# JonasGeiping/fullbatchtraining

Measured on AMD Instinct MI355X. Metric: full-batch GD images/sec (ResNet-18 CIFAR-10 shaped, all chunks accumulated per step), higher is better.
Workload: dtype bf16

## Files before the change

fullbatchtraining_amd/csrc/bn.hip:

```cpp
#include "common.h"
#include "profile.h"

__device__ __forceinline__ bool partial_sum2(const float* __restrict__ part, int n_mblocks, int blocks_per_group, int C, int g,
                                             int& c, double& s, double& q) {
    __shared__ double red[2][64][16];
    const int segs = (int)blockDim.x >> 4;
    const int cl = threadIdx.x & 15, seg = threadIdx.x >> 4;
    c = blockIdx.x * 16 + cl;
    double a = 0.0, b = 0.0;
    if (c < C) {
        const float* ps = part + ((long long)g * blocks_per_group) * C + c;
        const float* pq = part + ((long long)n_mblocks + (long long)g * blocks_per_group) * C + c;
        for (int k = seg; k < blocks_per_group; k += segs) { a += (double)ps[(long long)k * C]; b += (double)pq[(long long)k * C]; }
    }
    red[0][seg][cl] = a; red[1][seg][cl] = b;
    __syncthreads();
    if (seg != 0 || c >= C) return false;
    s = 0.0; q = 0.0;
    for (int k = 0; k < segs; ++k) { s += red[0][k][cl]; q += red[1][k][cl]; }
    return true;
}
static inline int bn_finalize_threads(int blocks_per_group) { return blocks_per_group >= 256 ? 1024 : 256; }

__global__ void bn_fwd_finalize_kernel(const float* __restrict__ part, int n_mblocks, int blocks_per_group, int C, double inv_count,
// ... 238 lines not shown
    float m = rm[c], v = rv[c];
    const float ub = unbias[c], keep = 1.f - momentum;
    for (int g = 0; g < n_groups; ++g)
        for (int p = 0; p < n_passes; ++p) {
            const long long o = p * pass_stride + (long long)g * ch_total + c;
            m = keep * m + momentum * mean_tab[o];
            v = keep * v + momentum * (var_tab[o] * ub);
        }
    rm[c] = m; rv[c] = v;
}

extern "C" int fb_bn_running_update(float* running_mean, float* running_var, const float* mean_tab, const float* var_tab, int32_t n_passes,
                                    int64_t pass_stride, const float* unbias, int32_t n_groups, int32_t ch_total, float momentum,
                                    void* stream) {
    if (!running_mean || !running_var || !mean_tab || !var_tab || !unbias) FB_FAIL(FB_ERR_ARG, "fb_bn_running_update: null pointer");
    hipLaunchKernelGGL(bn_running_update_kernel, dim3((ch_total + 255) / 256), dim3(256), 0, (hipStream_t)stream, running_mean,
                       running_var, mean_tab, var_tab, n_passes, (long long)pass_stride, unbias, n_groups, ch_total, momentum);
    FB_CHECK_LAUNCH("fb_bn_running_update");
    return FB_OK;
}

static inline int bn_reduce_pixels(long long n_pixels, long long ppg) {
    int pb = 128;
    while (pb < 1024 && ppg % (2 * pb) == 0 && n_pixels / (2 * pb) >= 2048) pb *= 2;
    return pb;
}
extern "C" int32_t fb_bn_bwd_reduce_rows(int64_t n_pixels, int64_t pixels_per_group) {
    if (n_pixels <= 0 || pixels_per_group <= 0) return 0;
    const int pb = bn_reduce_pixels(n_pixels, pixels_per_group);
    return (int32_t)((n_pixels + pb - 1) / pb);
}

struct BnReduceB { const uint4* x; const float* invstd; float* partial; int ch_off; };
template <typename T, bool DUAL = false>
__global__ __launch_bounds__(256) void bn_bwd_reduce_kernel(const uint4* __restrict__ dout, const uint4* __restrict__ y,
                                                            const unsigned char* __restrict__ mask,
                                                            const uint4* __restrict__ x, const float* __restrict__ mean_tab,
                                                            const float* __restrict__ invstd, int ch_total, int ch_off,
                                                            float* __restrict__ partial, long long n_pixels, int C, long long ppg,
                                                            int n_mblocks, int PB, const BnReduceB B) {
    constexpr int V = ET<T>::VEC;
    extern __shared__ float sm[];
    const int cvec = C / V;
    const long long p0 = (long long)blockIdx.x * PB;
    const long long g = p0 / ppg;
    const long long p1 = p0 + PB < n_pixels ? p0 + PB : n_pixels;
    auto mask_at = [&](long long i) -> unsigned {
        if (mask) return mask[i];
        if (!y) return 0xffu;
        float yv[V];
        ET<T>::unpack(y[i], yv);
        unsigned mk = 0;
#pragma unroll
        for (int k = 0; k < V; ++k) mk |= (yv[k] > 0.f ? 1u : 0u) << k;
        return mk;
    };
    int rows;
    if (256 % cvec == 0) {
        rows = 256 / cvec;
        const int cv = threadIdx.x % cvec, row = threadIdx.x / cvec, c0 = cv * V;
        float mu[V], is[V], s1[V], s2[V];
        float muB[DUAL ? V : 1], isB[DUAL ? V : 1], s2B[DUAL ? V : 1];
#pragma unroll
        for (int k = 0; k < V; ++k) { mu[k] = mean_tab[g * ch_total + ch_off + c0 + k]; is[k] = invstd[g * C + c0 + k]; s1[k] = 0.f; s2[k] = 0.f; }
        if constexpr (DUAL) {
#pragma unroll
            for (int k = 0; k < V; ++k) { muB[k] = mean_tab[g * ch_total + B.ch_off + c0 + k]; isB[k] = B.invstd[g * C + c0 + k]; s2B[k] = 0.f; }
        }
        auto one = [&](const uint4& dr, const uint4& xr, const uint4& xbr, unsigned mk) {
            float d[V], xv[V];
            ET<T>::unpack(dr, d); ET<T>::unpack(xr, xv);
#pragma unroll
            for (int k = 0; k < V; ++k) {
                const float dy = ((mk >> k) & 1u) ? d[k] : 0.f;
                s1[k] += dy; s2[k] += dy * ((xv[k] - mu[k]) * is[k]);
            }
            if constexpr (DUAL) {
                float xb[V];
                ET<T>::unpack(xbr, xb);
#pragma unroll
                for (int k = 0; k < V; ++k) {
                    const float dy = ((mk >> k) & 1u) ? d[k] : 0.f;
                    s2B[k] += dy * ((xb[k] - muB[k]) * isB[k]);
                }
            }
        };
        const long long hi = p1 * cvec;
        long long i = p0 * cvec + threadIdx.x;
        for (; i + (BN_SPAN_U - 1) * 256 < hi; i += BN_SPAN_U * 256) {
            uint4 dr[BN_SPAN_U], xr[BN_SPAN_U], xbr[BN_SPAN_U];
            unsigned mk[BN_SPAN_U];
#pragma unroll
            for (int u = 0; u < BN_SPAN_U; ++u) {
                dr[u] = ld_reduce(dout + i + u * 256); xr[u] = ld_reduce(x + i + u * 256); mk[u] = mask_at(i + u * 256);
                if constexpr (DUAL) xbr[u] = ld_reduce(B.x + i + u * 256); else xbr[u] = xr[u];
            }
#pragma unroll
            for (int u = 0; u < BN_SPAN_U; ++u) one(dr[u], xr[u], xbr[u], mk[u]);
        }
        for (; i < hi; i += 256) { if constexpr (DUAL) one(dout[i], x[i], B.x[i], mask_at(i)); else one(dout[i], x[i], x[i], mask_at(i)); }
#pragma unroll
        for (int k = 0; k < V; ++k) { sm[(row * C + c0 + k) * 2] = s1[k]; sm[(row * C + c0 + k) * 2 + 1] = s2[k]; }
        if constexpr (DUAL) {
#pragma unroll
            for (int k = 0; k < V; ++k) sm[2 * rows * C + row * C + c0 + k] = s2B[k];
        }
    } else {
        rows = 256 / cvec > 0 ? 256 / cvec : 1;
        const int lanes = cvec < 256 ? cvec : 256;
        for (int cv = threadIdx.x % lanes; cv < cvec; cv += lanes) {
            const int row = threadIdx.x / lanes;
            const int c0 = cv * V;
            float mu[V], is[V], s1[V], s2[V];
#pragma unroll
            for (int k = 0; k < V; ++k) { mu[k] = mean_tab[g * ch_total + ch_off + c0 + k]; is[k] = invstd[g * C + c0 + k]; s1[k] = 0.f; s2[k] = 0.f; }
            if (row < rows) {
                for (long long pidx = p0 + row; pidx < p1; pidx += rows) {
                    const long long i = pidx * cvec + cv;
                    float d[V], xv[V];
                    ET<T>::unpack(dout[i], d); ET<T>::unpack(x[i], xv);
                    const unsigned mk = mask_at(i);
#pragma unroll
                    for (int k = 0; k < V; ++k) {
                        const float dy = ((mk >> k) & 1u) ? d[k] : 0.f;
                        s1[k] += dy; s2[k] += dy * ((xv[k] - mu[k]) * is[k]);
                    }
                }
#pragma unroll
                for (int k = 0; k < V; ++k) { sm[(row * C + c0 + k) * 2] = s1[k]; sm[(row * C + c0 + k) * 2 + 1] = s2[k]; }
            }
        }
    }
    __syncthreads();
    for (int c = threadIdx.x; c < C; c += 256) {
        float a = 0.f, b = 0.f;
        for (int r = 0; r < rows; ++r) { a += sm[(r * C + c) * 2]; b += sm[(r * C + c) * 2 + 1]; }
        partial[(long long)blockIdx.x * C + c] = a;
        partial[((long long)n_mblocks + blockIdx.x) * C + c] = b;
        if constexpr (DUAL) {
            float bb = 0.f;
            for (int r = 0; r < rows; ++r) bb += sm[2 * rows * C + r * C + c];
            B.partial[(long long)blockIdx.x * C + c] = a;
            B.partial[((long long)n_mblocks + blockIdx.x) * C + c] = bb;
        }
    }
}

extern "C" int fb_bn_bwd_reduce(const void* dout, const void* y, const void* mask, const void* x, const float* mean_tab, const float* invstd,
                                int32_t ch_total, int32_t ch_off, float* partial, int64_t n_pixels, int32_t C,
                                int64_t pixels_per_group, int32_t dtype, void* stream) {
    if (!dout || !x || !mean_tab || !invstd || !partial) FB_FAIL(FB_ERR_ARG, "fb_bn_bwd_reduce: null pointer");
    if (pixels_per_group % 128 != 0) FB_FAIL(FB_ERR_SHAPE, "fb_bn_bwd_reduce: pixels_per_group=%lld must be a multiple of 128", (long long)pixels_per_group);
    const int V = dtype == FB_F32 ? 4 : 8;
    if (C % V != 0) FB_FAIL(FB_ERR_SHAPE, "fb_bn_bwd_reduce: C=%d", C);
    const int cvec = C / V, rows = 256 / cvec > 0 ? 256 / cvec : 1;
    const int PB = bn_reduce_pixels(n_pixels, pixels_per_group);
    const int n_mblocks = fb_bn_bwd_reduce_rows(n_pixels, pixels_per_group);
    const size_t smem = (size_t)rows * C * 2 * sizeof(float);
    if (smem > 64 * 1024) FB_FAIL(FB_ERR_UNSUPPORTED, "fb_bn_bwd_reduce: C=%d too large", C);
    const int32_t info[FB_PROF_INFO] = {(int32_t)(n_pixels / 128), C, (int32_t)(pixels_per_group / 128), dtype, 0, (mask || y) ? 1 : 0, 0, 0, 0, 0, 0};
    const int prof = fb_prof_begin(FB_PROF_BN_BWD_REDUCE, (hipStream_t)stream, info);
    if (dtype == FB_F32)
        hipLaunchKernelGGL((bn_bwd_reduce_kernel<float>), dim3(n_mblocks), dim3(256), smem, (hipStream_t)stream, (const uint4*)dout, (const uint4*)y,
                           (const unsigned char*)mask, (const uint4*)x, mean_tab, invstd, ch_total, ch_off, partial, (long long)n_pixels, C, (long long)pixels_per_group, n_mblocks, PB, BnReduceB{});
    else
        hipLaunchKernelGGL((bn_bwd_reduce_kernel<bf16_tag>), dim3(n_mblocks), dim3(256), smem, (hipStream_t)stream, (const uint4*)dout, (const uint4*)y,
                           (const unsigned char*)mask, (const uint4*)x, mean_tab, invstd, ch_total, ch_off, partial, (long long)n_pixels, C, (long long)pixels_per_group, n_mblocks, PB, BnReduceB{});
    fb_prof_end(prof, (hipStream_t)stream);
    FB_CHECK_LAUNCH("fb_bn_bwd_reduce");
    return FB_OK;
}

extern "C" int fb_bn_bwd_reduce2(const void* dout, const void* mask, const void* x_a, const float* invstd_a, int32_t ch_off_a, float* partial_a,
                                 const void* x_b, const float* invstd_b, int32_t ch_off_b, float* partial_b, const float* mean_tab, int32_t ch_total,
                                 int64_t n_pixels, int32_t C, int64_t pixels_per_group, int32_t dtype, void* stream) {
    if (!dout || !x_a || !x_b || !mean_tab || !invstd_a || !invstd_b || !partial_a || !partial_b) FB_FAIL(FB_ERR_ARG, "fb_bn_bwd_reduce2: null pointer");
    if (pixels_per_group % 128 != 0) FB_FAIL(FB_ERR_SHAPE, "fb_bn_bwd_reduce2: pixels_per_group=%lld must be a multiple of 128", (long long)pixels_per_group);
    const int V = dtype == FB_F32 ? 4 : 8;
    if (C % V != 0 || 256 % (C / V) != 0) FB_FAIL(FB_ERR_UNSUPPORTED, "fb_bn_bwd_reduce2: C=%d (the channel vectors of a pixel must divide 256)", C);
    const int cvec = C / V, rows = 256 / cvec;
    const int PB = bn_reduce_pixels(n_pixels, pixels_per_group);
    const int n_mblocks = fb_bn_bwd_reduce_rows(n_pixels, pixels_per_group);
    const size_t smem = (size_t)rows * C * 3 * sizeof(float);
    const int32_t info[FB_PROF_INFO] = {(int32_t)(n_pixels / 128), C, (int32_t)(pixels_per_group / 128), dtype, 1 , mask ? 1 : 0, 0, 0, 0, 0, 0};
    const int prof = fb_prof_begin(FB_PROF_BN_BWD_REDUCE, (hipStream_t)stream, info);
    const BnReduceB B{(const uint4*)x_b, invstd_b, partial_b, ch_off_b};
    if (dtype == FB_F32)
        hipLaunchKernelGGL((bn_bwd_reduce_kernel<float, true>), dim3(n_mblocks), dim3(256), smem, (hipStream_t)stream, (const uint4*)dout, (const uint4*)nullptr,
                           (const unsigned char*)mask, (const uint4*)x_a, mean_tab, invstd_a, ch_total, ch_off_a, partial_a, (long long)n_pixels, C, (long long)pixels_per_group, n_mblocks, PB, B);
    else
        hipLaunchKernelGGL((bn_bwd_reduce_kernel<bf16_tag, true>), dim3(n_mblocks), dim3(256), smem, (hipStream_t)stream, (const uint4*)dout, (const uint4*)nullptr,
                           (const unsigned char*)mask, (const uint4*)x_a, mean_tab, invstd_a, ch_total, ch_off_a, partial_a, (long long)n_pixels, C, (long long)pixels_per_group, n_mblocks, PB, B);
    fb_prof_end(prof, (hipStream_t)stream);
    FB_CHECK_LAUNCH("fb_bn_bwd_reduce2");
    return FB_OK;
}

__global__ void bn_bwd_finalize_kernel(const float* __restrict__ part, int n_mblocks, int blocks_per_group, int C, double inv_count,
                                       const float* __restrict__ scale, const float* __restrict__ mean_tab, const float* __restrict__ invstd,
                                       int ch_total, int ch_off, float* __restrict__ dgamma, float* __restrict__ dbeta, long long gstride,
                                       float* __restrict__ coef, int raw_x) {
    const int g = blockIdx.y;
    int c; double s1, s2;
    if (!partial_sum2(part, n_mblocks, blocks_per_group, C, g, c, s1, s2)) return;
    if (raw_x)
        s2 = (double)invstd[(long long)g * C + c] * (s2 - (double)mean_tab[(long long)g * ch_total + ch_off + c] * s1);
    dbeta[(long long)g * gstride + c] = (float)s1;
    dgamma[(long long)g * gstride + c] = (float)s2;
    const double sc = scale[(long long)g * C + c], is = invstd[(long long)g * C + c], mu = mean_tab[(long long)g * ch_total + ch_off + c];
    const double cx = -sc * is * s2 * inv_count;
    float* o = coef + ((long long)g * C + c) * 3;
    o[0] = (float)sc; o[1] = (float)cx; o[2] = (float)(-sc * s1 * inv_count - cx * mu);
}

extern "C" int fb_bn_bwd_finalize(const float* partial, int32_t n_mblocks, int32_t n_groups, int32_t C, double count, const float* scale,
                                  const float* mean_tab, const float* invstd, int32_t ch_total, int32_t ch_off, float* dgamma,
                                  float* dbeta, int64_t grad_group_stride, float* coef, int32_t raw_x, void* stream) {
    if (!partial || !scale || !mean_tab || !invstd || !dgamma || !dbeta || !coef) FB_FAIL(FB_ERR_ARG, "fb_bn_bwd_finalize: null pointer");
    if (n_mblocks % n_groups != 0) FB_FAIL(FB_ERR_SHAPE, "fb_bn_bwd_finalize: blocks/groups");
    dim3 grid((C + 15) / 16, n_groups);
    hipLaunchKernelGGL(bn_bwd_finalize_kernel, grid, dim3(bn_finalize_threads(n_mblocks / n_groups)), 0, (hipStream_t)stream, partial, n_mblocks, n_mblocks / n_groups, C, 1.0 / count,
                       scale, mean_tab, invstd, ch_total, ch_off, dgamma, dbeta, (long long)grad_group_stride, coef, (int)raw_x);
    FB_CHECK_LAUNCH("fb_bn_bwd_finalize");
    return FB_OK;
}

template <typename T>
__global__ void bn_bwd_apply_kernel(const uint4* __restrict__ dout, const uint4* __restrict__ y, const unsigned char* __restrict__ mask,
                                    const uint4* __restrict__ x,
                                    const float* __restrict__ coef, uint4* __restrict__ dx, uint4* __restrict__ dy_out, long long n_vec,
                                    int cvec, long long vec_per_group, int C) {
    constexpr int V = ET<T>::VEC;
    for (long long i = (long long)blockIdx.x * blockDim.x + threadIdx.x; i < n_vec; i += (long long)gridDim.x * blockDim.x) {
        const int c0 = (int)(i % cvec) * V;
        const long long g = i / vec_per_group;
        float d[V], xv[V], yv[V], o[V], dyv[V];
        ET<T>::unpack(dout[i], d); ET<T>::unpack(x[i], xv);
        unsigned mk = 0xffu;
        if (mask) mk = mask[i];
        else if (y) {
            ET<T>::unpack(y[i], yv);
            mk = 0;
#pragma unroll
            for (int k = 0; k < V; ++k) mk |= (yv[k] > 0.f ? 1u : 0u) << k;
        }
        const float* cf = coef + (g * C + c0) * 3;
#pragma unroll
        for (int k = 0; k < V; ++k) {
            const float dy = ((mk >> k) & 1u) ? d[k] : 0.f;
            dyv[k] = dy;
            o[k] = fb_bn_dx(cf[3 * k], cf[3 * k + 1], cf[3 * k + 2], dy, xv[k]);
        }
        dx[i] = ET<T>::pack(o);
        if (dy_out) dy_out[i] = ET<T>::pack(dyv);
    }
}

struct BnApplyB { const uint4* x; const float* coef; uint4* dx; };
template <typename T, bool DUAL = false>
__global__ __launch_bounds__(256) void bn_bwd_apply_span_kernel(const uint4* __restrict__ dout, const uint4* __restrict__ y,
                                                                const unsigned char* __restrict__ mask, const uint4* __restrict__ x,
                                                                const float* __restrict__ coef, uint4* __restrict__ dx, uint4* __restrict__ dy_out,
                                                                long long n_vec, int cvec, long long vec_per_group, int C, int span, float* __restrict__ amax,
                                                                BnApplyB B) {
    constexpr int V = ET<T>::VEC;
    float am = 0.f;
    const long long g = blockIdx.y, base = g * vec_per_group;
    const long long lim = n_vec - base < vec_per_group ? n_vec - base : vec_per_group;
    const long long lo = (long long)blockIdx.x * span;
    const long long hi = lo + span < lim ? lo + span : lim;
    const int c0 = (int)(threadIdx.x % cvec) * V;
    float cf[3 * V];
    load_coef<3 * V>(coef + (g * C + c0) * 3, cf);
    float cfB[DUAL ? 3 * V : 1];
    if constexpr (DUAL) { load_coef<3 * V>(B.coef + (g * C + c0) * 3, cfB); B.x += base; B.dx += base; }
    dout += base; x += base; dx += base;
    if (mask) mask += base;
    if (y) y += base;
    if (dy_out) dy_out += base;
    auto one = [&](const uint4& dr, const uint4& xr, const uint4& xbr, unsigned mk, long long i) {
        float d[V], xv[V], o[V], dyv[V];
        ET<T>::unpack(dr, d); ET<T>::unpack(xr, xv);
#pragma unroll
        for (int k = 0; k < V; ++k) {
            const float dy = ((mk >> k) & 1u) ? d[k] : 0.f;
            dyv[k] = dy;
            o[k] = fb_bn_dx(cf[3 * k], cf[3 * k + 1], cf[3 * k + 2], dy, xv[k]);
        }
        if (amax) {
#pragma unroll
            for (int k = 0; k < V; ++k) am = fmaxf(am, fabsf(o[k]));
        }
        st_stream(dx + i, ET<T>::pack(o));
        if (dy_out) st_stream(dy_out + i, ET<T>::pack(dyv));
        if constexpr (DUAL) {
            float xb[V], ob[V];
            ET<T>::unpack(xbr, xb);
#pragma unroll
            for (int k = 0; k < V; ++k) ob[k] = fb_bn_dx(cfB[3 * k], cfB[3 * k + 1], cfB[3 * k + 2], dyv[k], xb[k]);
            st_stream(B.dx + i, ET<T>::pack(ob));
        }
    };
    auto mask_at = [&](long long i) -> unsigned {
        if (mask) return mask[i];
        if (!y) return 0xffu;
        float yv[V];
        ET<T>::unpack(y[i], yv);
        unsigned mk = 0;
#pragma unroll
        for (int k = 0; k < V; ++k) mk |= (yv[k] > 0.f ? 1u : 0u) << k;
        return mk;
    };
    long long i = lo + threadIdx.x;
    for (; i + (BN_SPAN_U - 1) * 256 < hi; i += BN_SPAN_U * 256) {
        uint4 dr[BN_SPAN_U], xr[BN_SPAN_U], xbr[BN_SPAN_U];
        unsigned mk[BN_SPAN_U];
#pragma unroll
        for (int u = 0; u < BN_SPAN_U; ++u) {
            dr[u] = ld_stream(dout + i + u * 256); xr[u] = ld_stream(x + i + u * 256); mk[u] = mask_at(i + u * 256);
            if constexpr (DUAL) xbr[u] = ld_stream(B.x + i + u * 256); else xbr[u] = xr[u];
        }
#pragma unroll
        for (int u = 0; u < BN_SPAN_U; ++u) one(dr[u], xr[u], xbr[u], mk[u], i + u * 256);
    }
    for (; i < hi; i += 256) { if constexpr (DUAL) one(dout[i], x[i], B.x[i], mask_at(i), i); else one(dout[i], x[i], x[i], mask_at(i), i); }
    if (amax) amax_commit(amax, am);
}

extern "C" int fb_bn_bwd_apply(const void* dout, const void* y, const void* mask, const void* x, const float* coef, void* dx, void* dy_out,
                               int64_t n_pixels, int32_t C, int64_t pixels_per_group, int32_t dtype, float* amax_out, float* amax_ws, void* stream) {
    if (!dout || !x || !coef || !dx) FB_FAIL(FB_ERR_ARG, "fb_bn_bwd_apply: null pointer");
    if (amax_out && (dtype != FB_F32 || !amax_ws)) FB_FAIL(FB_ERR_ARG, "fb_bn_bwd_apply: amax_out is for fp32 tensors and needs amax_ws (fb_ws_bn_amax_floats)");
    const int64_t n_groups = (n_pixels + pixels_per_group - 1) / pixels_per_group;
    const int V = dtype == FB_F32 ? 4 : 8;
    const int cvec = C / V;
    const long long n_vec = n_pixels * cvec, vpg = pixels_per_group * cvec;
    const int32_t info[FB_PROF_INFO] = {(int32_t)(n_pixels / 128), C, (int32_t)(pixels_per_group / 128), dtype, 0, (mask || y) ? 1 : 0, dy_out ? 1 : 0, 0, 0, 0, 0};
    if (256 % cvec == 0 && vpg > 0) {
        const int prof = fb_prof_begin(FB_PROF_BN_BWD_APPLY, (hipStream_t)stream, info);
        const int span = bn_span(n_vec);
        const dim3 grid((unsigned)((vpg + span - 1) / span), (unsigned)((n_vec + vpg - 1) / vpg));
        if (dtype == FB_F32)
            hipLaunchKernelGGL((bn_bwd_apply_span_kernel<float>), grid, dim3(256), 0, (hipStream_t)stream, (const uint4*)dout, (const uint4*)y,
                               (const unsigned char*)mask, (const uint4*)x, coef, (uint4*)dx, (uint4*)dy_out, n_vec, cvec, vpg, C, span, amax_out ? amax_ws : nullptr, BnApplyB{});
        else
            hipLaunchKernelGGL((bn_bwd_apply_span_kernel<bf16_tag>), grid, dim3(256), 0, (hipStream_t)stream, (const uint4*)dout, (const uint4*)y,
                               (const unsigned char*)mask, (const uint4*)x, coef, (uint4*)dx, (uint4*)dy_out, n_vec, cvec, vpg, C, span, nullptr, BnApplyB{});
        fb_prof_end(prof, (hipStream_t)stream);
        if (amax_out) hipLaunchKernelGGL(amax_finish_kernel, dim3(grid.y), dim3(256), 0, (hipStream_t)stream, amax_ws, (int)grid.x, amax_out);
        FB_CHECK_LAUNCH("fb_bn_bwd_apply");
        return FB_OK;
    }
    const int blocks = (int)((n_vec + 255) / 256 < 8192 ? (n_vec + 255) / 256 : 8192);
    if (dtype == FB_F32)
        hipLaunchKernelGGL((bn_bwd_apply_kernel<float>), dim3(blocks), dim3(256), 0, (hipStream_t)stream, (const uint4*)dout, (const uint4*)y,
                           (const unsigned char*)mask, (const uint4*)x, coef, (uint4*)dx, (uint4*)dy_out, n_vec, cvec, vpg, C);
    else
        hipLaunchKernelGGL((bn_bwd_apply_kernel<bf16_tag>), dim3(blocks), dim3(256), 0, (hipStream_t)stream, (const uint4*)dout, (const uint4*)y,
                           (const unsigned char*)mask, (const uint4*)x, coef, (uint4*)dx, (uint4*)dy_out, n_vec, cvec, vpg, C);
    FB_CHECK_LAUNCH("fb_bn_bwd_apply");
    if (amax_out) return fb_absmax((const float*)dx, pixels_per_group * C, (int32_t)n_groups, pixels_per_group * C, 1, amax_out, stream);
    return FB_OK;
}


extern "C" int fb_bn_bwd_apply2(const void* dout, const void* mask, const void* x_a, const float* coef_a, void* dx_a, const void* x_b, const float* coef_b,
                                void* dx_b, int64_t n_pixels, int32_t C, int64_t pixels_per_group, int32_t dtype, void* stream) {
    if (!dout || !x_a || !coef_a || !dx_a || !x_b || !coef_b || !dx_b) FB_FAIL(FB_ERR_ARG, "fb_bn_bwd_apply2: null pointer");
    const int V = dtype == FB_F32 ? 4 : 8;
    if (C % V != 0 || 256 % (C / V) != 0 || pixels_per_group <= 0) FB_FAIL(FB_ERR_UNSUPPORTED, "fb_bn_bwd_apply2: C=%d (the channel vectors of a pixel must divide 256)", C);
    const int cvec = C / V;
    const long long n_vec = n_pixels * cvec, vpg = pixels_per_group * cvec;
    const int32_t info[FB_PROF_INFO] = {(int32_t)(n_pixels / 128), C, (int32_t)(pixels_per_group / 128), dtype, 1 , mask ? 1 : 0, 0, 0, 0, 0, 0};
    const int prof = fb_prof_begin(FB_PROF_BN_BWD_APPLY, (hipStream_t)stream, info);
    const int span = bn_span(n_vec);
    const dim3 grid((unsigned)((vpg + span - 1) / span), (unsigned)((n_vec + vpg - 1) / vpg));
    const BnApplyB B{(const uint4*)x_b, coef_b, (uint4*)dx_b};
    if (dtype == FB_F32)
        hipLaunchKernelGGL((bn_bwd_apply_span_kernel<float, true>), grid, dim3(256), 0, (hipStream_t)stream, (const uint4*)dout, (const uint4*)nullptr,
                           (const unsigned char*)mask, (const uint4*)x_a, coef_a, (uint4*)dx_a, (uint4*)nullptr, n_vec, cvec, vpg, C, span, (float*)nullptr, B);
    else
        hipLaunchKernelGGL((bn_bwd_apply_span_kernel<bf16_tag, true>), grid, dim3(256), 0, (hipStream_t)stream, (const uint4*)dout, (const uint4*)nullptr,
                           (const unsigned char*)mask, (const uint4*)x_a, coef_a, (uint4*)dx_a, (uint4*)nullptr, n_vec, cvec, vpg, C, span, (float*)nullptr, B);
    fb_prof_end(prof, (hipStream_t)stream);
    FB_CHECK_LAUNCH("fb_bn_bwd_apply2");
    return FB_OK;
}
```

fullbatchtraining_amd/csrc/cmdlist.cpp:

```cpp
#include <stdlib.h>

#include <memory>
#include <utility>
#include <vector>

#include "common.h"

namespace {

template <typename T> inline T word_as(uint64_t w) {
    T v;
    memcpy(&v, &w, sizeof(T));
    return v;
}

using Thunk = int (*)(const uint64_t*, void*);

template <typename F, F f> struct Bind;
template <typename... A, int (*f)(A...)> struct Bind<int (*)(A...), f> {
    static constexpr int N = sizeof...(A);
    template <size_t I, typename T> static T arg(const uint64_t* w, void* st) {
        if constexpr (I == N - 1) return (T)st;
        else return word_as<T>(w[I]);
    }
    template <size_t... I> static int run(const uint64_t* w, void* st, std::index_sequence<I...>) { return f(arg<I, A>(w, st)...); }
    static int call(const uint64_t* w, void* st) { return run(w, st, std::index_sequence_for<A...>{}); }
};

struct Entry { const char* name; Thunk fn; int nargs; };
#define FB_ENTRY(name) {#name, &Bind<decltype(&name), &name>::call, Bind<decltype(&name), &name>::N}
const Entry kEntries[] = {
    FB_ENTRY(fb_conv2d), FB_ENTRY(fb_conv2d_wgrad), FB_ENTRY(fb_absmax), FB_ENTRY(fb_wgrad_reduce), FB_ENTRY(fb_weight_prep),
    FB_ENTRY(fb_bn_fwd_finalize), FB_ENTRY(fb_bn_apply), FB_ENTRY(fb_bn_running_update), FB_ENTRY(fb_bn_bwd_reduce),
    FB_ENTRY(fb_bn_bwd_finalize), FB_ENTRY(fb_bn_bwd_apply), FB_ENTRY(fb_avgpool2_fwd), FB_ENTRY(fb_maxpool3s2_fwd),
    FB_ENTRY(fb_maxpool3s2_bwd), FB_ENTRY(fb_head_pool), FB_ENTRY(fb_head_loss), FB_ENTRY(fb_head_bwd), FB_ENTRY(fb_mt_sqnorm),
    FB_ENTRY(fb_mt_accumulate), FB_ENTRY(fb_mt_fd_perturb), FB_ENTRY(fb_mt_fd_combine_accumulate), FB_ENTRY(fb_mt_fd_combine),
    FB_ENTRY(fb_mt_chunk_clip), FB_ENTRY(fb_bn_eval_coeffs), FB_ENTRY(fb_mt_norms2), FB_ENTRY(fb_mt_clip_sgd), FB_ENTRY(fb_mt_scale), FB_ENTRY(fb_bn_bwd_fused), FB_ENTRY(fb_bn_bwd_reduce2), FB_ENTRY(fb_bn_bwd_apply2),
    FB_ENTRY(fb_conv2d_wgrad_chain), FB_ENTRY(fb_mt_accumulate_sum), FB_ENTRY(fb_mt_accumulate_skip),
    FB_ENTRY(fb_maxpool3s2_fwd_idx), FB_ENTRY(fb_maxpool3s2_bwd_idx),
};
constexpr int kNumEntries = sizeof(kEntries) / sizeof(kEntries[0]);

enum { CMD_CALL = 0, CMD_EVENT_RECORD = 1, CMD_EVENT_WAIT = 2 };
struct Cmd { int32_t kind, fn, stream, ev; uint32_t off, n; };
struct CmdList {
    std::vector<Cmd> cmds;
    std::vector<uint64_t> words;
    std::vector<std::unique_ptr<uint64_t[]>> blobs;
};

std::vector<hipEvent_t> g_events;

}

extern "C" int32_t fb_cmd_fn_id(const char* name) {
    for (int i = 0; i < kNumEntries; ++i)
        if (strcmp(kEntries[i].name, name) == 0) return i;
    return -1;
}
extern "C" int32_t fb_cmd_fn_nargs(int32_t fn) { return fn >= 0 && fn < kNumEntries ? kEntries[fn].nargs : -1; }

extern "C" int32_t fb_event_new(void) {
    hipEvent_t e;
    if (hipEventCreateWithFlags(&e, hipEventDisableTiming) != hipSuccess) {
        snprintf(fb_err_buf, sizeof(fb_err_buf), "fb_event_new: hipEventCreateWithFlags failed");
        return -1;
    }
    g_events.push_back(e);
    return (int32_t)g_events.size() - 1;
}
extern "C" int32_t fb_event_count(void) { return (int32_t)g_events.size(); }
extern "C" int fb_event_record(int32_t ev, void* stream) {
// ... 62 lines not shown
```

fullbatchtraining_amd/csrc/common.h:

```cpp
#pragma once
#include <hip/hip_runtime.h>
#include <stdint.h>
#include <stdio.h>
#include <string.h>

#include "../../include/fb_engine.h"

typedef __attribute__((ext_vector_type(8))) __bf16 bf16x8_t;
typedef __attribute__((ext_vector_type(4))) short s16x4_t;
typedef __attribute__((ext_vector_type(4))) float f32x4_t;

extern thread_local char fb_err_buf[512];
#define FB_FAIL(code, ...)                                   \
    do {                                                     \
        snprintf(fb_err_buf, sizeof(fb_err_buf), __VA_ARGS__); \
        return (code);                                       \
    } while (0)
#define FB_CHECK_LAUNCH(name)                                                                   \
    do {                                                                                        \
        hipError_t e_ = hipGetLastError();                                                      \
        if (e_ != hipSuccess) FB_FAIL(FB_ERR_LAUNCH, "%s: launch failed: %s", name, hipGetErrorString(e_)); \
    } while (0)

static inline int64_t ceil_div64(int64_t a, int64_t b) { return (a + b - 1) / b; }
// ... 234 lines not shown
    c = __builtin_amdgcn_mfma_f32_16x16x32_f16(ah, bh, c, 0, 0, 0);
    return c;
}
__device__ __forceinline__ f32x4_t mma_planes3h(const uint4 (&a)[2], const uint4 (&b)[2], f32x4_t c, float inv) {
    const f16x8_t ah = __builtin_bit_cast(f16x8_t, a[0]), al = __builtin_bit_cast(f16x8_t, a[1]);
    const f16x8_t bh = __builtin_bit_cast(f16x8_t, b[0]), bl = __builtin_bit_cast(f16x8_t, b[1]);
    f32x4_t t = {0.f, 0.f, 0.f, 0.f};
    t = __builtin_amdgcn_mfma_f32_16x16x32_f16(al, bh, t, 0, 0, 0);
    t = __builtin_amdgcn_mfma_f32_16x16x32_f16(ah, bl, t, 0, 0, 0);
    t = __builtin_amdgcn_mfma_f32_16x16x32_f16(ah, bh, t, 0, 0, 0);
    return fma4(t, inv, c);
}
bool fb_f32_split_enabled();
bool fb_experimental();
const char* fb_getenv_experimental(const char* name);
int fb_persistent_cus();

typedef __attribute__((ext_vector_type(4))) unsigned fb_store_u32x4;
#ifndef FB_STORE_GUARD_NOPS
#define FB_STORE_GUARD_NOPS 3
#endif
__device__ __forceinline__ void store_b128_guard(fb_store_u32x4 data) {
#if FB_STORE_GUARD_NOPS >= 0
#ifdef FB_STORE_GUARD_NOMEM
    asm volatile("s_nop %1" ::"v"(data), "n"(FB_STORE_GUARD_NOPS));
#else
    asm volatile("s_nop %1" ::"v"(data), "n"(FB_STORE_GUARD_NOPS) : "memory");
#endif
#endif
}

__device__ __forceinline__ float fb_bn_dx(float c_dy, float c_x, float c_0, float dy, float x) { return fmaf(c_dy, dy, fmaf(c_x, x, c_0)); }

__device__ __forceinline__ float row16_sum(float v) {
    v += __builtin_bit_cast(float, __builtin_amdgcn_update_dpp(0, __builtin_bit_cast(int, v), 0x128, 0xf, 0xf, false));
    v += __builtin_bit_cast(float, __builtin_amdgcn_update_dpp(0, __builtin_bit_cast(int, v), 0x124, 0xf, 0xf, false));
    v += __builtin_bit_cast(float, __builtin_amdgcn_update_dpp(0, __builtin_bit_cast(int, v), 0x122, 0xf, 0xf, false));
    v += __builtin_bit_cast(float, __builtin_amdgcn_update_dpp(0, __builtin_bit_cast(int, v), 0x121, 0xf, 0xf, false));
    return v;
}

template <int NV> __device__ __forceinline__ void block_reduce_sum(float (&v)[NV], float* smem) {
    const int lane = threadIdx.x & 63, wave = threadIdx.x >> 6, nw = (blockDim.x + 63) >> 6;
#pragma unroll
    for (int i = 0; i < NV; ++i) {
#pragma unroll
        for (int off = 32; off > 0; off >>= 1) v[i] += __shfl_xor(v[i], off);
    }
    if (lane == 0)
        for (int i = 0; i < NV; ++i) smem[i * nw + wave] = v[i];
    __syncthreads();
    if (threadIdx.x == 0)
        for (int i = 0; i < NV; ++i) {
            float s = 0.f;
            for (int w = 0; w < nw; ++w) s += smem[i * nw + w];
            v[i] = s;
        }
    __syncthreads();
}
```

fullbatchtraining_amd/csrc/conv3x3_halo5.hip:

```cpp
#include "common.h"

#include <type_traits>

struct Halo5Params {
    const char* src; const char* wgt; char* dst; const char* addend; float* stat;
    const unsigned char* addend_mask;
    const char* bst_x; const unsigned char* bst_mask;
    int n_img, mode, addend_mode, n_mblocks, n_tiles;
#ifdef FB_H5_TRACE
    long long* trace;
#endif
};
#ifdef FB_H5_TRACE
#define H5_STAMP(k) do { if (tid == 0) p.trace[(long long)L * 8 + (k)] = wall_clock64(); } while (0)
#else
#define H5_STAMP(k) do { } while (0)
#endif

namespace {
template <int N> __device__ __forceinline__ void h5_wait_vmcnt() { asm volatile("s_waitcnt vmcnt(%0)" ::"n"(N) : "memory"); }
template <int N> __device__ __forceinline__ void h5_wait_lgkmcnt() {
    asm volatile("s_waitcnt lgkmcnt(%0)" ::"n"(N) : "memory");
    __builtin_amdgcn_sched_barrier(0);
}
typedef __attribute__((ext_vector_type(4))) unsigned h5_u32x4;
typedef __attribute__((ext_vector_type(2))) unsigned h5_u32x2;
template <int OFF> __device__ __forceinline__ uint4 h5_read16(unsigned byte_addr) {
    h5_u32x4 v;
    asm volatile("ds_read_b128 %0, %1 offset:%2" : "=v"(v) : "v"(byte_addr), "n"(OFF));
    return make_uint4(v[0], v[1], v[2], v[3]);
}
template <int I, int N, typename F> __device__ __forceinline__ void h5_static_for(F&& f) {
    if constexpr (I < N) { f(std::integral_constant<int, I>{}); h5_static_for<I + 1, N>(f); }
}
__device__ __forceinline__ int h5_xcd_remap(int b, int n) {
    const int q = n >> 3, r = n & 7, xcd = b & 7, slot = b >> 3;
    return (xcd < r ? xcd * (q + 1) : r * (q + 1) + (xcd - r) * q) + slot;
}
constexpr unsigned H5_OOB = 0x80000000u;
constexpr int H5_W = 32, H5_TH = 8, H5_PITCH = 34, H5_ROWS = (H5_TH + 2) * H5_PITCH;
constexpr int H5_NGRP = (H5_ROWS + 7) / 8;
constexpr int H5_HALO_BYTES = H5_NGRP * 1024, H5_WT_BYTES = 64 * 128, H5_WGT_BYTES = 9 * H5_WT_BYTES;
constexpr int H5_KH = (H5_NGRP + 3) / 4;
#ifndef FB_H5_ADD_DEPTH
#define FB_H5_ADD_DEPTH 3
#endif
constexpr int H5_AD = FB_H5_ADD_DEPTH, H5_ADN = H5_AD + 1;
}

template <int MODE, int ADD, int BST = 0>
__global__ __launch_bounds__(256) void conv3x3s1_c64_halo5_kernel(const Halo5Params p) {
#if defined(__HIP_DEVICE_COMPILE__)
    constexpr int W = H5_W, PITCH = H5_PITCH;
    __shared__ __attribute__((aligned(16))) char lds[H5_WGT_BYTES + 2 * H5_HALO_BYTES + 1024];

    const int tid = threadIdx.x, lane = tid & 63;
    const int wave = __builtin_amdgcn_readfirstlane(tid >> 6);
    const int ph = wave & 1, ch = wave >> 1;
    const int NB = gridDim.x;
    const int lrow8 = lane >> 3, t = lane & 15, g = lane >> 4;
    const unsigned lds0 = (unsigned)(size_t)(__attribute__((address_space(3))) char*)lds;

    {
        const __amdgpu_buffer_rsrc_t rW = __builtin_amdgcn_make_buffer_rsrc((void*)p.wgt, 0, 64 * 9 * 128, 0x00020000);
#pragma unroll
        for (int u = 0; u < 9; ++u) {
            const int tap = MODE == 0 ? u : 8 - u;
#pragma unroll
            for (int k = 0; k < 2; ++k) {
                const int piece = wave + 4 * k;
                const unsigned voff = (unsigned)((piece * 8 + lrow8) * 9 * 128 + (((lane & 7) ^ lrow8) * 16));
                __builtin_amdgcn_raw_ptr_buffer_load_lds(rW, (__attribute__((address_space(3))) void*)(lds + u * H5_WT_BYTES + piece * 1024), 16, voff,
                                                         tap * 128, 0, 0);
            }
        }
    }
    unsigned voffH[H5_KH];
    unsigned topbits = 0, botbits = 0;
#pragma unroll
    for (int k = 0; k < H5_KH; ++k) {
        const int row = (wave + 4 * k) * 8 + lrow8;
        const int hy = row / PITCH, hx = row - hy * PITCH;
        const bool ok = row < H5_ROWS && hx >= 1 && hx <= W;
        voffH[k] = ok ? (unsigned)((hy * W + hx) * 128 + (((lane & 7) ^ (hx & 7)) * 16)) : H5_OOB;
        topbits |= (hy == 0 ? 1u : 0u) << k;
        botbits |= (hy == H5_TH + 1 ? 1u : 0u) << k;
    }
    unsigned wa[2], wb[2];
#pragma unroll
    for (int h = 0; h < 2; ++h) {
        wa[h] = lds0 + (ch * 32 + t) * 128 + (((g + 4 * h) ^ (t & 7)) * 16);
        wb[h] = wa[h] + 4 * H5_WT_BYTES;
    }
    unsigned pa[2][3][2];
#pragma unroll
    for (int bf = 0; bf < 2; ++bf)
#pragma unroll
        for (int b = 0; b < 3; ++b)
#pragma unroll
            for (int h = 0; h < 2; ++h)
                pa[bf][b][h] = lds0 + H5_WGT_BYTES + bf * H5_HALO_BYTES + (ph * 4 * PITCH + t + b) * 128 + (((g + 4 * h) ^ ((t + b) & 7)) * 16);
    const int voffD = ((ph * 128 + t) * 64 + ch * 32 + g * 4) * 2;
    const int voffS = ((ph * 128 + t) * 64 + ch * 32 + (g & 1) * 16 + (g >> 1) * 8) * 2;

    auto halo_piece = [&](auto kc, int buf, int L, bool live) {
        constexpr int K = decltype(kc)::value;
        const int grp = wave + 4 * K;
        const int n0 = L >> 2, y0 = (L & 3) * H5_TH;
        const long long origin = ((long long)(n0 * W + y0 - 1) * W - 1) * 128;
        const __amdgpu_buffer_rsrc_t rA = __builtin_amdgcn_make_buffer_rsrc((void*)(p.src + origin), 0, ((H5_TH + 2) * W + 2) * 128, 0x00020000);
        const unsigned dead = (y0 == 0 ? topbits : 0u) | (y0 + H5_TH == W ? botbits : 0u);
        const unsigned v = (((dead >> K) & 1u) || !live) ? H5_OOB : voffH[K];
        const int dst = grp < H5_NGRP ? H5_WGT_BYTES + buf * H5_HALO_BYTES + grp * 1024 : H5_WGT_BYTES + 2 * H5_HALO_BYTES;
        __builtin_amdgcn_raw_ptr_buffer_load_lds(rA, (__attribute__((address_space(3))) void*)(lds + dst), 16, v, 0, 0, 0);
    };

    float ssum[2][4], ssq[2][4];
    h5_u32x2 ad[H5_ADN][2];
    unsigned adm[H5_ADN];
    h5_u32x2 bx[H5_ADN][2];
    unsigned bxm[H5_ADN];
    auto ad_issue = [&](auto jc, const int Lp) {
        constexpr int J = decltype(jc)::value;
        if constexpr (BST != 0 && J < 8) {
            const __amdgpu_buffer_rsrc_t rsrcX = __builtin_amdgcn_make_buffer_rsrc((void*)(p.bst_x + (long long)Lp * 256 * 128), 0, 256 * 128, 0x00020000);
#pragma unroll
            for (int i = 0; i < 2; ++i) bx[J % H5_ADN][i] = __builtin_amdgcn_raw_buffer_load_b64(rsrcX, voffD + i * 32, J * 2048, 0);
            const __amdgpu_buffer_rsrc_t rsrcN = __builtin_amdgcn_make_buffer_rsrc((void*)(p.bst_mask + (long long)Lp * 256 * 8), 0, 256 * 8, 0x00020000);
            bxm[J % H5_ADN] = __builtin_amdgcn_raw_buffer_load_b32(rsrcN, ((ph * 128 + t) * 8 + ch * 4), J * 128, 0);
        }
        if constexpr (ADD != 0 && J < 8) {
            const __amdgpu_buffer_rsrc_t rsrcE = __builtin_amdgcn_make_buffer_rsrc((void*)(p.addend + (long long)Lp * 256 * 128), 0, 256 * 128, 0x00020000);
#pragma unroll
            for (int i = 0; i < 2; ++i) ad[J % H5_ADN][i] = __builtin_amdgcn_raw_buffer_load_b64(rsrcE, voffD + i * 32, J * 2048, 0);
            if constexpr (ADD == 2) {
                const __amdgpu_buffer_rsrc_t rsrcM = __builtin_amdgcn_make_buffer_rsrc((void*)(p.addend_mask + (long long)Lp * 256 * 8), 0, 256 * 8, 0x00020000);
                adm[J % H5_ADN] = __builtin_amdgcn_raw_buffer_load_b32(rsrcM, ((ph * 128 + t) * 8 + ch * 4), J * 128, 0);
            }
        }
    };
    auto epi_prefetch = [&](const int Lp) { h5_static_for<0, H5_AD>([&](auto jc) { ad_issue(jc, Lp); }); };
    auto epi_slice = [&](auto sc, f32x4_t (&accp)[2][8], const int Lp) {
        constexpr int S = decltype(sc)::value;
        if constexpr (S < 16) {
            if constexpr (S == 0) {
#pragma unroll
                for (int i = 0; i < 2; ++i)
// ... 35 lines not shown
                        for (int r = 0; r < 4; ++r) { ssum[i][r] += v[r]; ssq[i][r] += v[r] * v[r]; }
                    }
                }
                const h5_u32x2 lo = __builtin_amdgcn_permlane16_swap(pk[0][0], pk[1][0], false, false);
                const h5_u32x2 hi = __builtin_amdgcn_permlane16_swap(pk[0][1], pk[1][1], false, false);
                const h5_u32x4 outv = {lo[0], hi[0], lo[1], hi[1]};
                __builtin_amdgcn_raw_buffer_store_b128(outv, rsrcD, voffS, J * 2048, 0);
                store_b128_guard(outv);
                ad_issue(std::integral_constant<int, J + H5_AD>{}, Lp);
            }
        } else if constexpr (S == 16) {
            if constexpr (MODE == 0 || BST != 0) {
#pragma unroll
                for (int i = 0; i < 2; ++i)
#pragma unroll
                    for (int r = 0; r < 4; ++r) { ssum[i][r] = row16_sum(ssum[i][r]); ssq[i][r] = row16_sum(ssq[i][r]); }
            }
        } else {
            if ((MODE == 0 || BST != 0) && t == 0) {
                const long long blk = 2LL * Lp + ph;
#pragma unroll
                for (int i = 0; i < 2; ++i) {
                    const int co = ch * 32 + i * 16 + g * 4;
                    *(float4*)(p.stat + blk * 64 + co) = make_float4(ssum[i][0], ssum[i][1], ssum[i][2], ssum[i][3]);
                    *(float4*)(p.stat + ((long long)p.n_mblocks + blk) * 64 + co) = make_float4(ssq[i][0], ssq[i][1], ssq[i][2], ssq[i][3]);
                }
            }
        }
    };

    int L = h5_xcd_remap(blockIdx.x, NB);
    if (L >= p.n_tiles) return;
    h5_static_for<0, H5_KH>([&](auto kc) { halo_piece(kc, 0, L, true); });

    f32x4_t accA[2][8], accB[2][8];

    auto tile = [&](auto bufc, auto prevc, const int L, const bool has_next) {
        constexpr int BUF = decltype(bufc)::value;
        constexpr bool PREV = decltype(prevc)::value;
        f32x4_t (&acc)[2][8] = BUF ? accB : accA;
        f32x4_t (&accp)[2][8] = BUF ? accA : accB;
        H5_STAMP(0);
        h5_wait_vmcnt<0>();
        __builtin_amdgcn_s_barrier();
        H5_STAMP(1);
#pragma unroll
        for (int i = 0; i < 2; ++i)
#pragma unroll
            for (int j = 0; j < 8; ++j) acc[i][j] = (f32x4_t){0.f, 0.f, 0.f, 0.f};

        uint4 wf[2][2], pf[2][8];
        auto issue_reads = [&](auto sc) {
            constexpr int S = decltype(sc)::value, U = S >> 1, H = S & 1, A = U / 3, B = U % 3, SET = S & 1;
            h5_static_for<0, 2>([&](auto ic) {
                constexpr int I = decltype(ic)::value;
                if constexpr (U < 4) wf[SET][I] = h5_read16<U * H5_WT_BYTES + I * 2048>(wa[H]);
                else wf[SET][I] = h5_read16<(U - 4) * H5_WT_BYTES + I * 2048>(wb[H]);
            });
            h5_static_for<0, 8>([&](auto jc) {
                constexpr int J = decltype(jc)::value;
                pf[SET][J] = h5_read16<((A + (J >> 1)) * PITCH + (J & 1) * 16) * 128>(pa[BUF][B][H]);
            });
        };
        issue_reads(std::integral_constant<int, 0>{});
        if constexpr (PREV) epi_prefetch(L - NB);
        h5_static_for<0, 18>([&](auto sc) {
            constexpr int S = decltype(sc)::value, SET = S & 1;
            if constexpr (S + 1 < 18) {
                issue_reads(std::integral_constant<int, S + 1>{});
                h5_wait_lgkmcnt<10>();
            } else {
                h5_wait_lgkmcnt<0>();
            }
#pragma unroll
            for (int i = 0; i < 2; ++i)
#pragma unroll
                for (int j = 0; j < 8; ++j) acc[i][j] = mma_chunk<bf16_tag>(wf[SET][i], pf[SET][j], acc[i][j]);
            if constexpr (PREV) epi_slice(sc, accp, L - NB);
            if constexpr (PREV) {
#pragma unroll
                for (int k = 0; k < 16; ++k) {
                    __builtin_amdgcn_sched_group_barrier(0x008, 1, 0);
                    __builtin_amdgcn_sched_group_barrier(0x002, 2, 0);
                }
            }
            if constexpr (S < H5_KH) halo_piece(std::integral_constant<int, S>{}, BUF ^ 1, has_next ? L + NB : L, has_next);
        });
        H5_STAMP(3);
    };

    bool has_next = L + NB < p.n_tiles;
    tile(std::integral_constant<int, 0>{}, std::false_type{}, L, has_next);
    int parity = 0;
    while (has_next) {
        L += NB;
        has_next = L + NB < p.n_tiles;
        tile(std::integral_constant<int, 1>{}, std::true_type{}, L, has_next);
        parity = 1;
        if (!has_next) break;
        L += NB;
        has_next = L + NB < p.n_tiles;
        tile(std::integral_constant<int, 0>{}, std::true_type{}, L, has_next);
        parity = 0;
    }
    epi_prefetch(L);
    if (parity == 0) h5_static_for<0, 18>([&](auto sc) { epi_slice(sc, accA, L); });
    else h5_static_for<0, 18>([&](auto sc) { epi_slice(sc, accB, L); });
    h5_wait_vmcnt<0>();
    H5_STAMP(4); H5_STAMP(5);
#endif
}

int fb_conv3x3_halo5_takes(const fb_conv_args* a) {
    static const bool disabled = getenv("FB_DISABLE_HALO5") != nullptr;
    if (disabled || a->dtype != FB_BF16) return 0;
    if (a->R != 3 || a->S != 3 || a->stride != 1 || a->pad != 1) return 0;
    if (a->Hs != 32 || a->Ws != 32 || a->Hd != 32 || a->Wd != 32 || a->Cs != 64 || a->Cd != 64) return 0;
    if (a->imgs_per_wset > 0 && a->imgs_per_wset < a->n_img) return 0;
    if (a->addend && a->addend_mode != 1) return 0;
    if (a->addend_mask && (!a->addend || a->mode != 1)) return 0;
    if (a->mode == 0 && !a->stat_partial) return 0;
    if (a->bst_x && (a->mode != 1 || !a->bst_mask || !a->stat_partial)) return 0;
    return 1;
}

int fb_try_conv3x3_halo5(const fb_conv_args* a, hipStream_t st) {
    if (!fb_conv3x3_halo5_takes(a)) return 0;
    const int n_cu = fb_persistent_cus();
    Halo5Params p;
    p.src = (const char*)a->src; p.wgt = (const char*)a->wgt; p.dst = (char*)a->dst; p.addend = (const char*)a->addend;
    p.stat = (a->mode == 0 || a->bst_x) ? a->stat_partial : nullptr;
    p.addend_mask = (const unsigned char*)a->addend_mask;
    p.bst_x = (const char*)a->bst_x; p.bst_mask = (const unsigned char*)a->bst_mask;
    p.n_img = a->n_img; p.mode = a->mode; p.addend_mode = a->addend ? 1 : 0;
    p.n_tiles = a->n_img * 4;
    p.n_mblocks = p.n_tiles * 2;
#ifdef FB_H5_TRACE
    extern long long* g_h5_trace;
    p.trace = g_h5_trace;
#endif
    const dim3 grid(p.n_tiles < n_cu ? p.n_tiles : n_cu);
    if (a->mode == 0) {
        hipLaunchKernelGGL((conv3x3s1_c64_halo5_kernel<0, 0>), grid, dim3(256), 0, st, p);
    } else if (a->bst_x) {
        if (a->addend && a->addend_mask) hipLaunchKernelGGL((conv3x3s1_c64_halo5_kernel<1, 2, 1>), grid, dim3(256), 0, st, p);
        else if (a->addend) hipLaunchKernelGGL((conv3x3s1_c64_halo5_kernel<1, 1, 1>), grid, dim3(256), 0, st, p);
        else hipLaunchKernelGGL((conv3x3s1_c64_halo5_kernel<1, 0, 1>), grid, dim3(256), 0, st, p);
    } else if (a->addend && a->addend_mask) {
        hipLaunchKernelGGL((conv3x3s1_c64_halo5_kernel<1, 2>), grid, dim3(256), 0, st, p);
    } else if (a->addend) {
        hipLaunchKernelGGL((conv3x3s1_c64_halo5_kernel<1, 1>), grid, dim3(256), 0, st, p);
    } else {
        hipLaunchKernelGGL((conv3x3s1_c64_halo5_kernel<1, 0>), grid, dim3(256), 0, st, p);
    }
    return 1;
}
```

fullbatchtraining_amd/csrc/conv_igemm.hip:

```cpp
#include "common.h"
#include "profile.h"

#include "conv_params.h"

template <typename T, int BN_CO>
__global__ __launch_bounds__(256) void conv_igemm_kernel(const ConvParams p) {
    constexpr int EB = ET<T>::EB;
    constexpr int BKE = 128 / EB;
    constexpr int WROWS = BN_CO / 32;
    constexpr int FI = BN_CO / 32;
    constexpr int FJ = 4;
    constexpr int TILE_CHUNKS = (128 + BN_CO) * 8;
    __shared__ uint4 lds[2 * TILE_CHUNKS];

    const int tid = threadIdx.x, lane = tid & 63, wave = tid >> 6;
    const int wave_co = wave >> 1, wave_px = wave & 1;
    const int mblk = blockIdx.x, co_blk = blockIdx.y, cls = blockIdx.z;
    const int cpy = (p.os == 2) ? (cls >> 1) : 0, cpx = (p.os == 2) ? (cls & 1) : 0;
    const int chunk = tid & 7, lrow = tid >> 3;

    int a_img[4], a_y[4], a_x[4];
    const int qHW = p.qH * p.qW;
#pragma unroll
    for (int i = 0; i < 4; ++i) {
// ... 125 lines not shown
#pragma unroll
                for (int r = 0; r < 4; ++r) { ssum[i][r] += v[r]; ssq[i][r] += v[r] * v[r]; }
            }
        }
    }
    if (p.stat != nullptr) {
        float* red = (float*)lds;
        __syncthreads();
#pragma unroll
        for (int i = 0; i < FI; ++i)
#pragma unroll
            for (int r = 0; r < 4; ++r) {
                float a = ssum[i][r], b = ssq[i][r];
                a = row16_sum(a); b = row16_sum(b);
                if ((lane & 15) == 0) {
                    const int col = wave_co * (BN_CO / 2) + i * 16 + (lane >> 4) * 4 + r;
                    red[(wave_px * BN_CO + col) * 2] = a; red[(wave_px * BN_CO + col) * 2 + 1] = b;
                }
            }
        __syncthreads();
        if (tid < BN_CO) {
            const float a = red[tid * 2] + red[(BN_CO + tid) * 2];
            const float b = red[tid * 2 + 1] + red[(BN_CO + tid) * 2 + 1];
            const long long blk = (long long)cls * gridDim.x + mblk;
            p.stat[blk * p.Cd + co_blk * BN_CO + tid] = a;
            p.stat[((long long)p.n_mblocks + blk) * p.Cd + co_blk * BN_CO + tid] = b;
        }
    }
}

int fb_try_conv3x3_halo4(const fb_conv_args* a, hipStream_t st);
int fb_try_conv3x3_halo5(const fb_conv_args* a, hipStream_t st);
int fb_conv3x3_halo5_takes(const fb_conv_args* a);
int fb_try_conv3x3s2_dgrad_quad(const fb_conv_args* a, hipStream_t st);
int fb_try_conv1x1_k32(const fb_conv_args* a, hipStream_t st);
int fb_try_conv1x1_stream(const fb_conv_args* a, hipStream_t st);
int fb_try_conv1x1_gemm(const fb_conv_args* a, hipStream_t st);
int fb_try_conv1x1_pipe(const fb_conv_args* a, hipStream_t st);

int fb_conv1x1_pipe_takes(const fb_conv_args* a);
int fb_conv3x3_halo4_takes(const fb_conv_args* a);
int fb_conv1x1_gemm_takes(const fb_conv_args* a);
static int igemm_masked_addend_ok(const fb_conv_args* a) {
    if (getenv("FB_IGEMM_NO_MASK") != nullptr || a->mode != 1 || a->stride != 1 || a->bst_x) return 0;
    if (a->Cs % 32 != 0 || a->Cd % 64 != 0) return 0;
    static const bool v1 = getenv("FB_IGEMM_V1") != nullptr;
    if (v1) return 0;
    ConvParams p{};
    p.n_img = a->n_img; p.Hs = a->Hs; p.Ws = a->Ws; p.Cs = a->Cs; p.Hd = a->Hd; p.Wd = a->Wd; p.Cd = a->Cd; p.R = a->R; p.S = a->S;
    p.qH = a->Hd; p.qW = a->Wd;
    return fb_igemm_glds_fits(p, a->dtype);
}
extern "C" int32_t fb_conv_masked_addend_supported(const fb_conv_args* a) {
    if (!a || !a->addend || !a->addend_mask || a->addend_mode != 1) return 0;
    return fb_conv3x3_halo5_takes(a) || fb_conv1x1_pipe_takes(a) || fb_conv3x3_halo4_takes(a) || fb_conv1x1_gemm_takes(a) || igemm_masked_addend_ok(a);
}

extern "C" int32_t fb_conv_bwd_stat_supported(const fb_conv_args* a) {
    static const bool disabled = getenv("FB_DISABLE_FUSED_BWD_STAT") != nullptr;
    if (disabled || !a || !a->bst_x || !a->bst_mask || !a->stat_partial || a->mode != 1 || a->dtype != FB_BF16) return 0;
    if ((long long)a->n_img * a->Hd * a->Wd % 128 != 0) return 0;
    static const char* widths = getenv("FB_FUSED_BWD_STAT_W");
    if (widths) {
        char tag[8];
        snprintf(tag, sizeof(tag), "%d,", a->Wd);
        char list[64];
        snprintf(list, sizeof(list), "%s,", widths);
        if (!strstr(list, tag) || (a->Wd < 10 && list != strstr(list, tag) && *(strstr(list, tag) - 1) != ',')) return 0;
    }
    return fb_conv3x3_halo5_takes(a) || fb_conv3x3_halo4_takes(a);
}

template <typename T> static int launch_conv(const ConvParams& p, int classes, hipStream_t st) {
    const int mblocks = (p.M + 127) / 128;
    if (p.Cd % 128 == 0 && (long long)mblocks * (p.Cd / 128) * classes >= 512) {
        dim3 grid(mblocks, p.Cd / 128, classes);
        hipLaunchKernelGGL((conv_igemm_kernel<T, 128>), grid, dim3(256), 0, st, p);
    } else {
        dim3 grid(mblocks, p.Cd / 64, classes);
        hipLaunchKernelGGL((conv_igemm_kernel<T, 64>), grid, dim3(256), 0, st, p);
    }
    return 0;
}

extern "C" int fb_conv2d(const fb_conv_args* a, void* stream) {
    if (!a || !a->src || !a->wgt || !a->dst) FB_FAIL(FB_ERR_ARG, "fb_conv2d: null pointer");
    const int EB = a->dtype == FB_F32 ? 4 : 2;
    if (a->Cs % 32 != 0) FB_FAIL(FB_ERR_SHAPE, "fb_conv2d: Cs=%d must be a multiple of 32", a->Cs);
    if (a->Cd % 64 != 0) FB_FAIL(FB_ERR_SHAPE, "fb_conv2d: Cd=%d must be a multiple of 64", a->Cd);
    if (a->mode != 0 && a->mode != 1) FB_FAIL(FB_ERR_ARG, "fb_conv2d: mode %d", a->mode);
    if (a->addend_mask && !fb_conv_masked_addend_supported(a))
        FB_FAIL(FB_ERR_UNSUPPORTED, "fb_conv2d: addend_mask is not implemented for this shape (ask fb_conv_masked_addend_supported)");
    if (a->bst_x && !fb_conv_bwd_stat_supported(a))
        FB_FAIL(FB_ERR_UNSUPPORTED, "fb_conv2d: the fused BatchNorm-backward reduction is not implemented for this shape (ask fb_conv_bwd_stat_supported)");
    if (a->stride != 1 && a->stride != 2) FB_FAIL(FB_ERR_UNSUPPORTED, "fb_conv2d: stride %d", a->stride);
    ConvParams p;
    p.src = (const char*)a->src; p.wgt = (const char*)a->wgt; p.dst = (char*)a->dst; p.addend = (const char*)a->addend;
    p.stat = a->stat_partial;
    p.n_img = a->n_img; p.Hs = a->Hs; p.Ws = a->Ws; p.Cs = a->Cs; p.Hd = a->Hd; p.Wd = a->Wd; p.Cd = a->Cd;
    p.R = a->R; p.S = a->S; p.stride = a->stride; p.pad = a->pad; p.mode = a->mode;
    p.imgs_per_wset = a->imgs_per_wset > 0 ? a->imgs_per_wset : a->n_img;
    p.wset_stride_bytes = a->wset_stride * EB;
    p.addend_mode = a->addend ? a->addend_mode : 0;
    p.addend_mask = a->addend ? (const unsigned char*)a->addend_mask : nullptr;
    p.amax_src = a->dtype == FB_F32 ? a->amax_src : nullptr; p.amax_wgt = a->dtype == FB_F32 ? a->amax_wgt : nullptr;
    if ((p.amax_src == nullptr) != (p.amax_wgt == nullptr)) FB_FAIL(FB_ERR_ARG, "fb_conv2d: amax_src and amax_wgt go together");
    p.amax_imgs = a->amax_imgs > 0 ? a->amax_imgs : a->n_img;
    int classes = 1;
    if (a->mode == 0) {
        if (a->Hd != (a->Hs + 2 * a->pad - a->R) / a->stride + 1 || a->Wd != (a->Ws + 2 * a->pad - a->S) / a->stride + 1)
            FB_FAIL(FB_ERR_SHAPE, "fb_conv2d: fwd output %dx%d inconsistent with input %dx%d", a->Hd, a->Wd, a->Hs, a->Ws);
        p.qH = a->Hd; p.qW = a->Wd; p.os = 1; p.ss = a->stride;
    } else {
        if (a->Hs != (a->Hd + 2 * a->pad - a->R) / a->stride + 1 || a->Ws != (a->Wd + 2 * a->pad - a->S) / a->stride + 1)
            FB_FAIL(FB_ERR_SHAPE, "fb_conv2d: dgrad shapes inconsistent");
        if (a->stat_partial && !a->bst_x) FB_FAIL(FB_ERR_ARG, "fb_conv2d: statistics in mode 1 need bst_x / bst_mask");
        if (a->stride == 1) { p.qH = a->Hd; p.qW = a->Wd; p.os = 1; }
        else {
            if ((a->Hd & 1) || (a->Wd & 1)) FB_FAIL(FB_ERR_SHAPE, "fb_conv2d: stride-2 dgrad needs even input dims");
            p.qH = a->Hd / 2; p.qW = a->Wd / 2; p.os = 2; classes = 4;
        }
        p.ss = 1;
    }
    p.M = a->n_img * p.qH * p.qW;
    p.n_mblocks = ((p.M + 127) / 128) * classes;
    hipStream_t st = (hipStream_t)stream;
    const int32_t info[FB_PROF_INFO] = {a->n_img, a->Hs, a->Ws, a->Cs, a->Hd, a->Wd, a->Cd, a->R, a->stride,
                                        (a->addend ? a->addend_mode : 0) | (a->addend_mask ? 4 : 0) | (a->bst_x ? 8 : 0) | (a->dtype << 4), 0};
// ... 27 lines not shown
```

fullbatchtraining_amd/csrc/conv_wgrad.hip:

```cpp
#include "common.h"
#include "profile.h"

struct WgradParams {
    const char* x; const char* dy; float* out;
    int n_img, Hs, Ws, Cs, Hd, Wd, Cd;
    int R, S, stride, pad;
    int imgs_per_group, split_k, px_per_group, px_per_split;
    long long group_stride;
    const float* amax_x; const float* amax_dy;
    const char* bn_x; const unsigned char* bn_mask; const float* bn_coef;
};

template <typename T> struct WG;
template <> struct WG<bf16_tag> { static constexpr int PAD = 16; };
template <> struct WG<float> { static constexpr int PAD = 64; };
template <> struct WG<f32s_tag> : WG<float> {};
template <> struct WG<f32h_tag> : WG<float> {};

template <typename T> __device__ __forceinline__ void load_frag_t(const char* tile, int row_bytes, int pb, int c0, int lane, uint4 (&out)[2]);
template <> __device__ __forceinline__ void load_frag_t<bf16_tag>(const char* tile, int row_bytes, int pb, int c0, int lane, uint4 (&out)[2]) {
    const int t = lane & 15, g = lane >> 4;
    const char* a0 = tile + (pb + g * 8 + (t >> 2)) * row_bytes + (c0 + (t & 3) * 4) * 2;
    const s16x4_t lo = __builtin_amdgcn_ds_read_tr16_b64_v4i16((s16x4_t __attribute__((address_space(3)))*)(a0));
    const s16x4_t hi = __builtin_amdgcn_ds_read_tr16_b64_v4i16((s16x4_t __attribute__((address_space(3)))*)(a0 + 4 * row_bytes));
// ... 192 lines not shown
    if constexpr (WK > 1) {
        float* red = (float*)lds;
        __syncthreads();
#pragma unroll
        for (int i = 0; i < 4; ++i)
#pragma unroll
            for (int j = 0; j < NJ; ++j)
#pragma unroll
                for (int q = 0; q < 4; ++q) red[(wk * 64 + i * 16 + (lane >> 4) * 4 + q) * TN + wn * 16 * NJ + j * 16 + (lane & 15)] = acc[i][j][q];
        __syncthreads();
        for (int e = tid; e < 64 * TN; e += 256) {
            float v = 0.f;
#pragma unroll
            for (int w = 0; w < WK; ++w) v += red[w * 64 * TN + e];
            const int co = tile_m * TM + e / TN, ci = tile_n * TN + e % TN;
            out[((long long)co * taps + tap) * p.Cs + ci] = v;
        }
    } else {
#pragma unroll
        for (int i = 0; i < 4; ++i)
#pragma unroll
            for (int j = 0; j < NJ; ++j)
#pragma unroll
                for (int q = 0; q < 4; ++q) {
                    const int co = tile_m * TM + wm * 64 + i * 16 + (lane >> 4) * 4 + q;
                    const int ci = tile_n * TN + wn * 16 * NJ + j * 16 + (lane & 15);
                    out[((long long)co * taps + tap) * p.Cs + ci] = acc[i][j][q];
                }
    }
}

int fb_try_wgrad3x3(const fb_wgrad_args* a, hipStream_t st);
int fb_try_wgrad3x3_v2(const fb_wgrad_args* a, hipStream_t st);
int fb_try_wgrad1x1(const fb_wgrad_args* a, hipStream_t st);

extern "C" int32_t fb_wgrad_bn_fused_supported(const fb_wgrad_args* a) {
    static const bool disabled = getenv("FB_DISABLE_WGRAD_BNF") != nullptr;
    return !disabled && a && !a->amax_x && !a->amax_dy && a->R == 1 && a->S == 1 && a->stride == 1 && a->pad == 0 && a->Cs % 32 == 0 && a->Cs % 64 != 0
           && a->Cd % 64 == 0 && a->Hs == a->Hd && a->Ws == a->Wd;
}

extern "C" int fb_conv2d_wgrad(const fb_wgrad_args* a, void* stream) {
    if (!a || !a->x || !a->dy || !a->dw_partial) FB_FAIL(FB_ERR_ARG, "fb_conv2d_wgrad: null pointer");
    if (a->bn_x && (!a->bn_coef || !fb_wgrad_bn_fused_supported(a))) FB_FAIL(FB_ERR_UNSUPPORTED, "fb_conv2d_wgrad: bn_x (BatchNorm apply in the loader) is for 1x1 layers with Cs < 64 (no fp16x2 planes) and needs bn_coef");
    if (a->Cs % 32 != 0 || a->Cd % 64 != 0) FB_FAIL(FB_ERR_SHAPE, "fb_conv2d_wgrad: Cs=%d must be a multiple of 32, Cd=%d of 64", a->Cs, a->Cd);
    if (a->n_img % a->imgs_per_group != 0) FB_FAIL(FB_ERR_SHAPE, "fb_conv2d_wgrad: n_img %% imgs_per_group != 0");
    if (a->split_k < 1) FB_FAIL(FB_ERR_ARG, "fb_conv2d_wgrad: split_k < 1");
    WgradParams p;
    p.x = (const char*)a->x; p.dy = (const char*)a->dy; p.out = a->dw_partial;
    p.n_img = a->n_img; p.Hs = a->Hs; p.Ws = a->Ws; p.Cs = a->Cs; p.Hd = a->Hd; p.Wd = a->Wd; p.Cd = a->Cd;
    p.R = a->R; p.S = a->S; p.stride = a->stride; p.pad = a->pad;
    p.imgs_per_group = a->imgs_per_group; p.split_k = a->split_k;
    p.group_stride = a->group_stride ? a->group_stride : (long long)a->split_k * a->Cd * a->R * a->S * a->Cs;
    p.px_per_group = a->imgs_per_group * a->Hd * a->Wd;
    p.amax_x = a->dtype == FB_F32 ? a->amax_x : nullptr; p.amax_dy = a->dtype == FB_F32 ? a->amax_dy : nullptr;
    p.bn_x = (const char*)a->bn_x; p.bn_mask = (const unsigned char*)a->bn_mask; p.bn_coef = a->bn_coef;
    if ((p.amax_x == nullptr) != (p.amax_dy == nullptr)) FB_FAIL(FB_ERR_ARG, "fb_conv2d_wgrad: amax_x and amax_dy go together");
    const bool hsplit = p.amax_x != nullptr;
    const int n_groups = a->n_img / a->imgs_per_group;
    hipStream_t st = (hipStream_t)stream;
    const bool big = (a->Cs % 128 == 0) && (a->Cd % 128 == 0) && (a->Cs >= 256 || a->Cd >= 256 || a->R == 3);
    const int kstep = big ? (a->dtype == FB_F32 ? 32 : 64) : 128;
    p.px_per_split = (int)(ceil_div64(ceil_div64(p.px_per_group, a->split_k), kstep) * kstep);
    const int taps = a->R * a->S;
    const bool split = fb_f32_split_enabled();
    const int32_t info[FB_PROF_INFO] = {a->n_img, a->Hs, a->Ws, a->Cs, a->Hd, a->Wd, a->Cd, a->R, a->stride, a->split_k | (a->dtype << 16), FB_K_WGRAD_GENERIC};
    const int prof = fb_prof_begin(FB_PROF_WGRAD, st, info);
    static const bool wide160 = getenv("FB_DISABLE_WGRAD_WIDE160") == nullptr;
    if (wide160 && a->dtype == FB_BF16 && a->R == 1 && a->S == 1 && a->Cs % 160 == 0 && a->Cs % 64 != 0 && a->Cd % 64 == 0) {
        dim3 grid((a->Cd / 64) * (a->Cs / 160), taps, n_groups * a->split_k);
        if (a->bn_x) hipLaunchKernelGGL((conv_wgrad_kernel<bf16_tag, 1, 2, 2, 2, 5, true>), grid, dim3(256), 0, st, p);
        else hipLaunchKernelGGL((conv_wgrad_kernel<bf16_tag, 1, 2, 2, 2, 5, false>), grid, dim3(256), 0, st, p);
    } else if (a->bn_x) {
        dim3 grid((a->Cd / 64) * (a->Cs / 32), taps, n_groups * a->split_k);
        if (a->dtype == FB_F32 && split) hipLaunchKernelGGL((conv_wgrad_kernel<f32s_tag, 1, 1, 4, 1, 2, true>), grid, dim3(256), 0, st, p);
        else if (a->dtype == FB_F32) hipLaunchKernelGGL((conv_wgrad_kernel<float, 1, 1, 4, 1, 2, true>), grid, dim3(256), 0, st, p);
        else hipLaunchKernelGGL((conv_wgrad_kernel<bf16_tag, 1, 1, 4, 1, 2, true>), grid, dim3(256), 0, st, p);
    } else if (fb_try_wgrad3x3_v2(a, st)) { fb_prof_kernel(prof, FB_K_WGRAD3X3_V2);
// ... 160 lines not shown
```

fullbatchtraining_amd/csrc/conv_wgrad3x3_v2.hip:

```cpp
#include "common.h"

#include <type_traits>

struct Wgrad3V2Params {
    const char* x; const char* dy; float* out;
    int n_img, H, Cs, Cd;
    int imgs_per_group, imgs_per_block, split_k;
    long long group_stride;
    int n_chains; float* sq_part;
};

namespace {
typedef __attribute__((ext_vector_type(2))) unsigned w3_u32x2;
template <int OFF> __device__ __forceinline__ w3_u32x2 w3_read_tr(unsigned byte_addr) {
    w3_u32x2 v;
    asm volatile("ds_read_b64_tr_b16 %0, %1 offset:%2" : "=v"(v) : "v"(byte_addr), "n"(OFF));
    return v;
}
template <int N> __device__ __forceinline__ void w3_wait_lgkmcnt() {
    asm volatile("s_waitcnt lgkmcnt(%0)" ::"n"(N) : "memory");
    __builtin_amdgcn_sched_barrier(0);
}
template <int N> __device__ __forceinline__ void w3_wait_vmcnt() { asm volatile("s_waitcnt vmcnt(%0)" ::"n"(N) : "memory"); }
template <int I, int N, typename F> __device__ __forceinline__ void w3_static_for(F&& f) {
    if constexpr (I < N) { f(std::integral_constant<int, I>{}); w3_static_for<I + 1, N>(f); }
}
__device__ __forceinline__ uint4 w3_join(w3_u32x2 lo, w3_u32x2 hi) { return make_uint4(lo[0], lo[1], hi[0], hi[1]); }
__device__ __forceinline__ int w3_f(int row) { return ((row >> 1) & 1) | (((row >> 3) & 1) << 1); }
constexpr unsigned W3_OOB = 0x80000000u;

template <int W> struct W3GeoGen {
    static constexpr bool PER_BLOCK = true;
    static constexpr int RS = W == 56 ? 1 : (W == 28 ? 4 : 7);
    static constexpr int VALID = RS * W;
    static constexpr int KPX = (VALID + 31) / 32 * 32;
    static constexpr int PITCH = W == 56 ? 64 : (W == 28 ? 32 : 16);
    static constexpr int IMGS = 1;
    static constexpr int IMG_ROWS = (RS + 2) * PITCH;
    static constexpr int HROWS = IMG_ROWS;
    static constexpr bool WHOLE = false;
    __device__ static __forceinline__ int pix_row(int p, int s) { return p < VALID ? (p / W) * PITCH + (p % W) + s : 0; }
    static constexpr int blk_rows(int, int R) { return R * PITCH; }
// ... 27 lines not shown
    static constexpr int KPX = 32;
    static constexpr int PITCH = W == 16 ? 40 : (W == 8 ? 24 : 16);
    static constexpr int RS = W == 16 ? 2 : 4;
    static constexpr int IMGS = W == 4 ? 2 : 1;
    static constexpr int IMG_ROWS = (2 * RS + 1) * PITCH;
    static constexpr int HROWS = IMGS * IMG_ROWS;
    static constexpr int HI_DELTA = W == 4 ? 2 * PITCH : 8;
    static constexpr bool WHOLE = W == 4;
    __device__ static __forceinline__ int lane_row(int pl, int s) {
        if constexpr (W == 4) return (pl / 16) * IMG_ROWS + 2 * ((pl % 16) / 4) * PITCH + 2 * (pl % 4) + s;
        else return 2 * (pl / W) * PITCH + 2 * (pl % W) + s;
    }
    static constexpr int blk_rows(int, int R) { return R * PITCH; }
    __device__ static __forceinline__ int fB(int row) { return (row >> 1) & 3; }
};
struct W3GeoCP4 {
    static constexpr bool PER_BLOCK = false;
    static constexpr int VALID = 64, KPX = 64, PITCH = 4, RS = 4, IMGS = 4;
    static constexpr int IMG_ROWS = 17;
    static constexpr int BLK_ROWS = 48;
    static constexpr int HROWS = 88;
    static constexpr int HI_DELTA = 4;
    static constexpr bool WHOLE = true;
    __device__ static __forceinline__ int tap_row(int pl, int u) {
        const int img = pl / 16, y = (pl % 16) / 4 + u / 3 - 1, x = pl % 4 + u % 3 - 1;
        return img * IMG_ROWS + ((y >= 0 && y < 4 && x >= 0 && x < 4) ? y * 4 + x : 16);
    }
    __device__ static __forceinline__ int lane_row(int, int) { return 0; }
    static constexpr int blk_rows(int BLK, int) { return BLK * BLK_ROWS; }
    __device__ static __forceinline__ int fB(int row) { return w3_f(row); }
};
}

template <int W, int SD, bool CP = false, bool CHAIN = false>
__global__ __launch_bounds__(CHAIN ? 512 : 256) void conv_wgrad3x3_v2_kernel(const Wgrad3V2Params p) {
#if defined(__HIP_DEVICE_COMPILE__)
    static_assert(!CP || (W == 4 && SD == 1), "compact layout: 4x4 maps, stride 1");
    static_assert(!CHAIN || CP, "chunk chains: compact 4x4 layout");
    constexpr int NWV = CHAIN ? 8 : 4, FIW = CHAIN ? 2 : 4;
    using G = typename std::conditional<CP, W3GeoCP4, W3Geo<W, SD>>::type;
    constexpr int WI = SD * W;
    const int Hi = SD * p.H;
    constexpr int KPX = G::KPX, PITCH = G::PITCH, HROWS = G::HROWS;
    constexpr int A_BYTES = KPX * 128, B_BYTES = HROWS * 128, STAGE = A_BYTES + B_BYTES;
    constexpr int NGA = KPX / 8, NGB = HROWS / 8;
    constexpr int KA = (NGA + NWV - 1) / NWV, KB = (NGB + NWV - 1) / NWV;
    __shared__ __attribute__((aligned(16))) char lds[2 * STAGE];

    const int tid = threadIdx.x, lane = tid & 63;
    const int wave = __builtin_amdgcn_readfirstlane(tid >> 6);
    const int cib = CHAIN ? (wave & 3) : wave, coh = CHAIN ? (wave >> 2) : 0;
    const int tiles_n = p.Cs / 64, tiles = tiles_n * (p.Cd / 64);
    const int n_items = gridDim.x;
    int item;
    {
        const int b = blockIdx.x, q = n_items >> 3, r = n_items & 7, xcd = b & 7, slot = b >> 3;
        item = (xcd < r ? xcd * (q + 1) : r * (q + 1) + (xcd - r) * q) + slot;
    }
    const int tile = item % tiles, gs = item / tiles;
    const int tile_m = __builtin_amdgcn_readfirstlane(tile / tiles_n), tile_n = __builtin_amdgcn_readfirstlane(tile % tiles_n);
    const int group = __builtin_amdgcn_readfirstlane(CHAIN ? gs : gs / p.split_k), split = __builtin_amdgcn_readfirstlane(CHAIN ? 0 : gs % p.split_k);
    const int n_chunks = p.n_img / p.imgs_per_group;
    const int my_chunks = CHAIN ? (n_chunks - group + p.n_chains - 1) / p.n_chains : 0;
    const int spc = p.imgs_per_group / G::IMGS;
    const int img0 = CHAIN ? 0 : group * p.imgs_per_group + split * p.imgs_per_block;
    const int img_end = CHAIN ? p.n_img : min(img0 + p.imgs_per_block, (group + 1) * p.imgs_per_group);
    const int steps_per_img = G::WHOLE ? 1 : p.H / G::RS;
    const int n_steps = CHAIN ? my_chunks * spc : (G::WHOLE ? (img_end - img0) / G::IMGS : (img_end - img0) * steps_per_img);
    const int rowA_b = p.Cd * 2, rowB_b = p.Cs * 2;
// ... 30 lines not shown
            voffB[k] = (xok && sy >= 0 && sy < WI) ? base + (unsigned)(sy * WI * rowB_b) : W3_OOB;
        } else {
            hyB[k] = xok ? hy - 1 : -(1 << 20);
            voffB[k] = base;
        }
    }
    auto issue = [&](int stage, int step) {
        char* base = lds + stage * STAGE;
        int img, y0;
        if constexpr (CHAIN) { img = (group + (step / spc) * p.n_chains) * p.imgs_per_group + (step % spc) * G::IMGS; y0 = 0; }
        else if constexpr (G::WHOLE) { img = step * G::IMGS; y0 = 0; }
        else { img = step / steps_per_img; y0 = (step % steps_per_img) * G::RS; }
        const int soffA = (img * p.H + y0) * W * rowA_b;
#pragma unroll
        for (int k = 0; k < KA; ++k)
            if (wave + NWV * k < NGA)
                __builtin_amdgcn_raw_ptr_buffer_load_lds(rsrcA, (__attribute__((address_space(3))) void*)(base + (wave + NWV * k) * 1024), 16,
                                                         voffA[k], soffA, 0, 0);
        const int soffB = img * Hi * WI * rowB_b;
#pragma unroll
        for (int k = 0; k < KB; ++k) {
            if (wave + NWV * k < NGB) {
                unsigned v = voffB[k];
                if constexpr (!G::WHOLE) {
                    const int sy = SD * y0 + hyB[k];
                    v = (unsigned)sy < (unsigned)Hi ? voffB[k] + (unsigned)(sy * WI * rowB_b) : W3_OOB;
                }
                __builtin_amdgcn_raw_ptr_buffer_load_lds(rsrcB, (__attribute__((address_space(3))) void*)(base + A_BYTES + (wave + NWV * k) * 1024),
                                                         16, v, soffB, 0, 0);
            }
        }
    };

    const unsigned lds0 = (unsigned)(size_t)(__attribute__((address_space(3))) char*)lds;
    const int t = lane & 15, g = lane >> 4;
    const int pl = g * 8 + (t >> 2);
    unsigned la[FIW];
#pragma unroll
    for (int i = 0; i < FIW; ++i) la[i] = lds0 + pl * 128 + (((i + coh * FIW) ^ w3_f(pl)) * 32) + (t & 3) * 8;
    constexpr int NBLK = G::PER_BLOCK ? KPX / 32 : 1, NS = CP ? 9 : 3;
    unsigned lb[NBLK][NS], lbh[NBLK][NS];
#pragma unroll
    for (int blk = 0; blk < NBLK; ++blk)
#pragma unroll
        for (int s = 0; s < NS; ++s) {
            int row, rowh;
            if constexpr (CP) { row = W3GeoCP4::tap_row(pl, s); rowh = W3GeoCP4::tap_row(pl + 4, s); }
            else if constexpr (G::PER_BLOCK) { row = G::pix_row(blk * 32 + pl, s); rowh = G::pix_row(blk * 32 + pl + 4, s); }
            else { row = G::lane_row(pl, s); rowh = row + G::HI_DELTA; }
            lb[blk][s] = lds0 + A_BYTES + row * 128 + ((cib ^ G::fB(row)) * 32) + (t & 3) * 8;
            lbh[blk][s] = lds0 + A_BYTES + rowh * 128 + ((cib ^ G::fB(rowh)) * 32) + (t & 3) * 8;
        }

    f32x4_t acc[9][FIW], tot[CHAIN ? 9 : 1][CHAIN ? FIW : 1];
#pragma unroll
    for (int u = 0; u < 9; ++u)
#pragma unroll
        for (int i = 0; i < FIW; ++i) {
            acc[u][i] = (f32x4_t){0.f, 0.f, 0.f, 0.f};
            if constexpr (CHAIN) tot[u][i] = (f32x4_t){0.f, 0.f, 0.f, 0.f};
        }

    if (n_steps > 0) {
        issue(0, 0);
        w3_wait_vmcnt<0>();
        __builtin_amdgcn_s_barrier();
    }
    for (int step = 0; step < n_steps; ++step) {
        const int cur = step & 1;
        if (step + 1 < n_steps) issue(cur ^ 1, step + 1);
        const unsigned so = cur * STAGE;
        unsigned a0[FIW];
#pragma unroll
        for (int i = 0; i < FIW; ++i) a0[i] = la[i] + so;
        w3_static_for<0, KPX / 32>([&](auto blkc) {
            constexpr int BLK = decltype(blkc)::value;
            constexpr int PB = BLK * 32;
            constexpr int BI = G::PER_BLOCK ? BLK : 0;
            unsigned b0[NS], b1[NS];
#pragma unroll
            for (int s = 0; s < NS; ++s) { b0[s] = lb[BI][s] + so; b1[s] = lbh[BI][s] + so; }
            uint4 af[FIW];
            w3_static_for<0, FIW>([&](auto ic) {
                constexpr int I = decltype(ic)::value;
                af[I] = w3_join(w3_read_tr<PB * 128>(a0[I]), w3_read_tr<PB * 128 + 512>(a0[I]));
            });
            uint4 bf[9];
            w3_static_for<0, 3>([&](auto bc) {
                constexpr int B0 = decltype(bc)::value * 3;
                w3_static_for<B0, B0 + 3>([&](auto uc) {
                    constexpr int U = decltype(uc)::value, R = U / 3, S = U % 3;
                    constexpr int OFF = G::blk_rows(BLK, R) * 128, BS = CP ? U : S;
                    bf[U] = w3_join(w3_read_tr<OFF>(b0[BS]), w3_read_tr<OFF>(b1[BS]));
                });
                w3_wait_lgkmcnt<0>();
#pragma unroll
                for (int u = B0; u < B0 + 3; ++u)
#pragma unroll
                    for (int i = 0; i < FIW; ++i) acc[u][i] = mma_chunk<bf16_tag>(af[i], bf[u], acc[u][i]);
            });
        });
        if constexpr (CHAIN) {
            if (step % spc == spc - 1) {
                float sq = 0.f;
#pragma unroll
                for (int u = 0; u < 9; ++u)
#pragma unroll
                    for (int i = 0; i < FIW; ++i)
#pragma unroll
                        for (int q = 0; q < 4; ++q) {
                            sq = fmaf(acc[u][i][q], acc[u][i][q], sq);
                            tot[u][i][q] += acc[u][i][q];
                            acc[u][i][q] = 0.f;
                        }
#pragma unroll
                for (int off = 32; off > 0; off >>= 1) sq += __shfl_xor(sq, off);
                if (lane == 0) p.sq_part[((long long)(group + (step / spc) * p.n_chains) * tiles + tile) * 8 + wave] = sq;
            }
        }
        w3_wait_vmcnt<0>();
        __builtin_amdgcn_s_barrier();
    }

    float* out = CHAIN ? p.out + ((long long)group * p.Cd) * 9 * p.Cs : p.out + group * p.group_stride + ((long long)split * p.Cd) * 9 * p.Cs;
    const __amdgpu_buffer_rsrc_t rsrcO = __builtin_amdgcn_make_buffer_rsrc((void*)out, 0, p.Cd * 9 * p.Cs * 4, 0x00020000);
    const int voffO = (((tile_m * 64 + coh * 32 + (lane >> 4) * 4) * 9) * p.Cs + tile_n * 64 + cib * 16 + (lane & 15)) * 4;
    const int row4 = p.Cs * 4;
#pragma unroll
    for (int u = 0; u < 9; ++u)
#pragma unroll
        for (int i = 0; i < FIW; ++i)
#pragma unroll
            for (int q = 0; q < 4; ++q)
                __builtin_amdgcn_raw_buffer_store_b32(__float_as_uint(CHAIN ? tot[u][i][q] : acc[u][i][q]), rsrcO, voffO, ((i * 16 + q) * 9 + u) * row4, 0);
#endif
}

int fb_try_wgrad3x3_v2(const fb_wgrad_args* a, hipStream_t st) {
    static const bool disabled = getenv("FB_DISABLE_WGRAD3_V2") != nullptr;
    if (disabled || a->dtype != FB_BF16) return 0;
    if (a->R != 3 || a->S != 3 || a->pad != 1 || (a->stride != 1 && a->stride != 2)) return 0;
    const int SD = a->stride;
    if (a->Hs != SD * a->Hd || a->Ws != SD * a->Wd || a->Hd != a->Wd) return 0;
    const int W = a->Wd;
    const bool general = SD == 1 && (W == 56 || W == 28 || W == 14);
    if (W != 32 && W != 16 && W != 8 && W != 4 && !general) return 0;
    if (SD == 2 && W == 32) return 0;
    if (a->Cs % 64 != 0 || a->Cd % 64 != 0) return 0;
    int imgs_per_block = (a->imgs_per_group + a->split_k - 1) / a->split_k;
    const char* cp_env = getenv("FB_WGRAD3_COMPACT");
    const bool compact = W == 4 && SD == 1 && a->imgs_per_group % 4 == 0 && !(cp_env && atoi(cp_env) == 0);
    if (compact) imgs_per_block = (imgs_per_block + 3) / 4 * 4;
    else if (W == 4) { if (a->imgs_per_group & 1) return 0; imgs_per_block += imgs_per_block & 1; }
    const long long bytes_x = (long long)(imgs_per_block + 2) * a->Hs * a->Ws * a->Cs * 2, bytes_dy = (long long)(imgs_per_block + 2) * a->Hd * a->Wd * a->Cd * 2;
    if (bytes_x >= (1LL << 31) || bytes_dy >= (1LL << 31)) return 0;
    Wgrad3V2Params p;
    p.x = (const char*)a->x; p.dy = (const char*)a->dy; p.out = a->dw_partial;
    p.n_img = a->n_img; p.H = a->Hd; p.Cs = a->Cs; p.Cd = a->Cd;
    p.imgs_per_group = a->imgs_per_group; p.split_k = a->split_k; p.imgs_per_block = imgs_per_block;
    p.group_stride = a->group_stride ? a->group_stride : (long long)a->split_k * a->Cd * 9 * a->Cs;
    p.n_chains = 0; p.sq_part = nullptr;
    const int n_groups = a->n_img / a->imgs_per_group;
    dim3 grid((a->Cd / 64) * (a->Cs / 64) * n_groups * a->split_k);
    if (SD == 1) {
        if (W == 56) hipLaunchKernelGGL((conv_wgrad3x3_v2_kernel<56, 1>), grid, dim3(256), 0, st, p);
        else if (W == 28) hipLaunchKernelGGL((conv_wgrad3x3_v2_kernel<28, 1>), grid, dim3(256), 0, st, p);
        else if (W == 14) hipLaunchKernelGGL((conv_wgrad3x3_v2_kernel<14, 1>), grid, dim3(256), 0, st, p);
        else if (W == 32) hipLaunchKernelGGL((conv_wgrad3x3_v2_kernel<32, 1>), grid, dim3(256), 0, st, p);
        else if (W == 16) hipLaunchKernelGGL((conv_wgrad3x3_v2_kernel<16, 1>), grid, dim3(256), 0, st, p);
        else if (W == 8) hipLaunchKernelGGL((conv_wgrad3x3_v2_kernel<8, 1>), grid, dim3(256), 0, st, p);
        else if (compact) hipLaunchKernelGGL((conv_wgrad3x3_v2_kernel<4, 1, true>), grid, dim3(256), 0, st, p);
        else hipLaunchKernelGGL((conv_wgrad3x3_v2_kernel<4, 1>), grid, dim3(256), 0, st, p);
    } else {
        if (W == 16) hipLaunchKernelGGL((conv_wgrad3x3_v2_kernel<16, 2>), grid, dim3(256), 0, st, p);
        else if (W == 8) hipLaunchKernelGGL((conv_wgrad3x3_v2_kernel<8, 2>), grid, dim3(256), 0, st, p);
        else hipLaunchKernelGGL((conv_wgrad3x3_v2_kernel<4, 2>), grid, dim3(256), 0, st, p);
    }
    return 1;
}

static bool w3_chain_ok(const fb_wgrad_args* a) {
    static const bool disabled = getenv("FB_DISABLE_WGRAD3_CHAIN") != nullptr;
    if (disabled || !a || a->dtype != FB_BF16) return false;
    if (a->R != 3 || a->S != 3 || a->pad != 1 || a->stride != 1) return false;
    if (a->Hd != 4 || a->Wd != 4 || a->Hs != 4 || a->Ws != 4) return false;
    if (a->Cs % 64 != 0 || a->Cd % 64 != 0 || a->imgs_per_group < 4 || a->imgs_per_group % 4 != 0 || a->n_img % a->imgs_per_group != 0) return false;
    if (a->bn_x || a->amax_x || a->amax_dy) return false;
    if ((long long)a->n_img * 16 * a->Cs * 2 >= (1LL << 31) || (long long)a->n_img * 16 * a->Cd * 2 >= (1LL << 31)) return false;
    return true;
}

extern "C" int32_t fb_wgrad_chain_supported(const fb_wgrad_args* a) { return w3_chain_ok(a) ? 1 : 0; }

extern "C" int fb_conv2d_wgrad_chain(const fb_wgrad_args* a, int32_t n_chains, float* slabs, float* sq_part, void* stream) {
    if (!a || !a->x || !a->dy || !slabs || !sq_part) FB_FAIL(FB_ERR_ARG, "fb_conv2d_wgrad_chain: null pointer");
    if (!w3_chain_ok(a)) FB_FAIL(FB_ERR_UNSUPPORTED, "fb_conv2d_wgrad_chain: bf16 3x3 / stride 1 / pad 1 weight gradients on 4x4 maps, channels in multiples of 64, chunks of 4k images");
    const int n_chunks = a->n_img / a->imgs_per_group;
    if (n_chains < 1 || n_chains > n_chunks) FB_FAIL(FB_ERR_ARG, "fb_conv2d_wgrad_chain: n_chains=%d for %d chunks", n_chains, n_chunks);
    Wgrad3V2Params p;
    p.x = (const char*)a->x; p.dy = (const char*)a->dy; p.out = slabs;
    p.n_img = a->n_img; p.H = a->Hd; p.Cs = a->Cs; p.Cd = a->Cd;
    p.imgs_per_group = a->imgs_per_group; p.split_k = 1; p.imgs_per_block = a->imgs_per_group;
    p.group_stride = 0; p.n_chains = n_chains; p.sq_part = sq_part;
    dim3 grid((a->Cd / 64) * (a->Cs / 64) * n_chains);
    hipLaunchKernelGGL((conv_wgrad3x3_v2_kernel<4, 1, true, true>), grid, dim3(512), 0, (hipStream_t)stream, p);
    FB_CHECK_LAUNCH("fb_conv2d_wgrad_chain");
    return FB_OK;
}
```

fullbatchtraining_amd/csrc/runtime.cpp:

```cpp
#include <stdlib.h>
#include <vector>

#include "common.h"
#include "profile.h"
#include "conv_params.h"

thread_local char fb_err_buf[512] = "";
extern "C" const char* fb_last_error_string(void) { return fb_err_buf; }
extern "C" int fb_abi_version(void) { return 13; }

extern "C" int64_t fb_ws_conv_stat_floats(const fb_conv_args* a) {
    return a ? 2 * (((int64_t)a->n_img * a->Hd * a->Wd + 127) / 128) * a->Cd : 0;
}
extern "C" int64_t fb_ws_wgrad_slab_floats(const fb_wgrad_args* a) {
    if (!a || a->imgs_per_group <= 0) return 0;
    return (int64_t)(a->n_img / a->imgs_per_group) * a->split_k * a->Cd * a->R * a->S * a->Cs;
}
extern "C" int64_t fb_ws_bn_partial_floats(int64_t n_pixels, int32_t C) { return 2 * ((n_pixels + 127) / 128) * C; }
extern "C" int64_t fb_ws_mt_floats(int32_t n_groups) { return (int64_t)(n_groups > 2 ? n_groups : 2) * FB_MT_BLOCKS; }

bool fb_experimental() {
    static const bool on = getenv("FB_EXPERIMENTAL") != nullptr && atoi(getenv("FB_EXPERIMENTAL")) != 0;
    return on;
}
static const char* fb_exp_getenv(const char* name) { return fb_experimental() ? getenv(name) : nullptr; }
const char* fb_getenv_experimental(const char* name) { return fb_exp_getenv(name); }
int fb_persistent_cus() {
    static int per_dev[64] = {0};
    int dev = 0;
    if (hipGetDevice(&dev) != hipSuccess || dev < 0 || dev >= 64) dev = 0;
    int n = per_dev[dev];
    if (n == 0) {
        int cus = 0;
        if (hipDeviceGetAttribute(&cus, hipDeviceAttributeMultiprocessorCount, dev) != hipSuccess || cus <= 0) cus = 256;
        const char* r = getenv("FB_CU_RESERVE");
        const int reserve = r ? atoi(r) : 0;
        n = cus - (reserve > 0 ? reserve : 0);
        if (n < 8) n = 8;
        per_dev[dev] = n;
    }
    return n;
}
// ... 80 lines not shown
```

fullbatchtraining_amd/engine.py:

```python
import math
import os
import time
import warnings

import torch

from . import lib
from .lib import call, _ptr

BN_EPS = 1e-5
BN_MOMENTUM = 0.1


def _round_up(x, m):
    return (x + m - 1) // m * m


class ConvBN:

    def __init__(self, conv_name, bn_name, cin_real, cout, k, stride, pad, hin, win, patches=False):
        self.conv_name, self.bn_name = conv_name, bn_name
        self.k_orig, self.stride_orig, self.pad_orig = k, stride, pad
        self.hout = (hin + 2 * pad - k) // stride + 1
        self.wout = (win + 2 * pad - k) // stride + 1
# ... 96 lines not shown
        self.feat, self.h_final = cin, h
        self.late_block = sum(len(stage) for stage in list(model.layers)[:-1])
        self.late_offset = self.offsets[f"layers.{len(model.layers) - 1}.0.conv1.weight"]
        self.layers = [self.stem] + [c for b in self.blocks for c in b.convs + ([b.shortcut] if b.shortcut else [])]
        order = {name: i for i, name in enumerate(self.param_names)}
        self.layers_by_param = sorted(self.layers, key=lambda L: order[f"{L.conv_name}.weight"])
        ch, wc = 0, 0
        for L in self.layers_by_param:
            L.w_off = self.offsets[f"{L.conv_name}.weight"]
            L.g_off = self.offsets[f"{L.bn_name}.weight"]
            L.b_off = self.offsets[f"{L.bn_name}.bias"]
            L.ch_off, L.wc_off = ch, wc
            ch += L.cout
            wc += L.wc_numel
        self.ch_total, self.wc_total = ch, _round_up(wc, 64)
        self.fcw_off, self.fcb_off = self.offsets["fc.weight"], self.offsets["fc.bias"]


def stem_patches(x_nchw, layer, dtype, aug=None, out=None):
    if x_nchw.device.type != "cuda":
        raise lib.EngineError("stem_patches: the patch gather runs on the GPU (no CPU path)")
    x = x_nchw.float().contiguous()
    n, c, h, w = x.shape
    if out is None:
        out = torch.empty(n, layer.hout, layer.wout, layer.cin_pad, device=x.device, dtype=dtype)
    oy = ox = fl = pv = None
    crop_pad = 0
    if aug is not None:
        oy, ox, fl, crop_pad, pad_value = aug
        pv = (lib.c_float * c)(*[float(v) for v in pad_value]) if pad_value is not None else None
    call("fb_stem_patches", x.data_ptr(), out.data_ptr(), n, c, h, w, layer.k_orig, layer.stride_orig, layer.pad_orig, layer.cin_pad,
         _ptr(oy), _ptr(ox), _ptr(fl), crop_pad, pv, lib.dtype_code(dtype))
    return out


class _Events:
    RING = 1024

    def __init__(self):
        self.ring, self.pos, self.free = [], 0, []

    def release(self, ids):
        self.free.extend(ids)

    def record(self, stream=None):
        if lib.recording():
            ev = self.free.pop() if self.free else lib.event_new()
            lib.current_recorder().events.append(ev)
        elif len(self.ring) < self.RING:
            ev = lib.event_new()
            self.ring.append(ev)
        else:
            ev = self.ring[self.pos]
            self.pos = (self.pos + 1) % self.RING
        lib.event_record(ev, stream)
        return ev

    def wait(self, ev, stream=None):
        lib.event_wait(ev, stream)


class _Pool:

    def __init__(self, device, dtype, on_reuse=None, events=None):
        self.device, self.dtype, self.free, self.on_reuse, self.events = device, dtype, {}, on_reuse, events

# ... 54 lines not shown
        self.w_dgrad = [torch.zeros(1, self.plan.wc_total, device=self.device, dtype=self.dt), None]
        if fd_sets:
            self.w_fwd[1] = torch.zeros(self.G, self.plan.wc_total, device=self.device, dtype=self.dt)
            self.w_dgrad[1] = torch.zeros(self.G, self.plan.wc_total, device=self.device, dtype=self.dt)
        self.n_passes = 1 + fd_sets
        self.mean_tab = torch.zeros(self.n_passes, self.G, self.plan.ch_total, **f32)
        self.var_tab = torch.zeros(self.n_passes, self.G, self.plan.ch_total, **f32)
        self._unbias_tabs = {}
        self.unbias = self._unbias_for(self.valid)
        self.f32_split = os.environ.get("FB_F32_SPLIT", f32_split or "bf16x6") if compute_dtype == torch.float32 else None
        if self.f32_split not in (None, "bf16x6", "f16x2"):
            raise lib.EngineError(f"fp32 arithmetic {self.f32_split!r}: bf16x6 or f16x2")
        self._alloc_activations()
        self.mt_ws = torch.zeros(lib.load().fb_ws_mt_floats(self.G), **f32)
        self.sq = torch.zeros(self.G, **f32)
        self.vnorm2 = torch.zeros(self.G, **f32)
        self.eps_n = torch.zeros(self.G, **f32)
        self.norms2 = torch.zeros(2, **f32)
        self.amax_blocks, self.amax_slots, self.amax_map, self.amax_handouts = [], {}, {}, 0
        for li, L in enumerate(self.plan.layers):
            L.li = li
        self.w_amax = [torch.zeros(len(self.plan.layers), self.G if k else 1, device=self.device, dtype=torch.float32) for k in range(2)]
        self.amax_ws = None
        if self.f32_split == "f16x2":
            n_max = self.G * chunk
            need = max(lib.load().fb_ws_bn_amax_floats(n_max * L.hout * L.wout, L.cout, chunk * L.hout * L.wout) for L in self.plan.layers)
            self.amax_ws = torch.zeros(int(need), device=self.device, dtype=torch.float32)
        self.events = _Events()
        self.pool = _Pool(self.device, self.dt, on_reuse=lambda t: self.amax_map.pop(t.data_ptr(), None), events=self.events)
        self.use_replay = os.environ.get("FB_REPLAY", "1") != "0"
        self.cmdlists, self.replays, self.MAX_CMDLISTS = {}, 0, int(os.environ.get("FB_MAX_CMDLISTS", "256"))
        self.cmd_evictions, self.record_new, self.unrecorded_runs, self._warned_record_off, self._off_misses = 0, True, 0, False, 0
        self.masks = {}
        exp = os.environ.get("FB_EXPERIMENTAL", "0") not in ("", "0")
        self.fuse_bwd_stat = exp and os.environ.get("FB_FUSED_BWD_STAT", "0") != "0"
        self.bst_done = False
        self.bn_fused = exp and os.environ.get("FB_BN_BWD_FUSED", "0") == "1"
        es = torch.empty((), dtype=self.dt).element_size()
        self.bnf_ws = torch.empty(max((self.G * chunk * L.hout * L.wout * L.cout * es // 16 // 4096 * 2 + 4 * self.G) * L.cout for L in self.plan.layers) + 64,
                                  device=self.device, dtype=torch.float32)
        self.bnf_sync = torch.zeros(int(lib.load().fb_ws_bn_bwd_fused_ints(self.G)), device=self.device, dtype=torch.int32)
        sw = os.environ.get("FB_WGRAD_STREAM")
        self.wstream = torch.cuda.Stream(device=self.device) if sw != "0" else None
        self.stream_autotune = sw not in ("0", "1") and any(L.R == 1 and L.cin_pad >= 512 for L in self.plan.layers)
        self.stream_times = None
        self._wgrad_event = None
        self.label_smoothing, self.only_incorrect = 0.0, False
        self.load_from_model(model)

    def _unbias_for(self, batch):
        tab = self._unbias_tabs.get(batch)
        if tab is None:
            unbias = torch.ones(self.plan.ch_total)
            for L in self.plan.layers:
                m = batch * L.hout * L.wout
                unbias[L.ch_off:L.ch_off + L.cout] = m / (m - 1)
            tab = self._unbias_tabs[batch] = unbias.to(self.device)
        return tab

    def _alloc_activations(self):
        n, dev, dt = self.G * self.chunk, self.device, self.dt
        f32 = dict(device=dev, dtype=torch.float32)
        max_part, max_slab = 0, 0
        for L in self.plan.layers:
            L.x = torch.empty(n, L.hout, L.wout, L.cout, device=dev, dtype=dt)
            L.scale = torch.empty(self.G, L.cout, **f32)
# ... 8 lines not shown
            max_slab = max(max_slab, handle.fb_ws_wgrad_slab_floats(lib.C.byref(lib.WgradArgs(
                n_img=n, imgs_per_group=self.chunk, split_k=L.split_k, Cd=L.cout, R=L.R, S=L.S, Cs=L.cin_pad))))
        self.stat_ws = torch.empty(max_part, **f32)
        self.slab_ws = torch.empty(max_slab, **f32)
        self.chain_layers, self.chain_on = [], False
        if dt == torch.bfloat16 and os.environ.get("FB_WGRAD_CHAIN", "0") == "1" and os.environ.get("FB_EXPERIMENTAL", "0") not in ("", "0"):
            for L in self.plan.layers:
                a = lib.WgradArgs(None, None, None, n, L.hin, L.win, L.cin_pad, L.hout, L.wout, L.cout, L.R, L.S, L.stride, L.pad, self.chunk, 1, self.dtc, 0)
                if (len(self.chain_layers) < 4 and L.split_k == 1 and L.cin_pad == L.cin_real and L.w_off % 4 == 0
                        and bool(lib.load().fb_wgrad_chain_supported(lib.C.byref(a)))):
                    L.chain_tiles = (L.cout // 64) * (L.cin_pad // 64)
                    L.n_chains = int(os.environ.get("FB_WGRAD_CHAINS", "0")) or max(1, 512 // L.chain_tiles)
                    L.chain_sq = torch.zeros(self.G, L.chain_tiles * 8, **f32)
                    self.chain_layers.append(L)
        if self.chain_layers:
            self.chain_ws = torch.empty(max(min(L.n_chains, self.G) * L.cout * L.taps * L.cin_pad for L in self.chain_layers), **f32)
            self.gsum = torch.zeros(self.plan.P, **f32)
            cuts, lo = [], 0
            for L in sorted(self.chain_layers, key=lambda l: l.w_off):
                if L.w_off > lo:
                    cuts.append((lo, L.w_off))
                lo = L.w_off + L.cout * L.taps * L.cin_real
            if lo < self.plan.P:
                cuts.append((lo, self.plan.P))
            assert all(a % 4 == 0 for a, _ in cuts), cuts
            self.plain_segments = cuts
            self.sq_seg = torch.zeros(2, self.G, **f32)
        self.stem_out = torch.empty(n, self.plan.stem.hout, self.plan.stem.wout, 64, device=dev, dtype=dt)
        if self.plan.stem_pool:
            hp = (self.plan.stem.hout + 1) // 2
            self.stem_pooled = torch.empty(n, hp, hp, 64, device=dev, dtype=dt)
            self.stem_pool_idx = torch.empty(n, hp, hp, 64, device=dev, dtype=torch.uint8) if os.environ.get("FB_MAXPOOL_IDX", "1") != "0" else None
        for b in self.plan.blocks:
            b.mids = [torch.empty_like(c.x) for c in b.convs[:-1]]
            b.out = torch.empty_like(b.convs[-1].x)
            b.pooled = None
            if b.shortcut is not None and b.stride == 2:
                b.pooled = torch.empty(n, b.hin // 2, b.win // 2, b.cin, device=dev, dtype=dt)
        self.feat = torch.empty(n, self.plan.feat, **f32)
        self.logits = torch.empty(n, self.plan.classes, **f32)
        self.dlogits = torch.empty(n, self.plan.classes, **f32)
        self.loss = torch.zeros(self.G, **f32)
        self.correct = torch.zeros(self.G, **f32)

    def _choose_split(self, L):
        bf16 = self.dt == torch.bfloat16
        G = self.nominal_group
        widths = ((4, 8, 16, 32) + ((14, 28, 56) if bf16 else ())) if L.stride == 1 else ((4, 8, 16) if (bf16 or self.f32_split == "f16x2") else ())
        if (L.R == 3 and L.stride in (1, 2) and L.pad == 1 and L.hout == L.wout and L.hin == L.stride * L.hout and L.wout in widths
                and L.cin_pad % 64 == 0 and L.cout % 64 == 0 and not (L.wout == 4 and self.chunk % 2)):
            tiles = (L.cout // 64) * (L.cin_pad // 64)
            slots = 256 if (L.stride == 2 and L.wout == 4) else 512
            unit = 2 if L.wout == 4 else 1
            return max(1, min(slots // (tiles * G), self.chunk // (2 * unit)))
        big = L.cin_pad % 128 == 0 and L.cout % 128 == 0 and (L.cin_pad >= 256 or L.cout >= 256 or L.R == 3)
        tile = 128 if big else 64
        tiles = (L.cout // tile) * max(L.cin_pad // tile, 1) * L.taps
        px = self.chunk * L.hout * L.wout
        kstep = (32 if self.dt == torch.float32 else 64) if big else 128
        want = max(1, 1024 // max(tiles * G, 1))
        if L is self.plan.stem and L.cin_pad % 64 != 0 and len(self._stem_ranges(G)) > 1:
            per_range = self._stem_ranges(G)[0][1]
            tiles = (L.cout // 64) * (1 if (bf16 and L.cin_pad % 160 == 0) else L.cin_pad // 32)
            want = max(1, 512 // max(tiles * per_range, 1))
        split = max(1, min(want, px // (kstep * 4)))
        while split > 1 and (split - 1) * (_round_up(-(-px // split), kstep)) >= px:
            split -= 1
# ... 116 lines not shown
        if hit is not None and hit[1] == numel:
            return hit[0]
        slot = self._amax_slot(t, numel)
        call("fb_absmax", t.data_ptr(), numel // G, G, numel // G, 1, slot)
        return slot

    def _amax_slot(self, t, numel):
        key = t.data_ptr()
        self.amax_handouts += 1
        slot = self.amax_slots.get(key)
        if slot is None:
            idx = len(self.amax_slots)
            if idx >= self.AMAX_SLOT_LIMIT:
                raise lib.EngineError(f"fp16x2 scale slots: more than {self.AMAX_SLOT_LIMIT} distinct operand buffers -- buffers are expected to be "
                                      "persistent (activations, pool, dataset slices); something allocates a new tensor per launch")
            blk, row = divmod(idx, self.AMAX_BLOCK)
            if blk == len(self.amax_blocks):
                self.amax_blocks.append(torch.zeros(self.AMAX_BLOCK, self.G, device=self.device, dtype=torch.float32))
            slot = self.amax_slots[key] = self.amax_blocks[blk][row].data_ptr()
        self.amax_map[key] = (slot, numel)
        return slot

    def _amax_pair(self, L, src, numel, wsets, G):
        if self.f32_split != "f16x2":
            return None, None
        return self._amax(src, numel, G), self.w_amax[1 if wsets > 1 else 0][L.li].data_ptr()

    def _stem_ranges(self, G):
        S = self.plan.stem
        per_chunk = self.chunk * S.hin * S.win * S.cin_pad * torch.empty((), dtype=self.dt).element_size()
        step = max(1, int(os.environ.get("FB_STEM_RANGE_BYTES", (1 << 31) - 1)) // per_chunk)
        return [(g0, min(step, G - g0)) for g0 in range(0, G, step)]

    def _conv_bn_fwd(self, L, src, G, wsets, theta, pidx):
        if L is self.plan.stem and len(self._stem_ranges(G)) > 1 and not getattr(self, "_in_stem_range", False):
            self._in_stem_range = True
            try:
                amax = self._amax_pair(L, src, G * self.chunk * L.hin * L.win * L.cin_pad, wsets, G)
                for g0, g_n in self._stem_ranges(G):
                    self._conv_bn_fwd_range(L, src, g0, g_n, wsets, theta, pidx, amax)
            finally:
                self._in_stem_range = False
            return
        self._conv_bn_fwd_range(L, src, 0, G, wsets, theta, pidx)

    def _conv_bn_fwd_range(self, L, src, g0, G, wsets, theta, pidx, amax=None):
        es = src.element_size()
        i0 = g0 * self.chunk
        src_ptr = src.data_ptr() + i0 * L.hin * L.win * L.cin_pad * es
        x_ptr = L.x.data_ptr() + i0 * L.hout * L.wout * L.cout * es
        n = G * self.chunk
        wf = self.w_fwd[1 if wsets > 1 else 0]
        wptr = wf.data_ptr() + wf.element_size() * L.wc_off
        evalm = getattr(self, "_eval", False)
        if amax is None:
            am_s, am_w = self._amax_pair(L, src, n * L.hin * L.win * L.cin_pad, wsets, G)
        else:
            am_s = amax[0] + 4 * g0 if amax[0] is not None else None
            am_w = (amax[1] + (4 * g0 if wsets > 1 else 0)) if amax[1] is not None else None
        if wsets > 1:
            wptr += g0 * self.plan.wc_total * wf.element_size()
        a = lib.ConvArgs(src_ptr, wptr, x_ptr, None, None if evalm else self.stat_ws.data_ptr(), n, L.hin, L.win, L.cin_pad, L.hout, L.wout,
                         L.cout, L.R, L.S, L.stride, L.pad, 0, self.chunk if wsets > 1 else n, self.plan.wc_total if wsets > 1 else 0,
                         0, self.dtc, None, None, None, am_s, am_w, self.chunk)
        call("fb_conv2d", lib.C.byref(a))
        if evalm:
            return
        px = n * L.hout * L.wout
        n_mblocks = (px + 127) // 128
        pstride = self.plan.P if wsets > 1 else 0
        tab_off = 4 * g0 * self.plan.ch_total
        th_off = 4 * g0 * pstride
        call("fb_bn_fwd_finalize", self.stat_ws.data_ptr(), n_mblocks, G, L.cout, float(self.valid * L.hout * L.wout),
             theta.data_ptr() + 4 * L.g_off + th_off, theta.data_ptr() + 4 * L.b_off + th_off, pstride, BN_EPS,
             self.mean_tab[pidx].data_ptr() + tab_off, self.var_tab[pidx].data_ptr() + tab_off, self.plan.ch_total, L.ch_off,
             L.scale.data_ptr() + 4 * g0 * L.cout, L.shift.data_ptr() + 4 * g0 * L.cout, L.invstd.data_ptr() + 4 * g0 * L.cout)

    def _bn_apply(self, L, out, G, relu=True, res=None, resL=None, pool=None):
        px = G * self.chunk * L.hout * L.wout
        ppg = self.chunk * L.hout * L.wout
        fused = pool is not None and bool(lib.load().fb_bn_apply_can_pool(L.cout, L.wout, ppg, self.dtc)) and os.environ.get("FB_FUSED_POOL", "1") != "0"
        call("fb_bn_apply", L.x.data_ptr(), out.data_ptr(), L.scale.data_ptr(), L.shift.data_ptr(), _ptr(res),
             resL.scale.data_ptr() if resL is not None else None, resL.shift.data_ptr() if resL is not None else None,
             px, L.cout, ppg, self.valid * L.hout * L.wout if self.valid < self.chunk else 0, 1 if relu else 0,
             _ptr(self._mask_of(out)) if relu else None, _ptr(pool) if fused else None, L.wout, self.dtc,
             *((self._amax_slot(out, px * L.cout), self.amax_ws.data_ptr()) if self.f32_split == "f16x2" else (None, None)))
        return fused

    def _mask_of(self, act):
        key = act.data_ptr()
        m = self.masks.get(key)
        if m is None:
            m = torch.empty(act.numel() * act.element_size() // 16, device=self.device, dtype=torch.uint8)
            self.masks[key] = m
        return m

    def _sl(self, t, G):
        return t[: G * self.chunk]

    def forward(self, patches, labels, G, wsets, theta, pidx):
        plan = self.plan
        self.amax_map.clear()
        self._conv_bn_fwd(plan.stem, patches, G, wsets, theta, pidx)
        self._bn_apply(plan.stem, self.stem_out, G)
        a = self.stem_out
        if plan.stem_pool:
            s = plan.stem
            if self.stem_pool_idx is not None and not getattr(self, "_eval", False):
                call("fb_maxpool3s2_fwd_idx", a.data_ptr(), self.stem_pooled.data_ptr(), self.stem_pool_idx.data_ptr(), G * self.chunk, s.hout, s.wout, 64, self.dtc)
            else:
                call("fb_maxpool3s2_fwd", a.data_ptr(), self.stem_pooled.data_ptr(), G * self.chunk, s.hout, s.wout, 64, self.dtc)
            a = self.stem_pooled
        pooled_ready = False
        for bi, b in enumerate(plan.blocks):
            nxt = plan.blocks[bi + 1] if bi + 1 < len(plan.blocks) else None
            next_pool = nxt.pooled if nxt is not None else None
            a0 = a
            cur = a0
            for i, L in enumerate(b.convs):
                self._conv_bn_fwd(L, cur, G, wsets, theta, pidx)
                if i < len(b.convs) - 1:
                    self._bn_apply(L, b.mids[i], G)
                    cur = b.mids[i]
            last = b.convs[-1]
            if b.shortcut is not None:
                src = a0
                if b.pooled is not None:
                    if not pooled_ready:
                        call("fb_avgpool2_fwd", a0.data_ptr(), b.pooled.data_ptr(), G * self.chunk, b.hin, b.win, b.cin, self.dtc)
                    src = b.pooled
                self._conv_bn_fwd(b.shortcut, src, G, wsets, theta, pidx)
                pooled_ready = self._bn_apply(last, b.out, G, res=b.shortcut.x, resL=b.shortcut, pool=next_pool)
            else:
                pooled_ready = self._bn_apply(last, b.out, G, res=a0, pool=next_pool)
            a = b.out
        n = G * self.chunk
        hw = plan.h_final * plan.h_final
        call("fb_head_pool", a.data_ptr(), self.feat.data_ptr(), n, hw, plan.feat, self.dtc)
        pstride = plan.P if wsets > 1 else 0
        call("fb_head_loss", self.feat.data_ptr(), theta.data_ptr() + 4 * plan.fcw_off, theta.data_ptr() + 4 * plan.fcb_off, pstride,
             labels.data_ptr(), self.logits.data_ptr(), self.dlogits.data_ptr(), self.loss.data_ptr(), self.correct.data_ptr(), G,
             self.chunk, plan.feat, plan.classes,
             0.0 if getattr(self, "_eval", False) else float(self.label_smoothing), 0 if getattr(self, "_eval", False) else int(self.only_incorrect))
        return a

    def _bn_bwd(self, L, dout, mask, G, gout, pidx, want_dy, reduced=False, apply=True):
        n = G * self.chunk
        px = n * L.hout * L.wout
        ppg = self.chunk * L.hout * L.wout
        bits = self.masks.get(mask.data_ptr()) if mask is not None else None
        y = None if bits is not None else mask
        dx = self.pool.get((n, L.hout, L.wout, L.cout)) if apply else None
        dy = self.pool.get((n, L.hout, L.wout, L.cout)) if want_dy else None
        if (apply and not reduced and y is None and self.bn_fused and self.f32_split != "f16x2"
                and lib.load().fb_bn_bwd_fused_supported(px, L.cout, ppg, self.dtc)):
            if int(lib.load().fb_ws_bn_bwd_fused_floats(px, L.cout, ppg, self.dtc)) > self.bnf_ws.numel():
                raise lib.EngineError("fb_bn_bwd_fused: partial-row scratch too small for this launch")
            call("fb_bn_bwd_fused", dout.data_ptr(), _ptr(bits), L.x.data_ptr(), self.mean_tab[pidx].data_ptr(), L.invstd.data_ptr(), L.scale.data_ptr(),
                 self.plan.ch_total, L.ch_off, gout.data_ptr() + 4 * L.g_off, gout.data_ptr() + 4 * L.b_off, self.plan.P, L.coef.data_ptr(),
                 dx.data_ptr(), _ptr(dy), px, L.cout, ppg, float(self.valid * L.hout * L.wout), self.dtc, self.bnf_ws.data_ptr(), self.bnf_sync.data_ptr())
            return dx, dy
        if reduced:
            n_mblocks = px // 128
        else:
            n_mblocks = lib.load().fb_bn_bwd_reduce_rows(px, ppg)
            call("fb_bn_bwd_reduce", dout.data_ptr(), _ptr(y), _ptr(bits), L.x.data_ptr(), self.mean_tab[pidx].data_ptr(), L.invstd.data_ptr(),
                 self.plan.ch_total, L.ch_off, self.stat_ws.data_ptr(), px, L.cout, ppg, self.dtc)
        call("fb_bn_bwd_finalize", self.stat_ws.data_ptr(), n_mblocks, G, L.cout, float(self.valid * L.hout * L.wout), L.scale.data_ptr(),
             self.mean_tab[pidx].data_ptr(), L.invstd.data_ptr(), self.plan.ch_total, L.ch_off,
             gout.data_ptr() + 4 * L.g_off, gout.data_ptr() + 4 * L.b_off, self.plan.P, L.coef.data_ptr(), 1 if reduced else 0)
        if not apply:
            return None, None
        call("fb_bn_bwd_apply", dout.data_ptr(), _ptr(y), _ptr(bits), L.x.data_ptr(), L.coef.data_ptr(), dx.data_ptr(), _ptr(dy), px, L.cout, ppg,
             self.dtc, *((self._amax_slot(dx, px * L.cout), self.amax_ws.data_ptr()) if self.f32_split == "f16x2" else (None, None)))
        return dx, dy

    def _bn_bwd2(self, La, Lb, dout, mask, G, gout, pidx):
        n = G * self.chunk
        px, ppg = n * La.hout * La.wout, self.chunk * La.hout * La.wout
        bits = self.masks[mask.data_ptr()]
        rows = lib.load().fb_bn_bwd_reduce_rows(px, ppg)
        half = 2 * rows * La.cout
        pa, pb = self.stat_ws.data_ptr(), self.stat_ws.data_ptr() + 4 * half
        call("fb_bn_bwd_reduce2", dout.data_ptr(), bits.data_ptr(), La.x.data_ptr(), La.invstd.data_ptr(), La.ch_off, pa, Lb.x.data_ptr(), Lb.invstd.data_ptr(),
             Lb.ch_off, pb, self.mean_tab[pidx].data_ptr(), self.plan.ch_total, px, La.cout, ppg, self.dtc)
        for L, part in ((La, pa), (Lb, pb)):
            call("fb_bn_bwd_finalize", part, rows, G, L.cout, float(self.valid * L.hout * L.wout), L.scale.data_ptr(), self.mean_tab[pidx].data_ptr(),
                 L.invstd.data_ptr(), self.plan.ch_total, L.ch_off, gout.data_ptr() + 4 * L.g_off, gout.data_ptr() + 4 * L.b_off, self.plan.P, L.coef.data_ptr(), 0)
        dxa, dxb = self.pool.get((n, La.hout, La.wout, La.cout)), self.pool.get((n, La.hout, La.wout, La.cout))
        call("fb_bn_bwd_apply2", dout.data_ptr(), bits.data_ptr(), La.x.data_ptr(), La.coef.data_ptr(), dxa.data_ptr(), Lb.x.data_ptr(), Lb.coef.data_ptr(),
             dxb.data_ptr(), px, La.cout, ppg, self.dtc)
        return dxa, dxb

    def _bn_bwd2_ok(self, La, Lb, G):
        if os.environ.get("FB_BN_BWD_DUAL", "1") == "0" or self.f32_split == "f16x2" or La.cout != Lb.cout or (La.hout, La.wout) != (Lb.hout, Lb.wout):
            return False
        vec = 16 // torch.empty((), dtype=self.dt).element_size()
        n = G * self.chunk
        rows = lib.load().fb_bn_bwd_reduce_rows(n * La.hout * La.wout, self.chunk * La.hout * La.wout)
        return La.cout % vec == 0 and 256 % (La.cout // vec) == 0 and 4 * rows * La.cout <= self.stat_ws.numel()

    def _wgrad_bn_ok(self, L, mask):
        if os.environ.get("FB_WGRAD_BNF", "1") == "0" or self.f32_split == "f16x2" or self.masks.get(mask.data_ptr()) is None:
            return False
        a = lib.WgradArgs(None, None, None, self.chunk, L.hin, L.win, L.cin_pad, L.hout, L.wout, L.cout, L.R, L.S, L.stride, L.pad, self.chunk, 1, self.dtc, 0)
        return bool(lib.load().fb_wgrad_bn_fused_supported(lib.C.byref(a)))

    def _wgrad(self, L, src, dx, G, gout, bn=None):
        n = G * self.chunk
        if bn is not None:
            dx = bn[0]
        if self.chain_on and bn is None and any(L is c for c in self.chain_layers):
            S = min(L.n_chains, G)
            a = lib.WgradArgs(src.data_ptr(), dx.data_ptr(), None, n, L.hin, L.win, L.cin_pad, L.hout, L.wout, L.cout, L.R, L.S, L.stride, L.pad,
                              self.chunk, 1, self.dtc, 0)

            def launch_chain():
                call("fb_conv2d_wgrad_chain", lib.C.byref(a), S, self.chain_ws.data_ptr(), L.chain_sq.data_ptr())
                call("fb_wgrad_reduce", self.chain_ws.data_ptr(), self.gsum.data_ptr() + 4 * L.w_off, 0, 1, S, L.cout, L.taps, L.cin_pad, L.cin_real)

            if self.wstream is None:
                launch_chain()
                return
            ready = self.events.record()
            with torch.cuda.stream(self.wstream):
                self.events.wait(ready)
                launch_chain()
                self._wgrad_event = self.events.record()
            return
        direct = L.split_k == 1 and L.cin_pad == L.cin_real
        am_x = am_dy = None
        if self.f32_split == "f16x2":
            am_x, am_dy = self._amax(src, n * L.hin * L.win * L.cin_pad, G), self._amax(dx, n * L.hout * L.wout * L.cout, G)
        ranges = self._stem_ranges(G) if L is self.plan.stem else [(0, G)]
        es = src.element_size()
        args = []
        for g0, g_n in ranges:
            i0 = g0 * self.chunk
            args.append((g0, g_n, lib.WgradArgs(src.data_ptr() + i0 * L.hin * L.win * L.cin_pad * es, dx.data_ptr() + i0 * L.hout * L.wout * L.cout * es,
                                                gout.data_ptr() + 4 * (L.w_off + g0 * self.plan.P) if direct else self.slab_ws.data_ptr(), g_n * self.chunk,
                                                L.hin, L.win, L.cin_pad, L.hout, L.wout, L.cout, L.R, L.S, L.stride, L.pad, self.chunk, L.split_k, self.dtc,
                                                self.plan.P if direct else 0, am_x + 4 * g0 if am_x is not None else None,
                                                am_dy + 4 * g0 if am_dy is not None else None,
                                                *((L.x.data_ptr() + i0 * L.hout * L.wout * L.cout * es, self.masks[bn[1].data_ptr()].data_ptr() + i0 * L.hout * L.wout * L.cout * es // 16,
                                                   L.coef.data_ptr() + 4 * g0 * L.cout * 3) if bn is not None else (None, None, None)))))

        def launch():
            for g0, g_n, a in args:
                call("fb_conv2d_wgrad", lib.C.byref(a))
                if not direct:
                    call("fb_wgrad_reduce", self.slab_ws.data_ptr(), gout.data_ptr() + 4 * (L.w_off + g0 * self.plan.P), self.plan.P, g_n, L.split_k, L.cout,
                         L.taps, L.cin_pad, L.cin_real)

        if self.wstream is None:
            launch()
            return
        ready = self.events.record()
        with torch.cuda.stream(self.wstream):
            self.events.wait(ready)
            launch()
            self._wgrad_event = self.events.record()

    def _dgrad_args(self, L, src, wptr, dst, addend, G, wsets, addend_mode, addend_mask=None, stat=None, bst_x=None, bst_mask=None, amax=(None, None)):
        n = G * self.chunk
        return lib.ConvArgs(src, wptr, dst, addend, stat, n, L.hout, L.wout, L.cout, L.hin, L.win, L.cin_pad,
                            L.R, L.S, L.stride, L.pad, 1, self.chunk if wsets > 1 else n, self.plan.wc_total if wsets > 1 else 0,
                            addend_mode, self.dtc, addend_mask, bst_x, bst_mask, amax[0], amax[1], self.chunk)

    def _dgrad(self, L, dx, G, wsets, addend=None, addend_mode=0, addend_mask=None, bst=None):
        n = G * self.chunk
        out = self.pool.get((n, L.hin, L.win, L.cin_pad))
        wd = self.w_dgrad[1 if wsets > 1 else 0]
        wptr = wd.data_ptr() + wd.element_size() * L.wc_off
        self.bst_done = False
        a = None
        if bst is not None and self.fuse_bwd_stat:
            bits = self.masks.get(bst[1].data_ptr())
            if bits is not None and bst[0].cout == L.cin_pad:
# ... 12 lines not shown
        one = self.theta.data_ptr()
        a = self._dgrad_args(L, one, one, one, one, G, wsets, 1, one)
        return bool(lib.load().fb_conv_masked_addend_supported(lib.C.byref(a)))

    def backward(self, patches, G, wsets, theta, gout, pidx, on_block_done=None):
        plan, pool = self.plan, self.pool
        n = G * self.chunk
        hw = plan.h_final * plan.h_final
        pstride = plan.P if wsets > 1 else 0
        d = pool.get((n, plan.h_final, plan.h_final, plan.feat))
        call("fb_head_bwd", self.feat.data_ptr(), self.dlogits.data_ptr(), theta.data_ptr() + 4 * plan.fcw_off, pstride,
             gout.data_ptr() + 4 * plan.fcw_off, gout.data_ptr() + 4 * plan.fcb_off, plan.P, d.data_ptr(), G, self.chunk, hw, plan.feat,
             plan.classes, self.dtc)
        d_reduced = False
        for bi in range(len(plan.blocks) - 1, -1, -1):
            b = plan.blocks[bi]
            a0 = plan.blocks[bi - 1].out if bi > 0 else (self.stem_pooled if plan.stem_pool else self.stem_out)
            last = b.convs[-1]
            first = b.convs[0]
            out_bits = self.masks.get(b.out.data_ptr())
            lazy = out_bits is not None and (b.shortcut is not None or self._masked_addend_ok(first, G, wsets))
            dxs_early = None
            if lazy and b.shortcut is not None and not d_reduced and self._bn_bwd2_ok(last, b.shortcut, G):
                dx, dxs_early = self._bn_bwd2(last, b.shortcut, d, b.out, G, gout, pidx)
                dy = None
            else:
                dx, dy = self._bn_bwd(last, d, b.out, G, gout, pidx, want_dy=not lazy, reduced=d_reduced)
            if bi > 0:
                consumer = (plan.blocks[bi - 1].convs[-1], plan.blocks[bi - 1].out)
            else:
                consumer = None if plan.stem_pool else (plan.stem, self.stem_out)
            if not lazy:
                pool.put(d)
            srcs = [a0] + b.mids
            cur_dx = dx
            for i in range(len(b.convs) - 1, -1, -1):
                L = b.convs[i]
                self._wgrad(L, srcs[i], cur_dx, G, gout)
                ev_cur = self._wgrad_event
                if i > 0:
                    d_mid = self._dgrad(L, cur_dx, G, wsets, bst=(b.convs[i - 1], b.mids[i - 1]))
                    pool.put(cur_dx, event=ev_cur)
                    cur_dx, _ = self._bn_bwd(b.convs[i - 1], d_mid, b.mids[i - 1], G, gout, pidx, want_dy=False, reduced=self.bst_done)
                    pool.put(d_mid)
            if b.shortcut is not None:
                S = b.shortcut
                if dxs_early is not None:
                    dxs = dxs_early
                else:
                    dxs, _ = self._bn_bwd(S, d, b.out, G, gout, pidx, want_dy=False) if lazy else self._bn_bwd(S, dy, None, G, gout, pidx, want_dy=False)
                src = b.pooled if b.pooled is not None else a0
                self._wgrad(S, src, dxs, G, gout)
                d_p = self._dgrad(S, dxs, G, wsets)
                pool.put(dxs, event=self._wgrad_event)
                d_in = self._dgrad(first, cur_dx, G, wsets, addend=d_p, addend_mode=2 if b.pooled is not None else 1, bst=consumer)
                pool.put(d_p)
            elif lazy:
                d_in = self._dgrad(first, cur_dx, G, wsets, addend=d, addend_mode=1, addend_mask=out_bits, bst=consumer)
            else:
                d_in = self._dgrad(first, cur_dx, G, wsets, addend=dy, addend_mode=1, bst=consumer)
            d_reduced = self.bst_done
            pool.put(cur_dx, event=ev_cur)
            pool.put(d if lazy else dy)
            d = d_in
            if on_block_done is not None:
                on_block_done(bi)
        S = plan.stem
        if plan.stem_pool:
            d_r = pool.get((n, S.hout, S.wout, 64))
            if self.stem_pool_idx is not None:
                call("fb_maxpool3s2_bwd_idx", self.stem_pool_idx.data_ptr(), d.data_ptr(), d_r.data_ptr(), n, S.hout, S.wout, 64, self.dtc)
            else:
                call("fb_maxpool3s2_bwd", self.stem_out.data_ptr(), d.data_ptr(), d_r.data_ptr(), n, S.hout, S.wout, 64, self.dtc)
            pool.put(d)
            d = d_r
        if self._wgrad_bn_ok(S, self.stem_out) and not (d_reduced and not plan.stem_pool):
# ... 351 lines not shown
```

fullbatchtraining_amd/lib.py:

```python
import ctypes as C
import os
import struct

import torch

FB_F32, FB_BF16 = 0, 1
EXPECTED_ABI = 13
MT_BLOCKS = 1024
_LIB_PATH = os.environ.get("FB_LIB_PATH") or os.path.join(os.path.dirname(os.path.abspath(__file__)), "csrc", "libfbengine.so")

c_void_p, c_int, c_i64, c_float, c_double = C.c_void_p, C.c_int32, C.c_int64, C.c_float, C.c_double


class ConvArgs(C.Structure):
    _fields_ = [("src", c_void_p), ("wgt", c_void_p), ("dst", c_void_p), ("addend", c_void_p), ("stat_partial", c_void_p),
                ("n_img", c_int), ("Hs", c_int), ("Ws", c_int), ("Cs", c_int), ("Hd", c_int), ("Wd", c_int), ("Cd", c_int),
                ("R", c_int), ("S", c_int), ("stride", c_int), ("pad", c_int), ("mode", c_int),
                ("imgs_per_wset", c_int), ("wset_stride", c_i64), ("addend_mode", c_int), ("dtype", c_int), ("addend_mask", c_void_p),
                ("bst_x", c_void_p), ("bst_mask", c_void_p), ("amax_src", c_void_p), ("amax_wgt", c_void_p), ("amax_imgs", c_int)]


class WgradArgs(C.Structure):
    _fields_ = [("x", c_void_p), ("dy", c_void_p), ("dw_partial", c_void_p),
                ("n_img", c_int), ("Hs", c_int), ("Ws", c_int), ("Cs", c_int), ("Hd", c_int), ("Wd", c_int), ("Cd", c_int),
                ("R", c_int), ("S", c_int), ("stride", c_int), ("pad", c_int),
                ("imgs_per_group", c_int), ("split_k", c_int), ("dtype", c_int), ("group_stride", c_i64), ("amax_x", c_void_p), ("amax_dy", c_void_p),
                ("bn_x", c_void_p), ("bn_mask", c_void_p), ("bn_coef", c_void_p)]


_SIGS = {
    "fb_conv2d": [C.POINTER(ConvArgs), c_void_p],
    "fb_conv2d_wgrad": [C.POINTER(WgradArgs), c_void_p],
    "fb_absmax": [c_void_p, c_i64, c_int, c_i64, c_int, c_void_p, c_void_p],
    "fb_wgrad_reduce": [c_void_p, c_void_p, c_i64, c_int, c_int, c_int, c_int, c_int, c_int, c_void_p],
    "fb_weight_prep": [c_void_p, c_i64, c_i64, c_int, c_int, c_int, c_int, c_int, c_void_p, c_void_p, c_int, c_void_p, c_void_p],
    "fb_bn_fwd_finalize": [c_void_p, c_int, c_int, c_int, c_double, c_void_p, c_void_p, c_i64, c_float, c_void_p, c_void_p, c_int,
                           c_int, c_void_p, c_void_p, c_void_p, c_void_p],
    "fb_bn_apply": [c_void_p, c_void_p, c_void_p, c_void_p, c_void_p, c_void_p, c_void_p, c_i64, c_int, c_i64, c_i64, c_int, c_void_p, c_void_p, c_int,
                    c_int, c_void_p, c_void_p, c_void_p],
    "fb_bn_running_update": [c_void_p, c_void_p, c_void_p, c_void_p, c_int, c_i64, c_void_p, c_int, c_int, c_float, c_void_p],
    "fb_bn_bwd_reduce": [c_void_p, c_void_p, c_void_p, c_void_p, c_void_p, c_void_p, c_int, c_int, c_void_p, c_i64, c_int, c_i64, c_int, c_void_p],
    "fb_bn_bwd_finalize": [c_void_p, c_int, c_int, c_int, c_double, c_void_p, c_void_p, c_void_p, c_int, c_int, c_void_p, c_void_p,
                           c_i64, c_void_p, c_int, c_void_p],
    "fb_bn_bwd_apply": [c_void_p, c_void_p, c_void_p, c_void_p, c_void_p, c_void_p, c_void_p, c_i64, c_int, c_i64, c_int, c_void_p, c_void_p, c_void_p],
    "fb_bn_bwd_reduce2": [c_void_p, c_void_p, c_void_p, c_void_p, c_int, c_void_p, c_void_p, c_void_p, c_int, c_void_p, c_void_p, c_int, c_i64, c_int, c_i64, c_int,
                          c_void_p],
    "fb_bn_bwd_apply2": [c_void_p, c_void_p, c_void_p, c_void_p, c_void_p, c_void_p, c_void_p, c_void_p, c_i64, c_int, c_i64, c_int, c_void_p],
    "fb_bn_bwd_fused": [c_void_p, c_void_p, c_void_p, c_void_p, c_void_p, c_void_p, c_int, c_int, c_void_p, c_void_p, c_i64, c_void_p, c_void_p, c_void_p,
                        c_i64, c_int, c_i64, c_double, c_int, c_void_p, c_void_p, c_void_p],
    "fb_stem_patches": [c_void_p, c_void_p, c_i64, c_int, c_int, c_int, c_int, c_int, c_int, c_int, c_void_p, c_void_p, c_void_p, c_int,
                        C.POINTER(c_float), c_int, c_void_p],
    "fb_avgpool2_fwd": [c_void_p, c_void_p, c_int, c_int, c_int, c_int, c_int, c_void_p],
    "fb_maxpool3s2_fwd": [c_void_p, c_void_p, c_int, c_int, c_int, c_int, c_int, c_void_p],
    "fb_maxpool3s2_bwd": [c_void_p, c_void_p, c_void_p, c_int, c_int, c_int, c_int, c_int, c_void_p],
    "fb_maxpool3s2_fwd_idx": [c_void_p, c_void_p, c_void_p, c_int, c_int, c_int, c_int, c_int, c_void_p],
    "fb_maxpool3s2_bwd_idx": [c_void_p, c_void_p, c_void_p, c_int, c_int, c_int, c_int, c_int, c_void_p],
    "fb_head_pool": [c_void_p, c_void_p, c_int, c_int, c_int, c_int, c_void_p],
    "fb_head_loss": [c_void_p, c_void_p, c_void_p, c_i64, c_void_p, c_void_p, c_void_p, c_void_p, c_void_p, c_int, c_int, c_int, c_int,
                     c_float, c_int, c_void_p],
    "fb_head_bwd": [c_void_p, c_void_p, c_void_p, c_i64, c_void_p, c_void_p, c_i64, c_void_p, c_int, c_int, c_int, c_int, c_int, c_int,
                    c_void_p],
    "fb_mt_sqnorm": [c_void_p, c_i64, c_int, c_i64, c_float, c_void_p, c_float, c_void_p, c_void_p, c_void_p],
    "fb_mt_accumulate": [c_void_p, c_void_p, c_i64, c_int, c_i64, c_int, c_void_p, c_void_p, c_void_p],
    "fb_mt_fd_perturb": [c_void_p, c_void_p, c_i64, c_int, c_i64, c_float, c_float, c_float, c_void_p, c_void_p, c_void_p, c_float, c_void_p,
                         c_void_p],
    "fb_mt_fd_combine_accumulate": [c_void_p, c_void_p, c_void_p, c_void_p, c_i64, c_int, c_i64, c_void_p, c_float, c_int, c_void_p],
    "fb_mt_fd_combine": [c_void_p, c_void_p, c_void_p, c_i64, c_int, c_i64, c_void_p, c_float, c_void_p],
    "fb_mt_chunk_clip": [c_void_p, c_i64, c_int, c_i64, c_void_p, c_float, c_void_p, c_void_p],
    "fb_bn_eval_coeffs": [c_void_p, c_void_p, c_void_p, c_void_p, c_float, c_void_p, c_void_p, c_int, c_void_p],
    "fb_head_tta": [c_void_p, c_void_p, c_void_p, c_int, c_int, c_void_p, c_void_p, c_void_p, c_void_p],
    "fb_mt_norms2": [c_void_p, c_void_p, c_i64, c_void_p, c_void_p, c_void_p],
    "fb_mt_clip_sgd": [c_void_p, c_void_p, c_void_p, c_i64, c_void_p, c_float, c_float, c_float, c_float, c_float, c_int, c_int, c_void_p],
    "fb_mt_scale": [c_void_p, c_i64, c_float, c_void_p],
    "fb_mt_sam_ascent": [c_void_p, c_void_p, c_void_p, c_i64, c_void_p, c_float, c_float, c_void_p],
    "fb_mt_sam_restore": [c_void_p, c_void_p, c_i64, c_void_p],
    "fb_mt_absmax2": [c_void_p, c_i64, c_void_p, c_void_p, c_void_p],
    "fb_mt_pnorm2": [c_void_p, c_i64, c_float, c_void_p, c_void_p, c_void_p],
    "fb_mt_norm_bias": [c_void_p, c_void_p, c_i64, c_void_p, c_float, c_float, c_int, c_void_p],
    "fb_mt_ema": [c_void_p, c_void_p, c_i64, c_float, c_float, c_void_p],
    "fb_mt_clip_scale": [c_void_p, c_i64, c_void_p, c_float, c_void_p],
    "fb_mt_grad_noise": [c_void_p, c_void_p, c_i64, c_float, c_int, c_void_p],
    "fb_conv2d_wgrad_chain": [C.POINTER(WgradArgs), c_int, c_void_p, c_void_p, c_void_p],
    "fb_mt_accumulate_sum": [c_void_p, c_void_p, c_i64, c_int, c_int, c_void_p],
    "fb_mt_accumulate_skip": [c_void_p, c_void_p, c_i64, c_int, c_i64, c_int, c_void_p, c_void_p] + [c_i64] * 8 + [c_void_p],
}
EXPORTS = tuple(_SIGS) + ("fb_last_error_string", "fb_abi_version", "fb_profile_enable", "fb_profile_read", "fb_ws_conv_stat_floats",
                          "fb_ws_wgrad_slab_floats", "fb_ws_bn_partial_floats", "fb_ws_mt_floats", "fb_bn_bwd_reduce_rows", "fb_conv_masked_addend_supported", "fb_conv_bwd_stat_supported",
                          "fb_bn_apply_can_pool", "fb_ws_bn_amax_floats", "fb_profile_read_launches", "fb_cmd_fn_id", "fb_cmd_fn_nargs", "fb_event_new", "fb_event_count", "fb_bn_bwd_fused_supported", "fb_ws_bn_bwd_fused_floats", "fb_ws_bn_bwd_fused_ints", "fb_wgrad_bn_fused_supported", "fb_wgrad_chain_supported",
                          "fb_event_record", "fb_event_wait", "fb_cmdlist_create", "fb_cmdlist_destroy", "fb_cmdlist_size", "fb_cmdlist_add_call",
                          "fb_cmdlist_add_event", "fb_cmdlist_replay")
PROF_CLASSES = ("igemm_fwd", "igemm_dgrad", "wgrad", "bn_apply", "bn_bwd_reduce", "bn_bwd_apply", "bn_bwd_fused")
PROF_INFO = 11
PROF_KERNELS = {0: "?", 1: "conv_igemm_kernel (register-staged)", 2: "conv_igemm_v3_kernel", 3: "conv3x3s1_halo4_kernel", 4: "conv3x3s1_c64_halo5_kernel",
                5: "conv3x3s2_dgrad_quad_kernel", 6: "conv1x1_k32_kernel", 7: "conv1x1_stream_kernel", 8: "conv3x3s2_fwd_kernel", 9: "conv1x1_pipe_kernel", 10: "conv1x1_gemm_kernel",
                16: "conv_wgrad_kernel", 17: "conv_wgrad3x3_kernel", 18: "conv_wgrad3x3_v2_kernel", 19: "conv_wgrad1x1_kernel"}


def profile_enable(on, capacity=32768):
    lib = load()
    lib.fb_profile_enable.argtypes, lib.fb_profile_enable.restype = [c_int, c_int], c_int
    if lib.fb_profile_enable(1 if on else 0, capacity) != 0:
        raise EngineError(lib.fb_last_error_string().decode())


def profile_read():
    lib = load()
    lib.fb_profile_read.argtypes = [C.POINTER(c_double), C.POINTER(c_i64), C.POINTER(c_i64)]
    k = len(PROF_CLASSES)
    ms, n, d = (c_double * k)(), (c_i64 * k)(), (c_i64 * k)()
    if lib.fb_profile_read(ms, n, d) != 0:
        raise EngineError(lib.fb_last_error_string().decode())
    return {k: (ms[i], n[i], d[i]) for i, k in enumerate(PROF_CLASSES)}



def profile_read_launches(cap=1 << 18):
    lib = load()
    lib.fb_profile_read_launches.argtypes, lib.fb_profile_read_launches.restype = [C.POINTER(c_int), C.POINTER(c_float), c_i64], c_i64
    info, ms = (c_int * (cap * (PROF_INFO + 1)))(), (c_float * cap)()
    n = lib.fb_profile_read_launches(info, ms, cap)
    if n < 0:
# ... 8 lines not shown
class EngineError(RuntimeError):
    pass


def load():
    global _lib
    if _lib is None:
        if not os.path.isfile(_LIB_PATH):
            raise EngineError(f"{_LIB_PATH} is missing: run `python -m fullbatchtraining_amd.build` (needs hipcc). "
                              "The engine has no CPU or PyTorch fallback.")
        lib = C.CDLL(_LIB_PATH)
        for name, sig in _SIGS.items():
            fn = getattr(lib, name)
            fn.argtypes, fn.restype = sig, c_int
        lib.fb_last_error_string.restype = C.c_char_p
        lib.fb_abi_version.restype = c_int
        if lib.fb_abi_version() != EXPECTED_ABI:
            raise EngineError(f"{_LIB_PATH} has ABI version {lib.fb_abi_version()}, this package expects {EXPECTED_ABI}: rebuild it with "
                              "`python -m fullbatchtraining_amd.build --force`")
        lib.fb_ws_conv_stat_floats.argtypes, lib.fb_ws_conv_stat_floats.restype = [C.POINTER(ConvArgs)], c_i64
        lib.fb_ws_wgrad_slab_floats.argtypes, lib.fb_ws_wgrad_slab_floats.restype = [C.POINTER(WgradArgs)], c_i64
        lib.fb_ws_bn_partial_floats.argtypes, lib.fb_ws_bn_partial_floats.restype = [c_i64, c_int], c_i64
        lib.fb_ws_mt_floats.argtypes, lib.fb_ws_mt_floats.restype = [c_int], c_i64
        lib.fb_bn_bwd_reduce_rows.argtypes, lib.fb_bn_bwd_reduce_rows.restype = [c_i64, c_i64], c_int
        lib.fb_conv_masked_addend_supported.argtypes, lib.fb_conv_masked_addend_supported.restype = [C.POINTER(ConvArgs)], c_int
        lib.fb_conv_bwd_stat_supported.argtypes, lib.fb_conv_bwd_stat_supported.restype = [C.POINTER(ConvArgs)], c_int
        lib.fb_ws_bn_amax_floats.argtypes, lib.fb_ws_bn_amax_floats.restype = [c_i64, c_int, c_i64], c_i64
        lib.fb_bn_apply_can_pool.argtypes, lib.fb_bn_apply_can_pool.restype = [c_int, c_int, c_i64, c_int], c_int
        lib.fb_bn_bwd_fused_supported.argtypes, lib.fb_bn_bwd_fused_supported.restype = [c_i64, c_int, c_i64, c_int], c_int
        lib.fb_ws_bn_bwd_fused_floats.argtypes, lib.fb_ws_bn_bwd_fused_floats.restype = [c_i64, c_int, c_i64, c_int], c_i64
        lib.fb_ws_bn_bwd_fused_ints.argtypes, lib.fb_ws_bn_bwd_fused_ints.restype = [c_i64], c_i64
        lib.fb_wgrad_bn_fused_supported.argtypes, lib.fb_wgrad_bn_fused_supported.restype = [C.POINTER(WgradArgs)], c_int
        lib.fb_wgrad_chain_supported.argtypes, lib.fb_wgrad_chain_supported.restype = [C.POINTER(WgradArgs)], c_int
        lib.fb_cmd_fn_id.argtypes, lib.fb_cmd_fn_id.restype = [C.c_char_p], c_int
        lib.fb_cmd_fn_nargs.argtypes, lib.fb_cmd_fn_nargs.restype = [c_int], c_int
        lib.fb_event_new.argtypes, lib.fb_event_new.restype = [], c_int
        lib.fb_event_count.argtypes, lib.fb_event_count.restype = [], c_int
        lib.fb_event_record.argtypes, lib.fb_event_record.restype = [c_int, c_void_p], c_int
        lib.fb_event_wait.argtypes, lib.fb_event_wait.restype = [c_int, c_void_p], c_int
        lib.fb_cmdlist_create.argtypes, lib.fb_cmdlist_create.restype = [], c_void_p
        lib.fb_cmdlist_destroy.argtypes, lib.fb_cmdlist_destroy.restype = [c_void_p], None
        lib.fb_cmdlist_size.argtypes, lib.fb_cmdlist_size.restype = [c_void_p], c_i64
        lib.fb_cmdlist_add_call.argtypes, lib.fb_cmdlist_add_call.restype = [c_void_p, c_int, C.POINTER(C.c_uint64), c_int, c_int, c_void_p, c_int], c_int
        lib.fb_cmdlist_add_event.argtypes, lib.fb_cmdlist_add_event.restype = [c_void_p, c_int, c_int, c_int], c_int
        lib.fb_cmdlist_replay.argtypes, lib.fb_cmdlist_replay.restype = [c_void_p, C.POINTER(c_void_p), c_int], c_int
        _lib = lib
    return _lib


def _ptr(t):
    if t is None:
        return None
    if isinstance(t, int):
        return t
    return t.data_ptr()


def _stream():
    return torch.cuda.current_stream().cuda_stream


def call(name, *args):
    lib = load()
    st = _stream()
    status = getattr(lib, name)(*args, st)
    if status != 0:
# ... 181 lines not shown
```

include/fb_engine.h:

```cpp
#ifndef FB_ENGINE_H
#define FB_ENGINE_H

#include <stddef.h>
#include <stdint.h>

#ifdef __cplusplus
extern "C" {
#endif

typedef enum { FB_OK = 0, FB_ERR_ARG = -1, FB_ERR_SHAPE = -2, FB_ERR_LAUNCH = -3, FB_ERR_UNSUPPORTED = -4 } fb_status;
typedef enum { FB_F32 = 0, FB_BF16 = 1 } fb_dtype;

const char* fb_last_error_string(void);
int fb_abi_version(void);

int fb_profile_enable(int on, int capacity);
int fb_profile_read(double* ms, int64_t* launches, int64_t* dropped);
int64_t fb_profile_read_launches(int32_t* info, float* ms, int64_t cap);

int32_t fb_cmd_fn_id(const char* name);
int32_t fb_cmd_fn_nargs(int32_t fn);
int32_t fb_event_new(void);
int32_t fb_event_count(void);
int fb_event_record(int32_t ev, void* stream);
int fb_event_wait(int32_t ev, void* stream);
void* fb_cmdlist_create(void);
void fb_cmdlist_destroy(void* list);
int64_t fb_cmdlist_size(const void* list);
int fb_cmdlist_add_call(void* list, int32_t fn, const uint64_t* words, int32_t n_words, int32_t stream_idx, const void* blob, int32_t blob_bytes);
int fb_cmdlist_add_event(void* list, int32_t kind, int32_t ev, int32_t stream_idx);
int fb_cmdlist_replay(const void* list, void* const* streams, int32_t n_streams);

typedef struct {
    const void* src; const void* wgt; void* dst; const void* addend; float* stat_partial;
    int32_t n_img, Hs, Ws, Cs, Hd, Wd, Cd;
    int32_t R, S, stride, pad, mode;
    int32_t imgs_per_wset; int64_t wset_stride;
    int32_t addend_mode; int32_t dtype;
    const void* addend_mask;
    const void* bst_x; const void* bst_mask;
    const float* amax_src; const float* amax_wgt;
    int32_t amax_imgs;
} fb_conv_args;
int fb_conv2d(const fb_conv_args* a, void* stream);
int32_t fb_conv_masked_addend_supported(const fb_conv_args* a);
int32_t fb_conv_bwd_stat_supported(const fb_conv_args* a);
int fb_absmax(const float* x, int64_t n, int32_t n_sets, int64_t set_stride, int32_t per_set, float* out, void* stream);

typedef struct {
    const void* x; const void* dy; float* dw_partial;
    int32_t n_img, Hs, Ws, Cs, Hd, Wd, Cd;
    int32_t R, S, stride, pad;
    int32_t imgs_per_group; int32_t split_k; int32_t dtype;
    int64_t group_stride;
    const float* amax_x; const float* amax_dy;
    const void* bn_x; const void* bn_mask; const float* bn_coef;
} fb_wgrad_args;
int32_t fb_wgrad_bn_fused_supported(const fb_wgrad_args* a);
int fb_conv2d_wgrad(const fb_wgrad_args* a, void* stream);
int32_t fb_wgrad_chain_supported(const fb_wgrad_args* a);
int fb_conv2d_wgrad_chain(const fb_wgrad_args* a, int32_t n_chains, float* slabs, float* sq_part, void* stream);

int64_t fb_ws_conv_stat_floats(const fb_conv_args* a);
int64_t fb_ws_wgrad_slab_floats(const fb_wgrad_args* a);
int64_t fb_ws_bn_partial_floats(int64_t n_pixels, int32_t C);
int64_t fb_ws_mt_floats(int32_t n_groups);
int fb_wgrad_reduce(const float* dw_partial, float* out, int64_t out_group_stride, int32_t n_groups, int32_t split_k,
                    int32_t Cd, int32_t taps, int32_t Cs_pad, int32_t Cs_real, void* stream);
int fb_weight_prep(const float* master, int64_t wset_stride_in, int64_t wset_stride_out, int32_t n_wsets, int32_t Cout, int32_t taps,
                   int32_t Cin_real, int32_t Cin_pad, void* w_fwd, void* w_dgrad, int32_t dtype, const float* amax, void* stream);

int fb_bn_fwd_finalize(const float* stat_partial, int32_t n_mblocks, int32_t n_groups, int32_t C, double count,
                       const float* gamma, const float* beta, int64_t param_group_stride, float eps,
                       float* mean_tab, float* var_tab, int32_t ch_total, int32_t ch_off,
                       float* scale, float* shift, float* invstd, void* stream);
int fb_bn_apply(const void* x, void* y, const float* scale, const float* shift, const void* res, const float* rscale,
                const float* rshift, int64_t n_pixels, int32_t C, int64_t pixels_per_group, int64_t valid_pixels_per_group,
                int32_t relu, void* mask_out, void* pool_out, int32_t pool_W, int32_t dtype, float* amax_out, float* amax_ws, void* stream);
int64_t fb_ws_bn_amax_floats(int64_t n_pixels, int32_t C, int64_t pixels_per_group);
int32_t fb_bn_apply_can_pool(int32_t C, int32_t W, int64_t pixels_per_group, int32_t dtype);
int fb_bn_running_update(float* running_mean, float* running_var, const float* mean_tab, const float* var_tab, int32_t n_passes,
                         int64_t pass_stride, const float* unbias, int32_t n_groups, int32_t ch_total, float momentum, void* stream);
int32_t fb_bn_bwd_reduce_rows(int64_t n_pixels, int64_t pixels_per_group);
int fb_bn_bwd_reduce(const void* dout, const void* y, const void* mask, const void* x, const float* mean_tab, const float* invstd,
                     int32_t ch_total, int32_t ch_off, float* partial, int64_t n_pixels, int32_t C,
                     int64_t pixels_per_group, int32_t dtype, void* stream);
int fb_bn_bwd_finalize(const float* partial, int32_t n_mblocks, int32_t n_groups, int32_t C, double count,
                       const float* scale, const float* mean_tab, const float* invstd, int32_t ch_total, int32_t ch_off,
                       float* dgamma, float* dbeta, int64_t grad_group_stride, float* coef, int32_t raw_x, void* stream);
int fb_bn_bwd_apply(const void* dout, const void* y, const void* mask, const void* x, const float* coef, void* dx, void* dy_out,
                    int64_t n_pixels, int32_t C, int64_t pixels_per_group, int32_t dtype, float* amax_out, float* amax_ws, void* stream);

int fb_bn_bwd_reduce2(const void* dout, const void* mask, const void* x_a, const float* invstd_a, int32_t ch_off_a, float* partial_a,
                      const void* x_b, const float* invstd_b, int32_t ch_off_b, float* partial_b, const float* mean_tab, int32_t ch_total,
                      int64_t n_pixels, int32_t C, int64_t pixels_per_group, int32_t dtype, void* stream);
int fb_bn_bwd_apply2(const void* dout, const void* mask, const void* x_a, const float* coef_a, void* dx_a, const void* x_b, const float* coef_b,
                     void* dx_b, int64_t n_pixels, int32_t C, int64_t pixels_per_group, int32_t dtype, void* stream);
int32_t fb_bn_bwd_fused_supported(int64_t n_pixels, int32_t C, int64_t pixels_per_group, int32_t dtype);
int64_t fb_ws_bn_bwd_fused_floats(int64_t n_pixels, int32_t C, int64_t pixels_per_group, int32_t dtype);
int64_t fb_ws_bn_bwd_fused_ints(int64_t n_groups);
int fb_bn_bwd_fused(const void* dout, const void* mask, const void* x, const float* mean_tab, const float* invstd, const float* scale,
                    int32_t ch_total, int32_t ch_off, float* dgamma, float* dbeta, int64_t grad_group_stride, float* coef, void* dx,
                    void* dy_out, int64_t n_pixels, int32_t C, int64_t pixels_per_group, double count, int32_t dtype, float* partial,
                    int32_t* sync, void* stream);

int fb_stem_patches(const float* images, void* patches, int64_t n_img, int32_t C, int32_t H, int32_t W, int32_t k, int32_t stride,
                    int32_t pad, int32_t cin_pad, const int8_t* crop_oy, const int8_t* crop_ox, const int8_t* flip, int32_t crop_pad,
                    const float* pad_value, int32_t dtype, void* stream);

int fb_avgpool2_fwd(const void* x, void* y, int32_t n_img, int32_t H, int32_t W, int32_t C, int32_t dtype, void* stream);
int fb_maxpool3s2_fwd(const void* x, void* y, int32_t n_img, int32_t H, int32_t W, int32_t C, int32_t dtype, void* stream);
int fb_maxpool3s2_bwd(const void* x, const void* dy, void* dx, int32_t n_img, int32_t H, int32_t W, int32_t C, int32_t dtype,
                      void* stream);
int fb_maxpool3s2_fwd_idx(const void* x, void* y, void* idx, int32_t n_img, int32_t H, int32_t W, int32_t C, int32_t dtype, void* stream);
int fb_maxpool3s2_bwd_idx(const void* idx, const void* dy, void* dx, int32_t n_img, int32_t H, int32_t W, int32_t C, int32_t dtype,
                          void* stream);
int fb_head_pool(const void* a, float* feat, int32_t n_img, int32_t HW, int32_t C, int32_t dtype, void* stream);
int fb_head_loss(const float* feat, const float* fc_w, const float* fc_b, int64_t param_group_stride, const int64_t* labels,
                 float* logits, float* dlogits, float* loss, float* correct, int32_t n_groups, int32_t imgs_per_group,
                 int32_t C, int32_t classes, float label_smoothing, int32_t only_incorrect, void* stream);
int fb_bn_eval_coeffs(const float* gamma, const float* beta, const float* running_mean, const float* running_var, float eps, float* scale,
                      float* shift, int32_t C, void* stream);
int fb_head_tta(const float* logits_a, const float* logits_b, const int64_t* labels, int32_t n, int32_t classes, float* ws ,
                float* loss_sum, float* correct, void* stream);
// ... 39 lines not shown
```

Baseline: 219,000.

## Fold BN-ReLU into the consuming conv and recompute activations from pre-BN input

Inside residual blocks, the BatchNorm scale/shift plus ReLU of an intermediate activation is folded into the next conv's input load, so the normalized mid tensor no longer has to be written. In backward, wgrad, the BN reduce and the BN apply kernels recompute the activation and its ReLU mask from the raw conv output using per-channel scale and shift. The aim is to cut memory traffic for storing and rereading mid activations and masks. In exchange, every consumer does extra arithmetic, several conv, wgrad and BN kernel paths become more complex, and a new ABI is required.

```diff
diff --git a/fullbatchtraining_amd/csrc/bn.hip b/fullbatchtraining_amd/csrc/bn.hip
--- a/fullbatchtraining_amd/csrc/bn.hip
+++ b/fullbatchtraining_amd/csrc/bn.hip
@@ -294,14 +294,16 @@
 }
 
 struct BnReduceB { const uint4* x; const float* invstd; float* partial; int ch_off; };
-template <typename T, bool DUAL = false>
+struct BnAx { const float* scale; const float* shift; long long valid_vec; };
+template <typename T, bool DUAL = false, bool AX = false>
 __global__ __launch_bounds__(256) void bn_bwd_reduce_kernel(const uint4* __restrict__ dout, const uint4* __restrict__ y,
                                                             const unsigned char* __restrict__ mask,
                                                             const uint4* __restrict__ x, const float* __restrict__ mean_tab,
                                                             const float* __restrict__ invstd, int ch_total, int ch_off,
                                                             float* __restrict__ partial, long long n_pixels, int C, long long ppg,
-                                                            int n_mblocks, int PB, const BnReduceB B) {
+                                                            int n_mblocks, int PB, const BnReduceB B, const BnAx A) {
     constexpr int V = ET<T>::VEC;
+    static_assert(!AX || (V == 8 && !DUAL), "the affine-of-x mask source is a bf16 form");
     extern __shared__ float sm[];
     const int cvec = C / V;
     const long long p0 = (long long)blockIdx.x * PB;
@@ -325,6 +327,12 @@
         float muB[DUAL ? V : 1], isB[DUAL ? V : 1], s2B[DUAL ? V : 1];
 #pragma unroll
         for (int k = 0; k < V; ++k) { mu[k] = mean_tab[g * ch_total + ch_off + c0 + k]; is[k] = invstd[g * C + c0 + k]; s1[k] = 0.f; s2[k] = 0.f; }
+        float asc[AX ? 8 : 1], ash[AX ? 8 : 1];
+        if constexpr (AX) { load_coef<8>(A.scale + g * C + c0, asc); load_coef<8>(A.shift + g * C + c0, ash); }
+        auto ax_mask = [&](const uint4& xr, long long i) -> unsigned {
+            if constexpr (AX) return i - g * ppg * cvec < A.valid_vec ? fb_bn_relu_mask8(xr, asc, ash) : 0u;
+            else return 0xffu;
+        };
         if constexpr (DUAL) {
 #pragma unroll
             for (int k = 0; k < V; ++k) { muB[k] = mean_tab[g * ch_total + B.ch_off + c0 + k]; isB[k] = B.invstd[g * C + c0 + k]; s2B[k] = 0.f; }
@@ -354,13 +362,18 @@
             unsigned mk[BN_SPAN_U];
 #pragma unroll
             for (int u = 0; u < BN_SPAN_U; ++u) {
-                dr[u] = ld_reduce(dout + i + u * 256); xr[u] = ld_reduce(x + i + u * 256); mk[u] = mask_at(i + u * 256);
+                dr[u] = ld_reduce(dout + i + u * 256); xr[u] = ld_reduce(x + i + u * 256);
+                if constexpr (AX) mk[u] = ax_mask(xr[u], i + u * 256); else mk[u] = mask_at(i + u * 256);
                 if constexpr (DUAL) xbr[u] = ld_reduce(B.x + i + u * 256); else xbr[u] = xr[u];
             }
 #pragma unroll
             for (int u = 0; u < BN_SPAN_U; ++u) one(dr[u], xr[u], xbr[u], mk[u]);
         }
-        for (; i < hi; i += 256) { if constexpr (DUAL) one(dout[i], x[i], B.x[i], mask_at(i)); else one(dout[i], x[i], x[i], mask_at(i)); }
+        for (; i < hi; i += 256) {
+            if constexpr (AX) { const uint4 xr = x[i]; one(dout[i], xr, xr, ax_mask(xr, i)); }
+            else if constexpr (DUAL) one(dout[i], x[i], B.x[i], mask_at(i));
+            else one(dout[i], x[i], x[i], mask_at(i));
+        }
 #pragma unroll
         for (int k = 0; k < V; ++k) { sm[(row * C + c0 + k) * 2] = s1[k]; sm[(row * C + c0 + k) * 2 + 1] = s2[k]; }
         if constexpr (DUAL) {
@@ -424,12 +437,33 @@
     const int prof = fb_prof_begin(FB_PROF_BN_BWD_REDUCE, (hipStream_t)stream, info);
     if (dtype == FB_F32)
         hipLaunchKernelGGL((bn_bwd_reduce_kernel<float>), dim3(n_mblocks), dim3(256), smem, (hipStream_t)stream, (const uint4*)dout, (const uint4*)y,
-                           (const unsigned char*)mask, (const uint4*)x, mean_tab, invstd, ch_total, ch_off, partial, (long long)n_pixels, C, (long long)pixels_per_group, n_mblocks, PB, BnReduceB{});
+                           (const unsigned char*)mask, (const uint4*)x, mean_tab, invstd, ch_total, ch_off, partial, (long long)n_pixels, C, (long long)pixels_per_group, n_mblocks, PB, BnReduceB{}, BnAx{});
     else
         hipLaunchKernelGGL((bn_bwd_reduce_kernel<bf16_tag>), dim3(n_mblocks), dim3(256), smem, (hipStream_t)stream, (const uint4*)dout, (const uint4*)y,
-                           (const unsigned char*)mask, (const uint4*)x, mean_tab, invstd, ch_total, ch_off, partial, (long long)n_pixels, C, (long long)pixels_per_group, n_mblocks, PB, BnReduceB{});
+                           (const unsigned char*)mask, (const uint4*)x, mean_tab, invstd, ch_total, ch_off, partial, (long long)n_pixels, C, (long long)pixels_per_group, n_mblocks, PB, BnReduceB{}, BnAx{});
     fb_prof_end(prof, (hipStream_t)stream);
     FB_CHECK_LAUNCH("fb_bn_bwd_reduce");
+    return FB_OK;
+}
+
+extern "C" int fb_bn_bwd_reduce_ax(const void* dout, const void* x, const float* scale, const float* shift, int64_t valid_pixels_per_group,
+                                   const float* mean_tab, const float* invstd, int32_t ch_total, int32_t ch_off, float* partial, int64_t n_pixels,
+                                   int32_t C, int64_t pixels_per_group, int32_t dtype, void* stream) {
+    if (!dout || !x || !scale || !shift || !mean_tab || !invstd || !partial) FB_FAIL(FB_ERR_ARG, "fb_bn_bwd_reduce_ax: null pointer");
+    if (pixels_per_group <= 0 || pixels_per_group % 128 != 0) FB_FAIL(FB_ERR_SHAPE, "fb_bn_bwd_reduce_ax: pixels_per_group=%lld must be a multiple of 128", (long long)pixels_per_group);
+    if (dtype != FB_BF16 || C % 8 != 0 || 256 % (C / 8) != 0) FB_FAIL(FB_ERR_UNSUPPORTED, "fb_bn_bwd_reduce_ax: bf16, channel vectors of a pixel dividing 256 (C=%d)", C);
+    const int cvec = C / 8, rows = 256 / cvec;
+    const int PB = bn_reduce_pixels(n_pixels, pixels_per_group);
+    const int n_mblocks = fb_bn_bwd_reduce_rows(n_pixels, pixels_per_group);
+    const size_t smem = (size_t)rows * C * 2 * sizeof(float);
+    const long long valid = valid_pixels_per_group > 0 && valid_pixels_per_group < pixels_per_group ? valid_pixels_per_group : pixels_per_group;
+    const int32_t info[FB_PROF_INFO] = {(int32_t)(n_pixels / 128), C, (int32_t)(pixels_per_group / 128), dtype, 0, 2 , 0, 0, 0, 0, 0};
+    const int prof = fb_prof_begin(FB_PROF_BN_BWD_REDUCE, (hipStream_t)stream, info);
+    hipLaunchKernelGGL((bn_bwd_reduce_kernel<bf16_tag, false, true>), dim3(n_mblocks), dim3(256), smem, (hipStream_t)stream, (const uint4*)dout, (const uint4*)nullptr,
+                       (const unsigned char*)nullptr, (const uint4*)x, mean_tab, invstd, ch_total, ch_off, partial, (long long)n_pixels, C, (long long)pixels_per_group, n_mblocks, PB,
+                       BnReduceB{}, BnAx{scale, shift, valid * cvec});
+    fb_prof_end(prof, (hipStream_t)stream);
+    FB_CHECK_LAUNCH("fb_bn_bwd_reduce_ax");
     return FB_OK;
 }
 
@@ -449,10 +483,10 @@
     const BnReduceB B{(const uint4*)x_b, invstd_b, partial_b, ch_off_b};
     if (dtype == FB_F32)
         hipLaunchKernelGGL((bn_bwd_reduce_kernel<float, true>), dim3(n_mblocks), dim3(256), smem, (hipStream_t)stream, (const uint4*)dout, (const uint4*)nullptr,
-                           (const unsigned char*)mask, (const uint4*)x_a, mean_tab, invstd_a, ch_total, ch_off_a, partial_a, (long long)n_pixels, C, (long long)pixels_per_group, n_mblocks, PB, B);
+                           (const unsigned char*)mask, (const uint4*)x_a, mean_tab, invstd_a, ch_total, ch_off_a, partial_a, (long long)n_pixels, C, (long long)pixels_per_group, n_mblocks, PB, B, BnAx{});
     else
         hipLaunchKernelGGL((bn_bwd_reduce_kernel<bf16_tag, true>), dim3(n_mblocks), dim3(256), smem, (hipStream_t)stream, (const uint4*)dout, (const uint4*)nullptr,
-                           (const unsigned char*)mask, (const uint4*)x_a, mean_tab, invstd_a, ch_total, ch_off_a, partial_a, (long long)n_pixels, C, (long long)pixels_per_group, n_mblocks, PB, B);
+                           (const unsigned char*)mask, (const uint4*)x_a, mean_tab, invstd_a, ch_total, ch_off_a, partial_a, (long long)n_pixels, C, (long long)pixels_per_group, n_mblocks, PB, B, BnAx{});
     fb_prof_end(prof, (hipStream_t)stream);
     FB_CHECK_LAUNCH("fb_bn_bwd_reduce2");
     return FB_OK;
@@ -519,13 +553,14 @@
 }
 
 struct BnApplyB { const uint4* x; const float* coef; uint4* dx; };
-template <typename T, bool DUAL = false>
+template <typename T, bool DUAL = false, bool AX = false>
 __global__ __launch_bounds__(256) void bn_bwd_apply_span_kernel(const uint4* __restrict__ dout, const uint4* __restrict__ y,
                                                                 const unsigned char* __restrict__ mask, const uint4* __restrict__ x,
                                                                 const float* __restrict__ coef, uint4* __restrict__ dx, uint4* __restrict__ dy_out,
                                                                 long long n_vec, int cvec, long long vec_per_group, int C, int span, float* __restrict__ amax,
-                                                                BnApplyB B) {
+                                                                BnApplyB B, const BnAx A) {
     constexpr int V = ET<T>::VEC;
+    static_assert(!AX || (V == 8 && !DUAL), "the affine-of-x mask source is a bf16 form");
     float am = 0.f;
     const long long g = blockIdx.y, base = g * vec_per_group;
     const long long lim = n_vec - base < vec_per_group ? n_vec - base : vec_per_group;
@@ -536,6 +571,12 @@
     load_coef<3 * V>(coef + (g * C + c0) * 3, cf);
     float cfB[DUAL ? 3 * V : 1];
     if constexpr (DUAL) { load_coef<3 * V>(B.coef + (g * C + c0) * 3, cfB); B.x += base; B.dx += base; }
+    float asc[AX ? 8 : 1], ash[AX ? 8 : 1];
+    if constexpr (AX) { load_coef<8>(A.scale + g * C + c0, asc); load_coef<8>(A.shift + g * C + c0, ash); }
+    auto ax_mask = [&](const uint4& xr, long long i) -> unsigned {
+        if constexpr (AX) return i < A.valid_vec ? fb_bn_relu_mask8(xr, asc, ash) : 0u;
+        else return 0xffu;
+    };
     dout += base; x += base; dx += base;
     if (mask) mask += base;
     if (y) y += base;
@@ -579,14 +620,38 @@
         unsigned mk[BN_SPAN_U];
 #pragma unroll
         for (int u = 0; u < BN_SPAN_U; ++u) {
-            dr[u] = ld_stream(dout + i + u * 256); xr[u] = ld_stream(x + i + u * 256); mk[u] = mask_at(i + u * 256);
+            dr[u] = ld_stream(dout + i + u * 256); xr[u] = ld_stream(x + i + u * 256);
+            if constexpr (AX) mk[u] = ax_mask(xr[u], i + u * 256); else mk[u] = mask_at(i + u * 256);
             if constexpr (DUAL) xbr[u] = ld_stream(B.x + i + u * 256); else xbr[u] = xr[u];
         }
 #pragma unroll
         for (int u = 0; u < BN_SPAN_U; ++u) one(dr[u], xr[u], xbr[u], mk[u], i + u * 256);
     }
-    for (; i < hi; i += 256) { if constexpr (DUAL) one(dout[i], x[i], B.x[i], mask_at(i), i); else one(dout[i], x[i], x[i], mask_at(i), i); }
+    for (; i < hi; i += 256) {
+        if constexpr (AX) { const uint4 xr = x[i]; one(dout[i], xr, xr, ax_mask(xr, i), i); }
+        else if constexpr (DUAL) one(dout[i], x[i], B.x[i], mask_at(i), i);
+        else one(dout[i], x[i], x[i], mask_at(i), i);
+    }
     if (amax) amax_commit(amax, am);
+}
+
+extern "C" int fb_bn_bwd_apply_ax(const void* dout, const void* x, const float* scale, const float* shift, int64_t valid_pixels_per_group,
+                                  const float* coef, void* dx, int64_t n_pixels, int32_t C, int64_t pixels_per_group, int32_t dtype, void* stream) {
+    if (!dout || !x || !scale || !shift || !coef || !dx) FB_FAIL(FB_ERR_ARG, "fb_bn_bwd_apply_ax: null pointer");
+    if (dtype != FB_BF16 || C % 8 != 0 || 256 % (C / 8) != 0 || pixels_per_group <= 0) FB_FAIL(FB_ERR_UNSUPPORTED, "fb_bn_bwd_apply_ax: bf16, channel vectors of a pixel dividing 256 (C=%d)", C);
+    const int cvec = C / 8;
+    const long long n_vec = n_pixels * cvec, vpg = pixels_per_group * cvec;
+    const long long valid = valid_pixels_per_group > 0 && valid_pixels_per_group < pixels_per_group ? valid_pixels_per_group : pixels_per_group;
+    const int32_t info[FB_PROF_INFO] = {(int32_t)(n_pixels / 128), C, (int32_t)(pixels_per_group / 128), dtype, 0, 2 , 0, 0, 0, 0, 0};
+    const int prof = fb_prof_begin(FB_PROF_BN_BWD_APPLY, (hipStream_t)stream, info);
+    const int span = bn_span(n_vec);
+    const dim3 grid((unsigned)((vpg + span - 1) / span), (unsigned)((n_vec + vpg - 1) / vpg));
+    hipLaunchKernelGGL((bn_bwd_apply_span_kernel<bf16_tag, false, true>), grid, dim3(256), 0, (hipStream_t)stream, (const uint4*)dout, (const uint4*)nullptr,
+                       (const unsigned char*)nullptr, (const uint4*)x, coef, (uint4*)dx, (uint4*)nullptr, n_vec, cvec, vpg, C, span, (float*)nullptr, BnApplyB{},
+                       BnAx{scale, shift, valid * cvec});
+    fb_prof_end(prof, (hipStream_t)stream);
+    FB_CHECK_LAUNCH("fb_bn_bwd_apply_ax");
+    return FB_OK;
 }
 
 extern "C" int fb_bn_bwd_apply(const void* dout, const void* y, const void* mask, const void* x, const float* coef, void* dx, void* dy_out,
@@ -604,10 +669,10 @@
         const dim3 grid((unsigned)((vpg + span - 1) / span), (unsigned)((n_vec + vpg - 1) / vpg));
         if (dtype == FB_F32)
             hipLaunchKernelGGL((bn_bwd_apply_span_kernel<float>), grid, dim3(256), 0, (hipStream_t)stream, (const uint4*)dout, (const uint4*)y,
-                               (const unsigned char*)mask, (const uint4*)x, coef, (uint4*)dx, (uint4*)dy_out, n_vec, cvec, vpg, C, span, amax_out ? amax_ws : nullptr, BnApplyB{});
+                               (const unsigned char*)mask, (const uint4*)x, coef, (uint4*)dx, (uint4*)dy_out, n_vec, cvec, vpg, C, span, amax_out ? amax_ws : nullptr, BnApplyB{}, BnAx{});
         else
             hipLaunchKernelGGL((bn_bwd_apply_span_kernel<bf16_tag>), grid, dim3(256), 0, (hipStream_t)stream, (const uint4*)dout, (const uint4*)y,
-                               (const unsigned char*)mask, (const uint4*)x, coef, (uint4*)dx, (uint4*)dy_out, n_vec, cvec, vpg, C, span, nullptr, BnApplyB{});
+                               (const unsigned char*)mask, (const uint4*)x, coef, (uint4*)dx, (uint4*)dy_out, n_vec, cvec, vpg, C, span, nullptr, BnApplyB{}, BnAx{});
         fb_prof_end(prof, (hipStream_t)stream);
         if (amax_out) hipLaunchKernelGGL(amax_finish_kernel, dim3(grid.y), dim3(256), 0, (hipStream_t)stream, amax_ws, (int)grid.x, amax_out);
         FB_CHECK_LAUNCH("fb_bn_bwd_apply");
@@ -640,10 +705,10 @@
     const BnApplyB B{(const uint4*)x_b, coef_b, (uint4*)dx_b};
     if (dtype == FB_F32)
         hipLaunchKernelGGL((bn_bwd_apply_span_kernel<float, true>), grid, dim3(256), 0, (hipStream_t)stream, (const uint4*)dout, (const uint4*)nullptr,
-                           (const unsigned char*)mask, (const uint4*)x_a, coef_a, (uint4*)dx_a, (uint4*)nullptr, n_vec, cvec, vpg, C, span, (float*)nullptr, B);
+                           (const unsigned char*)mask, (const uint4*)x_a, coef_a, (uint4*)dx_a, (uint4*)nullptr, n_vec, cvec, vpg, C, span, (float*)nullptr, B, BnAx{});
     else
         hipLaunchKernelGGL((bn_bwd_apply_span_kernel<bf16_tag, true>), grid, dim3(256), 0, (hipStream_t)stream, (const uint4*)dout, (const uint4*)nullptr,
-                           (const unsigned char*)mask, (const uint4*)x_a, coef_a, (uint4*)dx_a, (uint4*)nullptr, n_vec, cvec, vpg, C, span, (float*)nullptr, B);
+                           (const unsigned char*)mask, (const uint4*)x_a, coef_a, (uint4*)dx_a, (uint4*)nullptr, n_vec, cvec, vpg, C, span, (float*)nullptr, B, BnAx{});
     fb_prof_end(prof, (hipStream_t)stream);
     FB_CHECK_LAUNCH("fb_bn_bwd_apply2");
     return FB_OK;
diff --git a/fullbatchtraining_amd/csrc/cmdlist.cpp b/fullbatchtraining_amd/csrc/cmdlist.cpp
--- a/fullbatchtraining_amd/csrc/cmdlist.cpp
+++ b/fullbatchtraining_amd/csrc/cmdlist.cpp
@@ -37,7 +37,7 @@
     FB_ENTRY(fb_mt_accumulate), FB_ENTRY(fb_mt_fd_perturb), FB_ENTRY(fb_mt_fd_combine_accumulate), FB_ENTRY(fb_mt_fd_combine),
     FB_ENTRY(fb_mt_chunk_clip), FB_ENTRY(fb_bn_eval_coeffs), FB_ENTRY(fb_mt_norms2), FB_ENTRY(fb_mt_clip_sgd), FB_ENTRY(fb_mt_scale), FB_ENTRY(fb_bn_bwd_fused), FB_ENTRY(fb_bn_bwd_reduce2), FB_ENTRY(fb_bn_bwd_apply2),
     FB_ENTRY(fb_conv2d_wgrad_chain), FB_ENTRY(fb_mt_accumulate_sum), FB_ENTRY(fb_mt_accumulate_skip),
-    FB_ENTRY(fb_maxpool3s2_fwd_idx), FB_ENTRY(fb_maxpool3s2_bwd_idx),
+    FB_ENTRY(fb_maxpool3s2_fwd_idx), FB_ENTRY(fb_maxpool3s2_bwd_idx), FB_ENTRY(fb_bn_bwd_reduce_ax), FB_ENTRY(fb_bn_bwd_apply_ax),
 };
 constexpr int kNumEntries = sizeof(kEntries) / sizeof(kEntries[0]);
 
diff --git a/fullbatchtraining_amd/csrc/common.h b/fullbatchtraining_amd/csrc/common.h
--- a/fullbatchtraining_amd/csrc/common.h
+++ b/fullbatchtraining_amd/csrc/common.h
@@ -290,6 +290,28 @@
 
 __device__ __forceinline__ float fb_bn_dx(float c_dy, float c_x, float c_0, float dy, float x) { return fmaf(c_dy, dy, fmaf(c_x, x, c_0)); }
 
+__device__ __forceinline__ uint4 fb_bn_relu_bf16x8(const uint4& x, const float (&sc)[8], const float (&sh)[8], bool live) {
+    const unsigned w[4] = {x.x, x.y, x.z, x.w};
+    unsigned o[4];
+#pragma unroll
+    for (int i = 0; i < 4; ++i) {
+        const float a = fmaxf(fmaf(__uint_as_float(w[i] << 16), sc[2 * i], sh[2 * i]), 0.f);
+        const float b = fmaxf(fmaf(__uint_as_float(w[i] & 0xffff0000u), sc[2 * i + 1], sh[2 * i + 1]), 0.f);
+        o[i] = live ? pack_bf16x2(a, b) : 0u;
+    }
+    return make_uint4(o[0], o[1], o[2], o[3]);
+}
+__device__ __forceinline__ unsigned fb_bn_relu_mask8(const uint4& x, const float (&sc)[8], const float (&sh)[8]) {
+    const unsigned w[4] = {x.x, x.y, x.z, x.w};
+    unsigned m = 0;
+#pragma unroll
+    for (int i = 0; i < 4; ++i) {
+        m |= (fmaf(__uint_as_float(w[i] << 16), sc[2 * i], sh[2 * i]) > 0.f ? 1u : 0u) << (2 * i);
+        m |= (fmaf(__uint_as_float(w[i] & 0xffff0000u), sc[2 * i + 1], sh[2 * i + 1]) > 0.f ? 1u : 0u) << (2 * i + 1);
+    }
+    return m;
+}
+
 __device__ __forceinline__ float row16_sum(float v) {
     v += __builtin_bit_cast(float, __builtin_amdgcn_update_dpp(0, __builtin_bit_cast(int, v), 0x128, 0xf, 0xf, false));
     v += __builtin_bit_cast(float, __builtin_amdgcn_update_dpp(0, __builtin_bit_cast(int, v), 0x124, 0xf, 0xf, false));
diff --git a/fullbatchtraining_amd/csrc/conv3x3_halo5.hip b/fullbatchtraining_amd/csrc/conv3x3_halo5.hip
--- a/fullbatchtraining_amd/csrc/conv3x3_halo5.hip
+++ b/fullbatchtraining_amd/csrc/conv3x3_halo5.hip
@@ -7,6 +7,8 @@
     const unsigned char* addend_mask;
     const char* bst_x; const unsigned char* bst_mask;
     int n_img, mode, addend_mode, n_mblocks, n_tiles;
+    const float* in_scale; const float* in_shift;
+    int in_ipg, in_valid;
 #ifdef FB_H5_TRACE
     long long* trace;
 #endif
@@ -46,13 +48,15 @@
 #define FB_H5_ADD_DEPTH 3
 #endif
 constexpr int H5_AD = FB_H5_ADD_DEPTH, H5_ADN = H5_AD + 1;
-}
-
-template <int MODE, int ADD, int BST = 0>
+constexpr int H5_TAB = H5_WGT_BYTES + 2 * H5_HALO_BYTES + 1024;
+}
+
+template <int MODE, int ADD, int BST = 0, int FOLD = 0>
 __global__ __launch_bounds__(256) void conv3x3s1_c64_halo5_kernel(const Halo5Params p) {
 #if defined(__HIP_DEVICE_COMPILE__)
+    static_assert(!FOLD || (MODE == 0 && ADD == 0 && BST == 0), "the folded input transform is a forward variant");
     constexpr int W = H5_W, PITCH = H5_PITCH;
-    __shared__ __attribute__((aligned(16))) char lds[H5_WGT_BYTES + 2 * H5_HALO_BYTES + 1024];
+    __shared__ __attribute__((aligned(16))) char lds[H5_WGT_BYTES + 2 * H5_HALO_BYTES + 1024 + (FOLD ? 1024 : 0)];
 
     const int tid = threadIdx.x, lane = tid & 63;
     const int wave = __builtin_amdgcn_readfirstlane(tid >> 6);
@@ -113,6 +117,34 @@
         const unsigned v = (((dead >> K) & 1u) || !live) ? H5_OOB : voffH[K];
         const int dst = grp < H5_NGRP ? H5_WGT_BYTES + buf * H5_HALO_BYTES + grp * 1024 : H5_WGT_BYTES + 2 * H5_HALO_BYTES;
         __builtin_amdgcn_raw_ptr_buffer_load_lds(rA, (__attribute__((address_space(3))) void*)(lds + dst), 16, v, 0, 0, 0);
+    };
+
+    auto tab_issue = [&](int buf, int L) __attribute__((always_inline)) {
+        const int chunk = (L >> 2) / p.in_ipg;
+        const __amdgpu_buffer_rsrc_t rS = __builtin_amdgcn_make_buffer_rsrc((void*)(p.in_scale + (long long)chunk * 64), 0, 256, 0x00020000);
+        const __amdgpu_buffer_rsrc_t rT = __builtin_amdgcn_make_buffer_rsrc((void*)(p.in_shift + (long long)chunk * 64), 0, 256, 0x00020000);
+        __builtin_amdgcn_raw_ptr_buffer_load_lds(rS, (__attribute__((address_space(3))) void*)(lds + H5_TAB + buf * 512), 4, (unsigned)lane * 4, 0, 0, 0);
+        __builtin_amdgcn_raw_ptr_buffer_load_lds(rT, (__attribute__((address_space(3))) void*)(lds + H5_TAB + buf * 512 + 256), 4, (unsigned)lane * 4, 0, 0, 0);
+    };
+    auto halo_xform = [&](int buf, int L) __attribute__((always_inline)) {
+        const int n0 = L >> 2, y0 = (L & 3) * H5_TH;
+        const bool img_ok = n0 % p.in_ipg < p.in_valid;
+        const unsigned dead = (y0 == 0 ? topbits : 0u) | (y0 + H5_TH == W ? botbits : 0u);
+        const float* tab = (const float*)(lds + H5_TAB + buf * 512);
+        h5_static_for<0, H5_KH>([&](auto kc) __attribute__((always_inline)) {
+            constexpr int K = decltype(kc)::value;
+            const int grp = wave + 4 * K;
+            if (grp < H5_NGRP) {
+                const bool live = img_ok && voffH[K] != H5_OOB && !((dead >> K) & 1u);
+                const int c0 = (int)((voffH[K] >> 4) & 7u) * 8;
+                const float4 s0 = *(const float4*)(tab + c0), s1 = *(const float4*)(tab + c0 + 4);
+                const float4 t0 = *(const float4*)(tab + 64 + c0), t1 = *(const float4*)(tab + 64 + c0 + 4);
+                const float sc[8] = {s0.x, s0.y, s0.z, s0.w, s1.x, s1.y, s1.z, s1.w}, sh[8] = {t0.x, t0.y, t0.z, t0.w, t1.x, t1.y, t1.z, t1.w};
+                uint4* q = (uint4*)(lds + H5_WGT_BYTES + buf * H5_HALO_BYTES + grp * 1024 + lane * 16);
+                *q = fb_bn_relu_bf16x8(*q, sc, sh, live);
+            }
+            if constexpr (K % 3 == 2) __builtin_amdgcn_sched_barrier(0);
+        });
     };
 
     float ssum[2][4], ssq[2][4];
@@ -214,6 +246,7 @@
     int L = h5_xcd_remap(blockIdx.x, NB);
     if (L >= p.n_tiles) return;
     h5_static_for<0, H5_KH>([&](auto kc) { halo_piece(kc, 0, L, true); });
+    if constexpr (FOLD != 0) tab_issue(0, L);
 
     f32x4_t accA[2][8], accB[2][8];
 
@@ -224,6 +257,10 @@
         f32x4_t (&accp)[2][8] = BUF ? accA : accB;
         H5_STAMP(0);
         h5_wait_vmcnt<0>();
+        if constexpr (FOLD != 0) {
+            halo_xform(BUF, L);
+            __builtin_amdgcn_fence(__ATOMIC_RELEASE, "workgroup");
+        }
         __builtin_amdgcn_s_barrier();
         H5_STAMP(1);
 #pragma unroll
@@ -267,6 +304,7 @@
                 }
             }
             if constexpr (S < H5_KH) halo_piece(std::integral_constant<int, S>{}, BUF ^ 1, has_next ? L + NB : L, has_next);
+            if constexpr (FOLD != 0 && S == 0) tab_issue(BUF ^ 1, has_next ? L + NB : L);
         });
         H5_STAMP(3);
     };
@@ -303,7 +341,19 @@
     if (a->addend_mask && (!a->addend || a->mode != 1)) return 0;
     if (a->mode == 0 && !a->stat_partial) return 0;
     if (a->bst_x && (a->mode != 1 || !a->bst_mask || !a->stat_partial)) return 0;
+    if (a->in_scale || a->in_shift) {
+        if (a->mode != 0 || !a->in_scale || !a->in_shift || a->in_imgs_per_group <= 0 || a->n_img % a->in_imgs_per_group != 0) return 0;
+        if (a->in_valid < 0 || a->in_valid > a->in_imgs_per_group) return 0;
+    }
     return 1;
+}
+
+int fb_conv3x3_halo5_takes_fold(const fb_conv_args* a) {
+    static const float one = 0.f;
+    fb_conv_args b = *a;
+    b.in_scale = &one; b.in_shift = &one;
+    if (!b.stat_partial) b.stat_partial = const_cast<float*>(&one);
+    return b.mode == 0 && fb_conv3x3_halo5_takes(&b);
 }
 
 int fb_try_conv3x3_halo5(const fb_conv_args* a, hipStream_t st) {
@@ -317,12 +367,17 @@
     p.n_img = a->n_img; p.mode = a->mode; p.addend_mode = a->addend ? 1 : 0;
     p.n_tiles = a->n_img * 4;
     p.n_mblocks = p.n_tiles * 2;
+    p.in_scale = a->in_scale; p.in_shift = a->in_shift;
+    p.in_ipg = a->in_scale ? a->in_imgs_per_group : 1;
+    p.in_valid = a->in_valid > 0 ? a->in_valid : p.in_ipg;
 #ifdef FB_H5_TRACE
     extern long long* g_h5_trace;
     p.trace = g_h5_trace;
 #endif
     const dim3 grid(p.n_tiles < n_cu ? p.n_tiles : n_cu);
-    if (a->mode == 0) {
+    if (a->mode == 0 && a->in_scale) {
+        hipLaunchKernelGGL((conv3x3s1_c64_halo5_kernel<0, 0, 0, 1>), grid, dim3(256), 0, st, p);
+    } else if (a->mode == 0) {
         hipLaunchKernelGGL((conv3x3s1_c64_halo5_kernel<0, 0>), grid, dim3(256), 0, st, p);
     } else if (a->bst_x) {
         if (a->addend && a->addend_mask) hipLaunchKernelGGL((conv3x3s1_c64_halo5_kernel<1, 2, 1>), grid, dim3(256), 0, st, p);
diff --git a/fullbatchtraining_amd/csrc/conv_igemm.hip b/fullbatchtraining_amd/csrc/conv_igemm.hip
--- a/fullbatchtraining_amd/csrc/conv_igemm.hip
+++ b/fullbatchtraining_amd/csrc/conv_igemm.hip
@@ -181,6 +181,8 @@
 int fb_try_conv3x3_halo4(const fb_conv_args* a, hipStream_t st);
 int fb_try_conv3x3_halo5(const fb_conv_args* a, hipStream_t st);
 int fb_conv3x3_halo5_takes(const fb_conv_args* a);
+int fb_conv3x3_halo5_takes_fold(const fb_conv_args* a);
+int fb_wgrad3x3_v2_takes_fold(const fb_wgrad_args* a);
 int fb_try_conv3x3s2_dgrad_quad(const fb_conv_args* a, hipStream_t st);
 int fb_try_conv1x1_k32(const fb_conv_args* a, hipStream_t st);
 int fb_try_conv1x1_stream(const fb_conv_args* a, hipStream_t st);
@@ -205,6 +207,13 @@
     return fb_conv3x3_halo5_takes(a) || fb_conv1x1_pipe_takes(a) || fb_conv3x3_halo4_takes(a) || fb_conv1x1_gemm_takes(a) || igemm_masked_addend_ok(a);
 }
 
+extern "C" int32_t fb_conv_bn_fold_supported(const fb_conv_args* f, const fb_wgrad_args* w) {
+    const char* off = getenv("FB_DISABLE_BN1_FOLD");
+    if ((off && atoi(off) != 0) || !f || !w) return 0;
+    if (f->amax_src || f->amax_wgt || w->amax_x || w->amax_dy || w->bn_x) return 0;
+    return fb_conv3x3_halo5_takes_fold(f) && fb_wgrad3x3_v2_takes_fold(w);
+}
+
 extern "C" int32_t fb_conv_bwd_stat_supported(const fb_conv_args* a) {
     static const bool disabled = getenv("FB_DISABLE_FUSED_BWD_STAT") != nullptr;
     if (disabled || !a || !a->bst_x || !a->bst_mask || !a->stat_partial || a->mode != 1 || a->dtype != FB_BF16) return 0;
@@ -243,6 +252,8 @@
     if (a->bst_x && !fb_conv_bwd_stat_supported(a))
         FB_FAIL(FB_ERR_UNSUPPORTED, "fb_conv2d: the fused BatchNorm-backward reduction is not implemented for this shape (ask fb_conv_bwd_stat_supported)");
     if (a->stride != 1 && a->stride != 2) FB_FAIL(FB_ERR_UNSUPPORTED, "fb_conv2d: stride %d", a->stride);
+    if ((a->in_scale || a->in_shift) && !fb_conv3x3_halo5_takes(a))
+        FB_FAIL(FB_ERR_UNSUPPORTED, "fb_conv2d: in_scale / in_shift (BatchNorm + ReLU of the input in the loader) is not implemented for these arguments (ask fb_conv_bn_fold_supported)");
     ConvParams p;
     p.src = (const char*)a->src; p.wgt = (const char*)a->wgt; p.dst = (char*)a->dst; p.addend = (const char*)a->addend;
     p.stat = a->stat_partial;
diff --git a/fullbatchtraining_amd/csrc/conv_wgrad.hip b/fullbatchtraining_amd/csrc/conv_wgrad.hip
--- a/fullbatchtraining_amd/csrc/conv_wgrad.hip
+++ b/fullbatchtraining_amd/csrc/conv_wgrad.hip
@@ -248,6 +248,7 @@
 
 int fb_try_wgrad3x3(const fb_wgrad_args* a, hipStream_t st);
 int fb_try_wgrad3x3_v2(const fb_wgrad_args* a, hipStream_t st);
+int fb_wgrad3x3_v2_takes_fold(const fb_wgrad_args* a);
 int fb_try_wgrad1x1(const fb_wgrad_args* a, hipStream_t st);
 
 extern "C" int32_t fb_wgrad_bn_fused_supported(const fb_wgrad_args* a) {
@@ -260,6 +261,8 @@
     if (!a || !a->x || !a->dy || !a->dw_partial) FB_FAIL(FB_ERR_ARG, "fb_conv2d_wgrad: null pointer");
     if (a->bn_x && (!a->bn_coef || !fb_wgrad_bn_fused_supported(a))) FB_FAIL(FB_ERR_UNSUPPORTED, "fb_conv2d_wgrad: bn_x (BatchNorm apply in the loader) is for 1x1 layers with Cs < 64 (no fp16x2 planes) and needs bn_coef");
     if (a->Cs % 32 != 0 || a->Cd % 64 != 0) FB_FAIL(FB_ERR_SHAPE, "fb_conv2d_wgrad: Cs=%d must be a multiple of 32, Cd=%d of 64", a->Cs, a->Cd);
+    if ((a->x_scale || a->x_shift) && (!a->x_scale || !a->x_shift || a->bn_x || a->amax_x || a->amax_dy || a->x_valid < 0 || a->x_valid > a->imgs_per_group || !fb_wgrad3x3_v2_takes_fold(a)))
+        FB_FAIL(FB_ERR_UNSUPPORTED, "fb_conv2d_wgrad: x_scale / x_shift (BatchNorm + ReLU of x in the loader) is not implemented for these arguments (ask fb_conv_bn_fold_supported)");
     if (a->n_img % a->imgs_per_group != 0) FB_FAIL(FB_ERR_SHAPE, "fb_conv2d_wgrad: n_img %% imgs_per_group != 0");
     if (a->split_k < 1) FB_FAIL(FB_ERR_ARG, "fb_conv2d_wgrad: split_k < 1");
     WgradParams p;
diff --git a/fullbatchtraining_amd/csrc/conv_wgrad3x3_v2.hip b/fullbatchtraining_amd/csrc/conv_wgrad3x3_v2.hip
--- a/fullbatchtraining_amd/csrc/conv_wgrad3x3_v2.hip
+++ b/fullbatchtraining_amd/csrc/conv_wgrad3x3_v2.hip
@@ -8,6 +8,7 @@
     int imgs_per_group, imgs_per_block, split_k;
     long long group_stride;
     int n_chains; float* sq_part;
+    const float* x_scale; const float* x_shift; int x_valid;
 };
 
 namespace {
@@ -101,9 +102,10 @@
 };
 }
 
-template <int W, int SD, bool CP = false, bool CHAIN = false>
+template <int W, int SD, bool CP = false, bool CHAIN = false, bool FOLD = false>
 __global__ __launch_bounds__(CHAIN ? 512 : 256) void conv_wgrad3x3_v2_kernel(const Wgrad3V2Params p) {
 #if defined(__HIP_DEVICE_COMPILE__)
+    static_assert(!FOLD || (W == 32 && SD == 1 && !CP && !CHAIN), "folded input transform: 32x32 maps, stride 1");
     static_assert(!CP || (W == 4 && SD == 1), "compact layout: 4x4 maps, stride 1");
     static_assert(!CHAIN || CP, "chunk chains: compact 4x4 layout");
     constexpr int NWV = CHAIN ? 8 : 4, FIW = CHAIN ? 2 : 4;
@@ -200,6 +202,28 @@
         }
     };
 
+    float xsc[FOLD ? 8 : 1], xsh[FOLD ? 8 : 1];
+    if constexpr (FOLD) {
+        const int c0 = (((lane & 7) >> 1) ^ w3_f(wave * 8 + lrow8)) * 16 + (lane & 1) * 8;
+#pragma unroll
+        for (int k = 0; k < 8; ++k) { xsc[k] = p.x_scale[(long long)group * 64 + c0 + k]; xsh[k] = p.x_shift[(long long)group * 64 + c0 + k]; }
+    }
+    auto xform = [&](int stage, int step) {
+        if constexpr (FOLD) {
+            const int img = step / steps_per_img, y0 = (step % steps_per_img) * G::RS;
+            const bool img_ok = split * p.imgs_per_block + img < p.x_valid;
+#pragma unroll
+            for (int k = 0; k < KB; ++k) {
+                if (wave + NWV * k < NGB) {
+                    const bool live = img_ok && (unsigned)(y0 + hyB[k]) < (unsigned)Hi;
+                    uint4* q = (uint4*)(lds + stage * STAGE + A_BYTES + (wave + NWV * k) * 1024 + lane * 16);
+                    *q = fb_bn_relu_bf16x8(*q, xsc, xsh, live);
+                }
+            }
+            __builtin_amdgcn_fence(__ATOMIC_RELEASE, "workgroup");
+        }
+    };
+
     const unsigned lds0 = (unsigned)(size_t)(__attribute__((address_space(3))) char*)lds;
     const int t = lane & 15, g = lane >> 4;
     const int pl = g * 8 + (t >> 2);
@@ -232,6 +256,7 @@
     if (n_steps > 0) {
         issue(0, 0);
         w3_wait_vmcnt<0>();
+        xform(0, 0);
         __builtin_amdgcn_s_barrier();
     }
     for (int step = 0; step < n_steps; ++step) {
@@ -287,6 +312,7 @@
             }
         }
         w3_wait_vmcnt<0>();
+        if (step + 1 < n_steps) xform(cur ^ 1, step + 1);
         __builtin_amdgcn_s_barrier();
     }
 
@@ -302,6 +328,15 @@
             for (int q = 0; q < 4; ++q)
                 __builtin_amdgcn_raw_buffer_store_b32(__float_as_uint(CHAIN ? tot[u][i][q] : acc[u][i][q]), rsrcO, voffO, ((i * 16 + q) * 9 + u) * row4, 0);
 #endif
+}
+
+int fb_wgrad3x3_v2_takes_fold(const fb_wgrad_args* a) {
+    static const bool disabled = getenv("FB_DISABLE_WGRAD3_V2") != nullptr;
+    if (disabled || a->dtype != FB_BF16 || a->R != 3 || a->S != 3 || a->pad != 1 || a->stride != 1) return 0;
+    if (a->Hs != 32 || a->Ws != 32 || a->Hd != 32 || a->Wd != 32 || a->Cs != 64 || a->Cd != 64) return 0;
+    if (a->imgs_per_group <= 0 || a->split_k < 1 || a->n_img % a->imgs_per_group != 0) return 0;
+    const int imgs_per_block = (a->imgs_per_group + a->split_k - 1) / a->split_k;
+    return (long long)(imgs_per_block + 2) * 32 * 32 * 64 * 2 < (1LL << 31);
 }
 
 int fb_try_wgrad3x3_v2(const fb_wgrad_args* a, hipStream_t st) {
@@ -328,12 +363,15 @@
     p.imgs_per_group = a->imgs_per_group; p.split_k = a->split_k; p.imgs_per_block = imgs_per_block;
     p.group_stride = a->group_stride ? a->group_stride : (long long)a->split_k * a->Cd * 9 * a->Cs;
     p.n_chains = 0; p.sq_part = nullptr;
+    p.x_scale = a->x_scale; p.x_shift = a->x_shift; p.x_valid = a->x_valid > 0 ? a->x_valid : a->imgs_per_group;
+    if (a->x_scale && !fb_wgrad3x3_v2_takes_fold(a)) return 0;
     const int n_groups = a->n_img / a->imgs_per_group;
     dim3 grid((a->Cd / 64) * (a->Cs / 64) * n_groups * a->split_k);
     if (SD == 1) {
         if (W == 56) hipLaunchKernelGGL((conv_wgrad3x3_v2_kernel<56, 1>), grid, dim3(256), 0, st, p);
         else if (W == 28) hipLaunchKernelGGL((conv_wgrad3x3_v2_kernel<28, 1>), grid, dim3(256), 0, st, p);
         else if (W == 14) hipLaunchKernelGGL((conv_wgrad3x3_v2_kernel<14, 1>), grid, dim3(256), 0, st, p);
+        else if (W == 32 && a->x_scale) hipLaunchKernelGGL((conv_wgrad3x3_v2_kernel<32, 1, false, false, true>), grid, dim3(256), 0, st, p);
         else if (W == 32) hipLaunchKernelGGL((conv_wgrad3x3_v2_kernel<32, 1>), grid, dim3(256), 0, st, p);
         else if (W == 16) hipLaunchKernelGGL((conv_wgrad3x3_v2_kernel<16, 1>), grid, dim3(256), 0, st, p);
         else if (W == 8) hipLaunchKernelGGL((conv_wgrad3x3_v2_kernel<8, 1>), grid, dim3(256), 0, st, p);
@@ -370,6 +408,7 @@
     p.n_img = a->n_img; p.H = a->Hd; p.Cs = a->Cs; p.Cd = a->Cd;
     p.imgs_per_group = a->imgs_per_group; p.split_k = 1; p.imgs_per_block = a->imgs_per_group;
     p.group_stride = 0; p.n_chains = n_chains; p.sq_part = sq_part;
+    p.x_scale = nullptr; p.x_shift = nullptr; p.x_valid = 0;
     dim3 grid((a->Cd / 64) * (a->Cs / 64) * n_chains);
     hipLaunchKernelGGL((conv_wgrad3x3_v2_kernel<4, 1, true, true>), grid, dim3(512), 0, (hipStream_t)stream, p);
     FB_CHECK_LAUNCH("fb_conv2d_wgrad_chain");
diff --git a/fullbatchtraining_amd/csrc/runtime.cpp b/fullbatchtraining_amd/csrc/runtime.cpp
--- a/fullbatchtraining_amd/csrc/runtime.cpp
+++ b/fullbatchtraining_amd/csrc/runtime.cpp
@@ -7,7 +7,7 @@
 
 thread_local char fb_err_buf[512] = "";
 extern "C" const char* fb_last_error_string(void) { return fb_err_buf; }
-extern "C" int fb_abi_version(void) { return 13; }
+extern "C" int fb_abi_version(void) { return 14; }
 
 extern "C" int64_t fb_ws_conv_stat_floats(const fb_conv_args* a) {
     return a ? 2 * (((int64_t)a->n_img * a->Hd * a->Wd + 127) / 128) * a->Cd : 0;
diff --git a/fullbatchtraining_amd/engine.py b/fullbatchtraining_amd/engine.py
--- a/fullbatchtraining_amd/engine.py
+++ b/fullbatchtraining_amd/engine.py
@@ -152,6 +152,31 @@
     call("fb_stem_patches", x.data_ptr(), out.data_ptr(), n, c, h, w, layer.k_orig, layer.stride_orig, layer.pad_orig, layer.cin_pad,
          _ptr(oy), _ptr(ox), _ptr(fl), crop_pad, pv, lib.dtype_code(dtype))
     return out
+
+
+class _Mids:
+
+    def __init__(self, convs):
+        self._like, self._t = list(convs), [None] * len(convs)
+
+    def __len__(self):
+        return len(self._t)
+
+    def __getitem__(self, i):
+        if isinstance(i, slice):
+            return [self[k] for k in range(*i.indices(len(self._t)))]
+        if self._t[i] is None:
+            self._t[i] = torch.empty_like(self._like[i].x)
+        return self._t[i]
+
+    def __iter__(self):
+        return (self[i] for i in range(len(self._t)))
+
+    def __radd__(self, other):
+        return list(other) + list(self)
+
+    def allocated(self, i):
+        return self._t[i] is not None
 
 
 class _Events:
@@ -272,6 +297,7 @@
         self.cmdlists, self.replays, self.MAX_CMDLISTS = {}, 0, int(os.environ.get("FB_MAX_CMDLISTS", "256"))
         self.cmd_evictions, self.record_new, self.unrecorded_runs, self._warned_record_off, self._off_misses = 0, True, 0, False, 0
         self.masks = {}
+        self._fold_cache = {}
         exp = os.environ.get("FB_EXPERIMENTAL", "0") not in ("", "0")
         self.fuse_bwd_stat = exp and os.environ.get("FB_FUSED_BWD_STAT", "0") != "0"
         self.bst_done = False
@@ -346,7 +372,7 @@
             self.stem_pooled = torch.empty(n, hp, hp, 64, device=dev, dtype=dt)
             self.stem_pool_idx = torch.empty(n, hp, hp, 64, device=dev, dtype=torch.uint8) if os.environ.get("FB_MAXPOOL_IDX", "1") != "0" else None
         for b in self.plan.blocks:
-            b.mids = [torch.empty_like(c.x) for c in b.convs[:-1]]
+            b.mids = _Mids(b.convs[:-1])
             b.out = torch.empty_like(b.convs[-1].x)
             b.pooled = None
             if b.shortcut is not None and b.stride == 2:
@@ -529,7 +555,24 @@
         step = max(1, int(os.environ.get("FB_STEM_RANGE_BYTES", (1 << 31) - 1)) // per_chunk)
         return [(g0, min(step, G - g0)) for g0 in range(0, G, step)]
 
-    def _conv_bn_fwd(self, L, src, G, wsets, theta, pidx):
+    def _fold_ok(self, Lp, L, G, wsets):
+        if getattr(self, "_eval", False) or self.dt != torch.bfloat16 or self.f32_split == "f16x2" or Lp.cout != L.cin_pad:
+            return False
+        key = (L.li, G, wsets, self.chunk)
+        hit = self._fold_cache.get(key)
+        if hit is None:
+            n, one = G * self.chunk, self.theta.data_ptr()
+            f = lib.ConvArgs(one, one, one, None, one, n, L.hin, L.win, L.cin_pad, L.hout, L.wout, L.cout, L.R, L.S, L.stride, L.pad, 0,
+                             self.chunk if wsets > 1 else n, self.plan.wc_total if wsets > 1 else 0, 0, self.dtc, None, None, None, None, None, self.chunk,
+                             one, one, self.chunk, 0)
+            w = lib.WgradArgs(one, one, one, n, L.hin, L.win, L.cin_pad, L.hout, L.wout, L.cout, L.R, L.S, L.stride, L.pad, self.chunk, L.split_k, self.dtc, 0)
+            hit = self._fold_cache[key] = bool(lib.load().fb_conv_bn_fold_supported(lib.C.byref(f), lib.C.byref(w)))
+        return hit
+
+    def _fold_args(self, Lp, g0=0):
+        return (Lp.scale.data_ptr() + 4 * g0 * Lp.cout, Lp.shift.data_ptr() + 4 * g0 * Lp.cout, self.valid if self.valid < self.chunk else 0)
+
+    def _conv_bn_fwd(self, L, src, G, wsets, theta, pidx, fold=None):
         if L is self.plan.stem and len(self._stem_ranges(G)) > 1 and not getattr(self, "_in_stem_range", False):
             self._in_stem_range = True
             try:
@@ -539,9 +582,9 @@
             finally:
                 self._in_stem_range = False
             return
-        self._conv_bn_fwd_range(L, src, 0, G, wsets, theta, pidx)
-
-    def _conv_bn_fwd_range(self, L, src, g0, G, wsets, theta, pidx, amax=None):
+        self._conv_bn_fwd_range(L, src, 0, G, wsets, theta, pidx, fold=fold)
+
+    def _conv_bn_fwd_range(self, L, src, g0, G, wsets, theta, pidx, amax=None, fold=None):
         es = src.element_size()
         i0 = g0 * self.chunk
         src_ptr = src.data_ptr() + i0 * L.hin * L.win * L.cin_pad * es
@@ -560,6 +603,9 @@
         a = lib.ConvArgs(src_ptr, wptr, x_ptr, None, None if evalm else self.stat_ws.data_ptr(), n, L.hin, L.win, L.cin_pad, L.hout, L.wout,
                          L.cout, L.R, L.S, L.stride, L.pad, 0, self.chunk if wsets > 1 else n, self.plan.wc_total if wsets > 1 else 0,
                          0, self.dtc, None, None, None, am_s, am_w, self.chunk)
+        if fold is not None:
+            a.in_scale, a.in_shift, a.in_valid = self._fold_args(fold, g0)
+            a.in_imgs_per_group = self.chunk
         call("fb_conv2d", lib.C.byref(a))
         if evalm:
             return
@@ -614,11 +660,15 @@
             next_pool = nxt.pooled if nxt is not None else None
             a0 = a
             cur = a0
+            fold = None
             for i, L in enumerate(b.convs):
-                self._conv_bn_fwd(L, cur, G, wsets, theta, pidx)
+                self._conv_bn_fwd(L, cur, G, wsets, theta, pidx, fold=fold)
                 if i < len(b.convs) - 1:
-                    self._bn_apply(L, b.mids[i], G)
-                    cur = b.mids[i]
+                    if self._fold_ok(L, b.convs[i + 1], G, wsets):
+                        fold, cur = L, L.x
+                    else:
+                        self._bn_apply(L, b.mids[i], G)
+                        fold, cur = None, b.mids[i]
             last = b.convs[-1]
             if b.shortcut is not None:
                 src = a0
@@ -641,10 +691,21 @@
              0.0 if getattr(self, "_eval", False) else float(self.label_smoothing), 0 if getattr(self, "_eval", False) else int(self.only_incorrect))
         return a
 
-    def _bn_bwd(self, L, dout, mask, G, gout, pidx, want_dy, reduced=False, apply=True):
+    def _bn_bwd(self, L, dout, mask, G, gout, pidx, want_dy, reduced=False, apply=True, affine=False):
         n = G * self.chunk
         px = n * L.hout * L.wout
         ppg = self.chunk * L.hout * L.wout
+        if affine:
+            valid_px = self.valid * L.hout * L.wout if self.valid < self.chunk else 0
+            dx = self.pool.get((n, L.hout, L.wout, L.cout))
+            call("fb_bn_bwd_reduce_ax", dout.data_ptr(), L.x.data_ptr(), L.scale.data_ptr(), L.shift.data_ptr(), valid_px, self.mean_tab[pidx].data_ptr(),
+                 L.invstd.data_ptr(), self.plan.ch_total, L.ch_off, self.stat_ws.data_ptr(), px, L.cout, ppg, self.dtc)
+            call("fb_bn_bwd_finalize", self.stat_ws.data_ptr(), lib.load().fb_bn_bwd_reduce_rows(px, ppg), G, L.cout, float(self.valid * L.hout * L.wout),
+                 L.scale.data_ptr(), self.mean_tab[pidx].data_ptr(), L.invstd.data_ptr(), self.plan.ch_total, L.ch_off,
+                 gout.data_ptr() + 4 * L.g_off, gout.data_ptr() + 4 * L.b_off, self.plan.P, L.coef.data_ptr(), 0)
+            call("fb_bn_bwd_apply_ax", dout.data_ptr(), L.x.data_ptr(), L.scale.data_ptr(), L.shift.data_ptr(), valid_px, L.coef.data_ptr(), dx.data_ptr(),
+                 px, L.cout, ppg, self.dtc)
+            return dx, None
         bits = self.masks.get(mask.data_ptr()) if mask is not None else None
         y = None if bits is not None else mask
         dx = self.pool.get((n, L.hout, L.wout, L.cout)) if apply else None
@@ -703,7 +764,7 @@
         a = lib.WgradArgs(None, None, None, self.chunk, L.hin, L.win, L.cin_pad, L.hout, L.wout, L.cout, L.R, L.S, L.stride, L.pad, self.chunk, 1, self.dtc, 0)
         return bool(lib.load().fb_wgrad_bn_fused_supported(lib.C.byref(a)))
 
-    def _wgrad(self, L, src, dx, G, gout, bn=None):
+    def _wgrad(self, L, src, dx, G, gout, bn=None, fold=None):
         n = G * self.chunk
         if bn is not None:
             dx = bn[0]
@@ -740,7 +801,8 @@
                                                 self.plan.P if direct else 0, am_x + 4 * g0 if am_x is not None else None,
                                                 am_dy + 4 * g0 if am_dy is not None else None,
                                                 *((L.x.data_ptr() + i0 * L.hout * L.wout * L.cout * es, self.masks[bn[1].data_ptr()].data_ptr() + i0 * L.hout * L.wout * L.cout * es // 16,
-                                                   L.coef.data_ptr() + 4 * g0 * L.cout * 3) if bn is not None else (None, None, None)))))
+                                                   L.coef.data_ptr() + 4 * g0 * L.cout * 3) if bn is not None else (None, None, None)),
+                                                *(self._fold_args(fold, g0) if fold is not None else (None, None, 0)))))
 
         def launch():
             for g0, g_n, a in args:
@@ -819,16 +881,17 @@
                 consumer = None if plan.stem_pool else (plan.stem, self.stem_out)
             if not lazy:
                 pool.put(d)
-            srcs = [a0] + b.mids
             cur_dx = dx
             for i in range(len(b.convs) - 1, -1, -1):
                 L = b.convs[i]
-                self._wgrad(L, srcs[i], cur_dx, G, gout)
+                Lp = b.convs[i - 1] if i > 0 else None
+                folded = Lp is not None and self._fold_ok(Lp, L, G, wsets)
+                self._wgrad(L, a0 if i == 0 else (Lp.x if folded else b.mids[i - 1]), cur_dx, G, gout, fold=Lp if folded else None)
                 ev_cur = self._wgrad_event
                 if i > 0:
-                    d_mid = self._dgrad(L, cur_dx, G, wsets, bst=(b.convs[i - 1], b.mids[i - 1]))
+                    d_mid = self._dgrad(L, cur_dx, G, wsets, bst=None if folded else (Lp, b.mids[i - 1]))
                     pool.put(cur_dx, event=ev_cur)
-                    cur_dx, _ = self._bn_bwd(b.convs[i - 1], d_mid, b.mids[i - 1], G, gout, pidx, want_dy=False, reduced=self.bst_done)
+                    cur_dx, _ = self._bn_bwd(Lp, d_mid, None if folded else b.mids[i - 1], G, gout, pidx, want_dy=False, reduced=self.bst_done, affine=folded)
                     pool.put(d_mid)
             if b.shortcut is not None:
                 S = b.shortcut
diff --git a/fullbatchtraining_amd/lib.py b/fullbatchtraining_amd/lib.py
--- a/fullbatchtraining_amd/lib.py
+++ b/fullbatchtraining_amd/lib.py
@@ -5,7 +5,7 @@
 import torch
 
 FB_F32, FB_BF16 = 0, 1
-EXPECTED_ABI = 13
+EXPECTED_ABI = 14
 MT_BLOCKS = 1024
 _LIB_PATH = os.environ.get("FB_LIB_PATH") or os.path.join(os.path.dirname(os.path.abspath(__file__)), "csrc", "libfbengine.so")
 
@@ -17,7 +17,8 @@
                 ("n_img", c_int), ("Hs", c_int), ("Ws", c_int), ("Cs", c_int), ("Hd", c_int), ("Wd", c_int), ("Cd", c_int),
                 ("R", c_int), ("S", c_int), ("stride", c_int), ("pad", c_int), ("mode", c_int),
                 ("imgs_per_wset", c_int), ("wset_stride", c_i64), ("addend_mode", c_int), ("dtype", c_int), ("addend_mask", c_void_p),
-                ("bst_x", c_void_p), ("bst_mask", c_void_p), ("amax_src", c_void_p), ("amax_wgt", c_void_p), ("amax_imgs", c_int)]
+                ("bst_x", c_void_p), ("bst_mask", c_void_p), ("amax_src", c_void_p), ("amax_wgt", c_void_p), ("amax_imgs", c_int),
+                ("in_scale", c_void_p), ("in_shift", c_void_p), ("in_imgs_per_group", c_int), ("in_valid", c_int)]
 
 
 class WgradArgs(C.Structure):
@@ -25,7 +26,8 @@
                 ("n_img", c_int), ("Hs", c_int), ("Ws", c_int), ("Cs", c_int), ("Hd", c_int), ("Wd", c_int), ("Cd", c_int),
                 ("R", c_int), ("S", c_int), ("stride", c_int), ("pad", c_int),
                 ("imgs_per_group", c_int), ("split_k", c_int), ("dtype", c_int), ("group_stride", c_i64), ("amax_x", c_void_p), ("amax_dy", c_void_p),
-                ("bn_x", c_void_p), ("bn_mask", c_void_p), ("bn_coef", c_void_p)]
+                ("bn_x", c_void_p), ("bn_mask", c_void_p), ("bn_coef", c_void_p),
+                ("x_scale", c_void_p), ("x_shift", c_void_p), ("x_valid", c_int)]
 
 
 _SIGS = {
@@ -43,6 +45,8 @@
     "fb_bn_bwd_finalize": [c_void_p, c_int, c_int, c_int, c_double, c_void_p, c_void_p, c_void_p, c_int, c_int, c_void_p, c_void_p,
                            c_i64, c_void_p, c_int, c_void_p],
     "fb_bn_bwd_apply": [c_void_p, c_void_p, c_void_p, c_void_p, c_void_p, c_void_p, c_void_p, c_i64, c_int, c_i64, c_int, c_void_p, c_void_p, c_void_p],
+    "fb_bn_bwd_reduce_ax": [c_void_p, c_void_p, c_void_p, c_void_p, c_i64, c_void_p, c_void_p, c_int, c_int, c_void_p, c_i64, c_int, c_i64, c_int, c_void_p],
+    "fb_bn_bwd_apply_ax": [c_void_p, c_void_p, c_void_p, c_void_p, c_i64, c_void_p, c_void_p, c_i64, c_int, c_i64, c_int, c_void_p],
     "fb_bn_bwd_reduce2": [c_void_p, c_void_p, c_void_p, c_void_p, c_int, c_void_p, c_void_p, c_void_p, c_int, c_void_p, c_void_p, c_int, c_i64, c_int, c_i64, c_int,
                           c_void_p],
     "fb_bn_bwd_apply2": [c_void_p, c_void_p, c_void_p, c_void_p, c_void_p, c_void_p, c_void_p, c_void_p, c_i64, c_int, c_i64, c_int, c_void_p],
@@ -86,7 +90,7 @@
 }
 EXPORTS = tuple(_SIGS) + ("fb_last_error_string", "fb_abi_version", "fb_profile_enable", "fb_profile_read", "fb_ws_conv_stat_floats",
                           "fb_ws_wgrad_slab_floats", "fb_ws_bn_partial_floats", "fb_ws_mt_floats", "fb_bn_bwd_reduce_rows", "fb_conv_masked_addend_supported", "fb_conv_bwd_stat_supported",
-                          "fb_bn_apply_can_pool", "fb_ws_bn_amax_floats", "fb_profile_read_launches", "fb_cmd_fn_id", "fb_cmd_fn_nargs", "fb_event_new", "fb_event_count", "fb_bn_bwd_fused_supported", "fb_ws_bn_bwd_fused_floats", "fb_ws_bn_bwd_fused_ints", "fb_wgrad_bn_fused_supported", "fb_wgrad_chain_supported",
+                          "fb_bn_apply_can_pool", "fb_ws_bn_amax_floats", "fb_profile_read_launches", "fb_cmd_fn_id", "fb_cmd_fn_nargs", "fb_event_new", "fb_event_count", "fb_bn_bwd_fused_supported", "fb_ws_bn_bwd_fused_floats", "fb_ws_bn_bwd_fused_ints", "fb_wgrad_bn_fused_supported", "fb_wgrad_chain_supported", "fb_conv_bn_fold_supported",
                           "fb_event_record", "fb_event_wait", "fb_cmdlist_create", "fb_cmdlist_destroy", "fb_cmdlist_size", "fb_cmdlist_add_call",
                           "fb_cmdlist_add_event", "fb_cmdlist_replay")
 PROF_CLASSES = ("igemm_fwd", "igemm_dgrad", "wgrad", "bn_apply", "bn_bwd_reduce", "bn_bwd_apply", "bn_bwd_fused")
@@ -161,6 +165,7 @@
         lib.fb_ws_bn_bwd_fused_ints.argtypes, lib.fb_ws_bn_bwd_fused_ints.restype = [c_i64], c_i64
         lib.fb_wgrad_bn_fused_supported.argtypes, lib.fb_wgrad_bn_fused_supported.restype = [C.POINTER(WgradArgs)], c_int
         lib.fb_wgrad_chain_supported.argtypes, lib.fb_wgrad_chain_supported.restype = [C.POINTER(WgradArgs)], c_int
+        lib.fb_conv_bn_fold_supported.argtypes, lib.fb_conv_bn_fold_supported.restype = [C.POINTER(ConvArgs), C.POINTER(WgradArgs)], c_int
         lib.fb_cmd_fn_id.argtypes, lib.fb_cmd_fn_id.restype = [C.c_char_p], c_int
         lib.fb_cmd_fn_nargs.argtypes, lib.fb_cmd_fn_nargs.restype = [c_int], c_int
         lib.fb_event_new.argtypes, lib.fb_event_new.restype = [], c_int
diff --git a/include/fb_engine.h b/include/fb_engine.h
--- a/include/fb_engine.h
+++ b/include/fb_engine.h
@@ -41,6 +41,8 @@
     const void* bst_x; const void* bst_mask;
     const float* amax_src; const float* amax_wgt;
     int32_t amax_imgs;
+    const float* in_scale; const float* in_shift;
+    int32_t in_imgs_per_group; int32_t in_valid;
 } fb_conv_args;
 int fb_conv2d(const fb_conv_args* a, void* stream);
 int32_t fb_conv_masked_addend_supported(const fb_conv_args* a);
@@ -55,9 +57,11 @@
     int64_t group_stride;
     const float* amax_x; const float* amax_dy;
     const void* bn_x; const void* bn_mask; const float* bn_coef;
+    const float* x_scale; const float* x_shift; int32_t x_valid;
 } fb_wgrad_args;
 int32_t fb_wgrad_bn_fused_supported(const fb_wgrad_args* a);
 int fb_conv2d_wgrad(const fb_wgrad_args* a, void* stream);
+int32_t fb_conv_bn_fold_supported(const fb_conv_args* f, const fb_wgrad_args* w);
 int32_t fb_wgrad_chain_supported(const fb_wgrad_args* a);
 int fb_conv2d_wgrad_chain(const fb_wgrad_args* a, int32_t n_chains, float* slabs, float* sq_part, void* stream);
 
@@ -90,6 +94,12 @@
                        float* dgamma, float* dbeta, int64_t grad_group_stride, float* coef, int32_t raw_x, void* stream);
 int fb_bn_bwd_apply(const void* dout, const void* y, const void* mask, const void* x, const float* coef, void* dx, void* dy_out,
                     int64_t n_pixels, int32_t C, int64_t pixels_per_group, int32_t dtype, float* amax_out, float* amax_ws, void* stream);
+
+int fb_bn_bwd_reduce_ax(const void* dout, const void* x, const float* scale, const float* shift, int64_t valid_pixels_per_group,
+                        const float* mean_tab, const float* invstd, int32_t ch_total, int32_t ch_off, float* partial, int64_t n_pixels,
+                        int32_t C, int64_t pixels_per_group, int32_t dtype, void* stream);
+int fb_bn_bwd_apply_ax(const void* dout, const void* x, const float* scale, const float* shift, int64_t valid_pixels_per_group,
+                       const float* coef, void* dx, int64_t n_pixels, int32_t C, int64_t pixels_per_group, int32_t dtype, void* stream);
 
 int fb_bn_bwd_reduce2(const void* dout, const void* mask, const void* x_a, const float* invstd_a, int32_t ch_off_a, float* partial_a,
                       const void* x_b, const float* invstd_b, int32_t ch_off_b, float* partial_b, const float* mean_tab, int32_t ch_total,
```

Result: no change. 217,500 (-0.7%).
